# yzh119/custom_op_benchmark

Measured on AMD Instinct MI355X. Metric: edges/sec fwd+bwd (SDDMM+softmax+SpMM) on Reddit d=64; HBM GB/s vs roofline, higher is better.
Workload: dtype f32; 1 GPU; reddit-shape Chung-Lu(alpha=0.50) graph, N=232965 E=114615892 per GPU, h=1 d=64, U[0,1) values, chunk_size=32, int64 CSR both orientations; graph=reddit, nodes=232965, edges=114615892, heads=1, d=64, chunk_size=32, row_chunks=3694777, col_chunks=3694424, parallelism=single GPU

## Files before the change

custom_op_benchmark_amd/_lib.py:

```python
import atexit
import collections
import ctypes
import os
import weakref

import torch

_HERE = os.path.dirname(os.path.abspath(__file__))
LIB_PATH = os.environ.get("GRAPHOP_LIB") or os.path.join(_HERE, "libgraphop_hip.so")
ABI_VERSION = 8

F32, F64 = 0, 1
_c64 = ctypes.c_int64
_vp = ctypes.c_void_p
_lib = None


class PlanInfo(ctypes.Structure):
    _fields_ = [("n_chunks", _c64), ("n_edges", _c64), ("n_segments", _c64), ("max_row", _c64),
                ("max_index", _c64), ("max_segment_len", _c64), ("rows_sorted", ctypes.c_int32),
                ("indptr_monotone", ctypes.c_int32), ("eid_identity", ctypes.c_int32),
                ("full_coverage", ctypes.c_int32), ("row_owned", ctypes.c_int32),
                ("has_idx32", ctypes.c_int32), ("dense_fill_pct", ctypes.c_int32),
                ("sorted_in_rows", ctypes.c_int32), ("n_dense_blocks", _c64), ("max_row_gap", _c64),
                ("n_geometry_fallbacks", _c64)]


class SweepInfo(ctypes.Structure):
    _fields_ = [("win_cols", _c64), ("W", ctypes.c_int32), ("T", ctypes.c_int32), ("V", ctypes.c_int32),
                ("n_dealt", ctypes.c_int32)]


ALLOC_FN = ctypes.CFUNCTYPE(ctypes.c_void_p, ctypes.c_size_t, ctypes.c_int, ctypes.c_void_p)
FREE_FN = ctypes.CFUNCTYPE(None, ctypes.c_void_p)


class ProfileRec(ctypes.Structure):
    _fields_ = [("name", ctypes.c_char * 48), ("kernel", ctypes.c_char * 48), ("calls", _c64), ("total_ms", ctypes.c_double),
                ("min_ms", ctypes.c_double), ("max_ms", ctypes.c_double)]


_P = _vp
_SIGNATURES = {
    "graphop_tune": [ctypes.c_char_p, ctypes.c_int],
    "graphop_tune_reset": [],
    "graphop_check_device_errors": [],
    "graphop_tune_get": [ctypes.c_char_p, ctypes.POINTER(ctypes.c_int)],
    "graphop_profile_enable": [ctypes.c_int],
    "graphop_profile_read": [ctypes.POINTER(ProfileRec), ctypes.c_int],
    "graphop_partition_csr_count": [_P, _c64, _c64, _P, _P],
    "graphop_partition_csr_fill": [_P, _P, _c64, _c64, _c64, _P, _P, _P],
    "graphop_plan_create": [_P, _P, _P, _P, _c64, _c64, _c64, _P, ctypes.POINTER(_vp)],
    "graphop_plan_info": [_P, ctypes.POINTER(PlanInfo)],
    "graphop_set_allocator": [ALLOC_FN, FREE_FN],
    "graphop_plan_prepare": [_P, ctypes.c_int, _c64, _c64, _c64, ctypes.c_int, _P],
    "graphop_plan_n_sweeps": [_P],
    "graphop_plan_sweep_info": [_P, ctypes.c_int, ctypes.POINTER(SweepInfo)],
    "graphop_plan_array": [_P, ctypes.c_char_p, ctypes.c_int, ctypes.POINTER(_vp), ctypes.POINTER(_c64)],
    "graphop_plan_import": [_P] * 4 + [ctypes.POINTER(PlanInfo)] + [_P] * 4 + [_c64] + [_P] * 4 + [ctypes.POINTER(_vp)],
    "graphop_plan_import_sweep": [_P, ctypes.POINTER(SweepInfo), _P, _P, _P, _P],
    "graphop_plan_sweep_dealt": [_P, ctypes.c_int, ctypes.c_int, ctypes.POINTER(ctypes.c_int32), ctypes.POINTER(ctypes.c_int32)],
    "graphop_plan_sweep_build_dealt": [_P, ctypes.POINTER(SweepInfo), ctypes.c_int32, ctypes.c_int32, _P],
    "graphop_maskedmm_csr_forward": [ctypes.c_int] + [_P] * 7 + [_c64] * 6 + [_P, _P],
    "graphop_maskedmm_csr_forward_partial": [ctypes.c_int] + [_P] * 7 + [_c64] * 7 + [_P],
    "graphop_maskedmm_csr_backward": [ctypes.c_int] + [_P] * 13 + [_c64] * 7 + [_P, _P, _P],
    "graphop_sparse_softmax_forward": [ctypes.c_int] + [_P] * 5 + [_c64] * 3 + [_P, _c64, _P, _P],
    "graphop_sparse_softmax_backward": [ctypes.c_int] + [_P] * 6 + [_c64] * 3 + [_P, _c64, _P, _P],
    "graphop_vector_spmm_forward": [ctypes.c_int] + [_P] * 7 + [_c64] * 6 + [_P, _P],
    "graphop_vector_spmm_backward": [ctypes.c_int] + [_P] * 13 + [_c64] * 7 + [_P, _P, _P],
    "graphop_spmm_pair_supported": [ctypes.c_int] + [_c64] * 5 + [_P],
    "graphop_spmm_pair": [ctypes.c_int] + [_P] * 9 + [_c64] * 6 + [_P, _P],
    "graphop_interleave_pairs": [ctypes.c_int, _P, _P, _P, _c64, _P],
    "graphop_node_mul_edge_forward": [ctypes.c_int] + [_P] * 6 + [_c64] * 5 + [_P, _P],
    "graphop_node_mul_edge_backward": [ctypes.c_int] + [_P] * 8 + [_c64] * 5 + [_P, _P],
    "graphop_gat_scores_forward": [ctypes.c_int] + [_P] * 7 + [_c64] * 5 + [ctypes.c_double, _P, _P],
    "graphop_gat_scores_backward": [ctypes.c_int] + [_P] * 13 + [_c64] * 6 + [ctypes.c_double, _P, _P, _P],
    "graphop_gatv2_scores_forward": [ctypes.c_int] + [_P] * 8 + [_c64] * 6 + [ctypes.c_double, _P, _P],
    "graphop_gatv2_scores_backward": [ctypes.c_int] + [_P] * 16 + [_c64] * 8 + [ctypes.c_double, _P, _P, _P],
    "graphop_gatv2_attention_forward": [ctypes.c_int] + [_P] * 9 + [_c64] * 6 + [ctypes.c_double, _P, _P],
    "graphop_gatv2_attention_backward": [ctypes.c_int] + [_P] * 18 + [_c64] * 8 + [ctypes.c_double, _P, _P, _P],
    "graphop_gatv2_attention_dropout_forward": [ctypes.c_int] + [_P] * 9 + [_c64] * 6
    + [ctypes.c_double, ctypes.c_double, ctypes.c_uint64, ctypes.c_uint32, _P, _P],
    "graphop_gatv2_attention_dropout_backward": [ctypes.c_int] + [_P] * 18 + [_c64] * 8
    + [ctypes.c_double, ctypes.c_double, ctypes.c_uint64, ctypes.c_uint32, _P, _P, _P],
    "graphop_gat_attention_forward": [ctypes.c_int] + [_P] * 9 + [_c64] * 6 + [ctypes.c_double, _P, _P],
    "graphop_gat_attention_backward": [ctypes.c_int] + [_P] * 18 + [_c64] * 8 + [ctypes.c_double, _P, _P, _P],
    "graphop_gat_attention_dropout_forward": [ctypes.c_int] + [_P] * 9 + [_c64] * 6
    + [ctypes.c_double, ctypes.c_double, ctypes.c_uint64, ctypes.c_uint32, _P, _P],
    "graphop_gat_attention_dropout_backward": [ctypes.c_int] + [_P] * 18 + [_c64] * 8
    + [ctypes.c_double, ctypes.c_double, ctypes.c_uint64, ctypes.c_uint32, _P, _P, _P],
    "graphop_edge_dropout_mask": [ctypes.c_int] + [_P] * 5 + [_c64] * 5
    + [ctypes.c_double, ctypes.c_uint64, ctypes.c_uint32, _P, _P],
    "graphop_gat_edge_attention_forward": [ctypes.c_int] + [_P] * 10 + [_c64] * 6
    + [ctypes.c_double, ctypes.c_double, ctypes.c_uint64, ctypes.c_uint32, _P, _P],
    "graphop_gat_edge_attention_backward": [ctypes.c_int] + [_P] * 20 + [_c64] * 8
    + [ctypes.c_double, ctypes.c_double, ctypes.c_uint64, ctypes.c_uint32, _P, _P, _P],
    "graphop_gatv2_edge_attention_forward": [ctypes.c_int] + [_P] * 10 + [_c64] * 6
    + [ctypes.c_double, ctypes.c_double, ctypes.c_uint64, ctypes.c_uint32, _P, _P],
    "graphop_gatv2_edge_attention_backward": [ctypes.c_int] + [_P] * 20 + [_c64] * 8
    + [ctypes.c_double, ctypes.c_double, ctypes.c_uint64, ctypes.c_uint32, _P, _P, _P],
    "graphop_gather_rows": [ctypes.c_int, _P, _P, _P, _c64, _c64, _c64, _P],
    "graphop_scatter_add_rows": [ctypes.c_int, _P, _P, _P, _c64, _c64, _c64, _P],
    "graphop_add_rows_unique": [ctypes.c_int, _P, _P, _P, _c64, _c64, _c64, _P],
    "graphop_add_rows_grouped": [ctypes.c_int, _P, _P, _P, _P, _P, _c64, _c64, _c64, _P],
    "graphop_attention_workspace_bytes": [ctypes.c_int, ctypes.c_int] + [_c64] * 5 + [_P, _P, _P,
                                                                                       ctypes.POINTER(_c64)],
    "graphop_attention_backward_is_fused": [ctypes.c_int] + [_c64] * 5 + [_P, _P, _P, ctypes.POINTER(ctypes.c_int)],
    "graphop_attention_forward": [ctypes.c_int] + [_P] * 9 + [_c64] * 6 + [_P, _c64, _P, _P],
    "graphop_attention_backward": [ctypes.c_int] + [_P] * 17 + [_c64] * 7 + [_P, _c64, _P, _P, _P],
    "graphop_attention_dropout_workspace_bytes": [ctypes.c_int, ctypes.c_int] + [_c64] * 5 + [_P, _P, _P,
                                                                                               ctypes.POINTER(_c64)],
    "graphop_attention_dropout_forward": [ctypes.c_int] + [_P] * 9 + [_c64] * 6 + [_P, _c64, _P, _P]
    + [ctypes.c_double, ctypes.c_uint64, ctypes.c_uint32, _c64],
    "graphop_attention_dropout_backward": [ctypes.c_int] + [_P] * 17 + [_c64] * 7 + [_P, _c64, _P, _P, _P]
    + [ctypes.c_double, ctypes.c_uint64, ctypes.c_uint32, _c64],
    "graphop_attention_bias_workspace_bytes": [ctypes.c_int, ctypes.c_int] + [_c64] * 5 + [_P, _P, _P, ctypes.c_int,
                                                                                            ctypes.POINTER(_c64)],
    "graphop_attention_bias_forward": [ctypes.c_int] + [_P] * 10 + [_c64] * 6 + [_P, _c64, _P, _P]
    + [ctypes.c_double, ctypes.c_uint64, ctypes.c_uint32, _c64],
    "graphop_attention_bias_backward": [ctypes.c_int] + [_P] * 19 + [_c64] * 7 + [_P, _c64, _P, _P, _P]
    + [ctypes.c_double, ctypes.c_uint64, ctypes.c_uint32, _c64],
    "graphop_attention_edge_workspace_bytes": [ctypes.c_int, ctypes.c_int] + [_c64] * 5 + [_P, _P, _P,
                                                                                            ctypes.POINTER(_c64)],
    "graphop_attention_edge_forward": [ctypes.c_int] + [_P] * 10 + [_c64] * 6 + [_P, _c64, _P, _P]
    + [ctypes.c_double, ctypes.c_uint64, ctypes.c_uint32, _c64],
    "graphop_attention_edge_backward": [ctypes.c_int] + [_P] * 19 + [_c64] * 7 + [_P, _c64, _P, _P, _P]
    + [ctypes.c_double, ctypes.c_uint64, ctypes.c_uint32, _c64],
    "graphop_attention_etype_workspace_bytes": [ctypes.c_int, ctypes.c_int] + [_c64] * 6 + [_P, _P, _P,
                                                                                             ctypes.POINTER(_c64)],
    "graphop_attention_etype_forward": [ctypes.c_int] + [_P] * 11 + [_c64] * 7 + [_P, _c64, _P, _P]
    + [ctypes.c_double, ctypes.c_uint64, ctypes.c_uint32, _c64],
    "graphop_attention_etype_backward": [ctypes.c_int] + [_P] * 20 + [_c64] * 8 + [_P, _c64, _P, _P, _P]
    + [ctypes.c_double, ctypes.c_uint64, ctypes.c_uint32, _c64],
    "graphop_attention_tbias_workspace_bytes": [ctypes.c_int, ctypes.c_int] + [_c64] * 6 + [_P, _P, _P,
                                                                                             ctypes.POINTER(_c64)],
    "graphop_attention_tbias_forward": [ctypes.c_int] + [_P] * 11 + [_c64] * 7 + [_P, _c64, _P, _P]
    + [ctypes.c_double, ctypes.c_uint64, ctypes.c_uint32, _c64],
    "graphop_attention_tbias_backward": [ctypes.c_int] + [_P] * 20 + [_c64] * 8 + [_P, _c64, _P, _P, _P]
    + [ctypes.c_double, ctypes.c_uint64, ctypes.c_uint32, _c64],
    "graphop_attention_weights": [ctypes.c_int] + [_P] * 10 + [_c64] * 6 + [_P, _P],
}
EXPORTED_SYMBOLS = sorted(list(_SIGNATURES) + ["graphop_abi_version", "graphop_last_error",
                                               "graphop_plan_destroy", "graphop_memory_bytes", "graphop_tune_key"])


def lib():
    global _lib
    if _lib is None:
        if not os.path.exists(LIB_PATH):
            raise RuntimeError(
                "graphop: %s is missing -- the HIP extension has not been built. Run "
                "`python -c 'import __graft_entry__ as g; g.build()'` (or `make -C "
                "custom_op_benchmark_amd/csrc`). There is no CPU fallback." % LIB_PATH)
        l = ctypes.CDLL(LIB_PATH)
        l.graphop_abi_version.restype = ctypes.c_int
        l.graphop_last_error.restype = ctypes.c_char_p
        l.graphop_plan_destroy.restype = None
        l.graphop_plan_destroy.argtypes = [_vp]
        l.graphop_memory_bytes.restype = ctypes.c_int64
        l.graphop_memory_bytes.argtypes = []
        l.graphop_tune_key.restype = ctypes.c_char_p
        l.graphop_tune_key.argtypes = [ctypes.c_int]
        for name, argtypes in _SIGNATURES.items():
            fn = getattr(l, name)
            fn.restype = ctypes.c_int
            fn.argtypes = argtypes
        if l.graphop_abi_version() != ABI_VERSION:
            raise RuntimeError("graphop: ABI version mismatch (library %d, binding %d)"
                               % (l.graphop_abi_version(), ABI_VERSION))
        if os.environ.get("GRAPHOP_TORCH_ALLOC", "1") != "0":
            l.graphop_set_allocator(_ALLOC_CB, _FREE_CB)
            atexit.register(_drop_allocator, l)
        _lib = l
    return _lib


_live_blocks = {}

# ... 379 lines not shown
```

custom_op_benchmark_amd/csrc/common.h:

```cpp
#pragma once

#include <hip/hip_runtime.h>
#include <stdint.h>
#include <stdio.h>
#include <stdlib.h>
#include <string.h>

#include <utility>

#include "graphop_hip.h"

namespace graphop {

using i64 = long long;

void set_error(const char* fmt, ...) __attribute__((format(printf, 1, 2)));
const char* get_error();

#define GO_CHECK_ARG(cond, ...)                \
  do {                                         \
    if (!(cond)) {                             \
      ::graphop::set_error(__VA_ARGS__);       \
      return GRAPHOP_ERR_INVALID_ARGUMENT;     \
    }                                          \
  } while (0)

#define GO_HIP(expr)                                                                      \
  do {                                                                                    \
    hipError_t _e = (expr);                                                               \
    if (_e != hipSuccess) {                                                               \
      ::graphop::set_error("%s failed: %s (%s:%d)", #expr, hipGetErrorString(_e), __FILE__, \
                           __LINE__);                                                     \
      return GRAPHOP_ERR_HIP;                                                             \
    }                                                                                     \
  } while (0)

#define GO_LAUNCH_CHECK() GO_HIP(hipGetLastError())

inline int env_int(const char* name, int dflt) {
  const char* v = getenv(name);
  return (v && *v) ? atoi(v) : dflt;
}

inline i64 ceil_div(i64 a, i64 b) { return (a + b - 1) / b; }

hipError_t go_malloc(void** p, size_t bytes, hipStream_t st);
void go_free(void* p);
bool go_alloc_stream_ordered();

int check_not_capturing(hipStream_t st, const char* what);

int* device_error_word(bool create);
int check_async_error(bool clear = false);
int tuning_plan_trim();
int walk_launch_id(const char* tag);

struct PlanStats {
  i64 unsorted;
  i64 bad_indptr;
  i64 eid_not_identity;
  i64 bad_eid;
  i64 bad_index;
  i64 max_row;
  i64 max_gap;
  i64 max_index;
  i64 max_seg_len;
  i64 n_segments;
  i64 unsorted_ids;
};

}

namespace graphop {
struct Sweep {
  int W = 0;
  i64 win_cols = 0;
  int T = 0;
  int V = 0;
  int* vr_row = nullptr;
  int* wp_lo = nullptr;
  int* wp_hi = nullptr;
  int runtime_wp = 0;
  int* queues = nullptr;
  unsigned queue_next = 0;
  struct Dealt {
    int L = 0, K = 0;
    int tiles = 0;
    int* rec = nullptr;
    int* ids = nullptr;
    int* eids = nullptr;
    long long n_ids = 0;
  };
  static constexpr int kMaxDealt = 4;
  Dealt dealt[kMaxDealt];
  int n_dealt = 0;
};
struct Walk {
  int W = 0;
  i64 win_cols = 0;
  int groups = 0;
  int GW = 0;
  int K = 0;
  int rounds = 0;
  int xcd_slots = 0;
  long long n_slots = 0;
  int* ids = nullptr;
  int* widx = nullptr;
  int* bin_pos = nullptr;
  int* bin_rows = nullptr;
  int* bin_cum = nullptr;
  int* sync = nullptr;
  long long sync_ints = 0;
  unsigned sync_next = 0;
  int max_steps = 0;
  long long longest_run = 0;
};
constexpr int kWalkSyncRing = 4;
constexpr int kWalkK = 15;
constexpr int kWalkFirstPiece = 1 << 30;
constexpr int kWalkRowMask = (1 << 30) - 1;
constexpr int kWalkKShift = 26;
constexpr long long kLongSegment = 1024;
constexpr long long kLongSegmentBwd = 2048;
constexpr int kQueueRing = 64;
constexpr int kQueueInts = 8 * 64;
}

struct graphop_plan {
  graphop_plan_info_t info;
  int sorted_in_rows;
  void* sweeps;
  void* sweep_mu;
  void* walks;
  const int64_t* row;
  const int64_t* indptr;
  const int64_t* eid;
  const int64_t* indices;
  int64_t* seg_chunk;
  int64_t* seg_eptr;
  int32_t* idx32;
  int32_t* eid32;
  int32_t* long_segs;
  int64_t n_long;
  int32_t* blk_seg;
  int32_t* seg_e0;
  int32_t* seg_row;
  int device;
  int mirrors_pinned;
};

#ifdef __HIPCC__
namespace graphop {

constexpr int kWave = 64;

template <int CTRL>
__device__ __forceinline__ float dpp_f32(float v) {
  return __builtin_bit_cast(
      float, __builtin_amdgcn_update_dpp(0, __builtin_bit_cast(int, v), CTRL, 0xF, 0xF, true));
}

template <int CTRL>
__device__ __forceinline__ double dpp_f64(double v) {
  const long long b = __builtin_bit_cast(long long, v);
  const int lo = __builtin_amdgcn_update_dpp(0, (int)b, CTRL, 0xF, 0xF, true);
  const int hi = __builtin_amdgcn_update_dpp(0, (int)(b >> 32), CTRL, 0xF, 0xF, true);
  return __builtin_bit_cast(double, ((long long)hi << 32) | (unsigned)lo);
}
template <int CTRL> __device__ __forceinline__ float dpp_t(float v) { return dpp_f32<CTRL>(v); }
template <int CTRL> __device__ __forceinline__ double dpp_t(double v) { return dpp_f64<CTRL>(v); }

template <int G>
__device__ __forceinline__ double group_sum(double v) {
  if constexpr (G >= 2) v += dpp_f64<0xB1>(v);
  if constexpr (G >= 4) v += dpp_f64<0x4E>(v);
  if constexpr (G >= 8) v += dpp_f64<0x141>(v);
  if constexpr (G >= 16) v += dpp_f64<0x140>(v);
  if constexpr (G >= 32) v += __shfl_xor(v, 16);
  if constexpr (G >= 64) v += __shfl_xor(v, 32);
  return v;
}

template <int G>
__device__ __forceinline__ float group_sum(float v) {
  if constexpr (G >= 2) v += dpp_f32<0xB1>(v);
  if constexpr (G >= 4) v += dpp_f32<0x4E>(v);
  if constexpr (G >= 8) v += dpp_f32<0x141>(v);
  if constexpr (G >= 16) v += dpp_f32<0x140>(v);
  if constexpr (G >= 32) v += __shfl_xor(v, 16);
  if constexpr (G >= 64) v += __shfl_xor(v, 32);
  return v;
}

__device__ __forceinline__ float group_sum_rt(float v, int g) {
  switch (g) {
    case 2: return group_sum<2>(v);
    case 4: return group_sum<4>(v);
    case 8: return group_sum<8>(v);
    case 16: return group_sum<16>(v);
    case 32: return group_sum<32>(v);
    case 64: return group_sum<64>(v);
    default: return v;
  }
}

template <typename F, int... I>
__device__ __forceinline__ void static_for_impl(F&& f, std::integer_sequence<int, I...>) {
  (f(std::integral_constant<int, I>{}), ...);
}
template <int N, typename F>
__device__ __forceinline__ void static_for(F&& f) {
  static_for_impl(f, std::make_integer_sequence<int, N>{});
}

template <int L, int U>
__device__ __forceinline__ int group_bcast(int v) {
  static_assert(U >= 0 && U < L, "lane out of range");
  if constexpr (L == 16) {
    return __builtin_amdgcn_update_dpp(0, v, 0x150 + U, 0xF, 0xF, true);
  } else if constexpr (L == 4) {
    return __builtin_amdgcn_update_dpp(0, v, U * 0x55, 0xF, 0xF, true);
  } else if constexpr (L == 8) {
    const int lo = __builtin_amdgcn_update_dpp(0, v, 0x150 + U, 0xF, 0xF, true);
    const int hi = __builtin_amdgcn_update_dpp(0, v, 0x150 + U + 8, 0xF, 0xF, true);
    return (threadIdx.x & 8) ? hi : lo;
  } else if constexpr (L == 64) {
    return __builtin_amdgcn_readlane(v, U);
  } else if constexpr (L == 32) {
    const int lo = __builtin_amdgcn_readlane(v, U);
    const int hi = __builtin_amdgcn_readlane(v, U + 32);
    return (threadIdx.x & 32) ? hi : lo;
  } else {
    return __shfl(v, U, L);
  }
}
template <int L, int U>
__device__ __forceinline__ unsigned group_bcast(unsigned v) { return (unsigned)group_bcast<L, U>((int)v); }
template <int L, int U>
__device__ __forceinline__ float group_bcast(float v) {
  return __builtin_bit_cast(float, group_bcast<L, U>(__builtin_bit_cast(int, v)));
}
template <int L, int U>
__device__ __forceinline__ double group_bcast(double v) {
  const long long b = __builtin_bit_cast(long long, v);
  const int lo = group_bcast<L, U>((int)b), hi = group_bcast<L, U>((int)(b >> 32));
  return __builtin_bit_cast(double, ((long long)hi << 32) | (unsigned)lo);
}

// ... 97 lines not shown
```

custom_op_benchmark_amd/csrc/graphop_hip.hip:

```cpp
#include <stdarg.h>

#include <map>
#include <mutex>
#include <set>
#include <string>
#include <vector>

#include "common.h"
#include "host.h"
#include "host_attn_rows.h"
#include "kernels_fast.h"
#include "kernels_walk.h"
#include "kernels_attn_walk.h"
#include "kernels_attn_bias_fwd.h"
#include "kernels_block.h"
#include "kernels_attn.h"
#include "kernels_generic.h"

namespace graphop {

namespace {

inline int cpg_for(i64 n_chunks, int cpg_max, int F) {
  return (int)chunks_per_group(n_chunks, F >= 256 ? 64 : (F / 4 > 0 ? F / 4 : 1), cpg_max);
}

inline unsigned blocks_for(i64 work, i64 per_block) {
  i64 b = ceil_div(work > 0 ? work : 1, per_block);
  return (unsigned)b;
}

inline bool fast_ok(int dtype, i64 h, i64 d, i64 n_edges, i64 n_src_rows) {
  if (tuning().force_generic || dtype != GRAPHOP_F32) return false;
  const i64 F = h * d;
  if (d % 4 != 0 || !pow2(F) || F < 16 || F > 1024 || !pow2(h)) return false;
  if (n_edges >= 0x7fffffffLL || n_src_rows >= 0x7fffffffLL) return false;
  return true;
}

inline bool fast64_ok(int dtype, i64 h, i64 d, i64 n_edges, i64 n_src_rows) {
  if (tuning().force_generic || dtype != GRAPHOP_F64 || h != 1) return false;
  if (d != 32 && d != 64 && d != 128) return false;
  return n_edges < 0x7fffffffLL && n_src_rows < 0x7fffffffLL;
}
}

int choose_sweep(const graphop_plan* plan, i64 n_table_rows, int L, int NV, hipStream_t st,
                 SweepLaunch* out, bool accumulating, const SweepOpts* opts) {
  const Tuning& t = tuning();
  if (!t.sweep || !plan) return 0;
  const graphop_plan_info_t& pi = plan->info;
  if (!pi.row_owned || !plan->sorted_in_rows || !pi.has_idx32 || !plan->indices) return 0;
  if (pi.n_segments == 0 || pi.n_edges == 0) return 0;
  const i64 row_bytes = (opts && opts->row_bytes > 0) ? opts->row_bytes : 16LL * L * NV;
  const i64 table_bytes = n_table_rows * row_bytes;
  if (table_bytes < (i64)t.sweep_min_kb * 1024) return 0;
  const i64 mean_row = pi.n_edges / pi.n_segments;
  auto windows_ok = [&](i64 w) {
    return w >= 2 && w <= t.max_windows && mean_row >= (i64)t.sweep_min_granule * w;
  };
  int coarse = (accumulating && pi.eid_identity && t.spmm_window_scale > 1) ? t.spmm_window_scale : 1;
  const i64 win_kb = (opts && opts->window_scale > 0) ? (i64)t.window_kb * opts->window_scale : (i64)t.window_kb;
  if (opts && opts->window_scale > 0) coarse = 1;
  i64 W = pow2ceil(ceil_div(table_bytes, win_kb * 1024));
  if (t.sweep_w > 0) W = t.sweep_w;
  if (!windows_ok(W)) {
    coarse = 1;
    W = table_bytes > (128LL << 20) ? pow2ceil(ceil_div(table_bytes, (i64)t.mall_window_kb * 1024)) : 0;
    if (!windows_ok(W)) return 0;
  } else if (t.sweep_w <= 0 && coarse > 1) {
    const i64 Wc = pow2ceil(ceil_div(table_bytes, (i64)t.window_kb * 1024 * coarse));
    if (Wc >= 2) W = Wc; else coarse = 1;
  } else if (t.sweep_w <= 0 && !accumulating && !(opts && opts->window_scale > 0) && row_bytes >= 1024) {
    while (W > 2 && mean_row < 12 * W) W >>= 1;
  }
  if (W < 2 || W > t.max_windows) return 0;
  const i64 win_cols = ceil_div(n_table_rows, W);
  int K = t.sweep_k > 0 ? t.sweep_k : (8 / NV > 0 ? 8 / NV : 1);
  if (opts && opts->K > 0) K = opts->K;
  if (t.sweep_k <= 0 && !(opts && opts->K > 0) && !pi.eid_identity && K > 1) K /= 2;
  if (K > L) K = L;
  const int gpb = kFastBlock / L;
  const int bpc_req = (opts && opts->bpc > 0) ? (opts->bpc < t.sweep_bpc || opts->window_scale > 0 ? opts->bpc : t.sweep_bpc)
                                              : t.sweep_bpc;
  const int bpc = bpc_req < 1 ? 1 : (bpc_req > kSweepBlocksPerCu ? kSweepBlocksPerCu : bpc_req);
  int T = t.vrow_t;
  if (T <= 0) {
    const i64 resident_vrows = (i64)t.n_cu * bpc * gpb * K;
    i64 target = pi.n_edges / (resident_vrows > 0 ? resident_vrows : 1);
    i64 p2 = 64;
    while (p2 * 2 <= target && p2 < 4096) p2 <<= 1;
    T = (int)(p2 * coarse * ((opts && opts->window_scale > 0) ? opts->window_scale : 1));
  }
  const Sweep* sw = nullptr;
  const int rc = plan_get_sweep(const_cast<graphop_plan*>(plan), (int)W, win_cols, T, st, &sw);
  if (rc != GRAPHOP_OK) return -rc;
  if (!sw) return 0;
  const int tile = (kWave / L) * K;
  const i64 tiles = ceil_div(sw->V, tile);
  if (tiles * ceil_div((i64)sw->W, 8) >= 0x7fffffffLL) return 0;
  out->view = SweepView{};
  const bool dry = opts && opts->dry_run;
  out->view.sync = dry ? nullptr : plan_take_queue(const_cast<graphop_plan*>(plan), sw);
  out->view.V = sw->V;
  out->view.W = sw->W;
  out->view.K = K;
  out->view.win_bytes = win_cols * row_bytes;
  out->view.table_bytes = table_bytes;
  out->view.touch = opts ? opts->touch : 0;
  if (!dry && zero_async(out->view.sync, sizeof(int) * kQueueInts, st) != hipSuccess) return -GRAPHOP_ERR_HIP;
  i64 nb = (i64)t.n_cu * bpc;
  const i64 need = ceil_div(tiles * sw->W, (i64)(kFastBlock / kWave));
  if (nb > need) nb = need;
  out->blocks = (unsigned)(nb < 1 ? 1 : nb);
  out->lds_bytes = (size_t)gpb * K * row_bytes;
  bool staged_ok = false;
  if (opts && opts->staged) {
    const Sweep::Dealt* dl = nullptr;
    const int rcd = plan_get_dealt(const_cast<graphop_plan*>(plan), sw, L, K, st, &dl, !opts->no_eids);
    if (rcd != GRAPHOP_OK) return -rcd;
    if (dl) {
      out->view.rec = (const int4*)dl->rec;
      out->view.ids_w = dl->ids;
      out->view.eids_w = dl->eids;
      out->lds_bytes += (size_t)gpb * opts->stage_lds_per_group;
      staged_ok = pi.eid_identity || dl->eids != nullptr || opts->no_eids;
    }
  }
  if (!staged_ok) {
    const int rcp = plan_pin_sweep_tables(const_cast<graphop_plan*>(plan), sw, st);
    if (rcp != GRAPHOP_OK) return -rcp;
  }
  out->view.wp_lo = sw->wp_lo;
  out->view.wp_hi = sw->wp_hi;
  out->view.vr_row = sw->vr_row;
  out->view.idx32 = plan->idx32;
  out->view.eid32 = plan->eid32;
  plan_trim(const_cast<graphop_plan*>(plan));
  out->view.wp_lo = sw->wp_lo;
  out->view.wp_hi = sw->wp_hi;
  out->view.idx32 = plan->idx32;
  out->view.eid32 = plan->eid32;
  return 1;
}

namespace {

inline bool table_off32(i64 n_table_rows, int L, int NV) { return n_table_rows * 16LL * L * NV < (1LL << 32); }
inline bool sddmm_staged_heads(int L, int NV, i64 h, i64 n_edges) {
  if (h < 2 || NV != 1 || L < 16 || L % h != 0 || n_edges * h >= 0x7fffffffLL) return false;
  const i64 d4 = L / h;
  return d4 == 4 || d4 == 8 || d4 == 16 || d4 == 32;
}
inline bool sddmm_staged(const graphop_plan* plan, int L, int NV, i64 h, i64 n_table_rows) {
  return (tuning().staged_ids & 1) && plan->info.eid_identity &&
         (h == 1 || (sddmm_staged_heads(L, NV, h, plan->info.n_edges) && table_off32(n_table_rows, L, NV)));
}
inline bool spmm_staged(int L, int NV, i64 h, i64 n_table_rows) {
  return (tuning().staged_ids & 2) && h == 1 && table_off32(n_table_rows, L, NV);
}

inline void allow_full_lds(const void* fn) {
  static std::mutex mu;
  static std::set<std::pair<int, const void*>> done;
  int dev = 0;
  (void)hipGetDevice(&dev);
  std::lock_guard<std::mutex> lk(mu);
  if (done.insert({dev, fn}).second)
    (void)hipFuncSetAttribute(fn, hipFuncAttributeMaxDynamicSharedMemorySize, 160 * 1024 - 1024);
}
struct WalkLaunch {
  WalkView view;
  unsigned blocks;
  size_t lds_bytes;
};

struct WalkDebug {
  long long* buf = nullptr;
  unsigned blocks = 0;
  const char* tag = "";
  hipStream_t st = nullptr;
  int rounds = 0, W = 0, waves_per_wg = 4;
  void arm(WalkLaunch* wl, const char* t, hipStream_t s, int wpw = 4) {
    waves_per_wg = wpw;
    if (!tuning().walk_debug) return;
    blocks = wl->blocks; tag = t; st = s; rounds = wl->view.rounds; W = wl->view.steps;
    if (hipMalloc((void**)&buf, sizeof(long long) * 34 * blocks) != hipSuccess) { buf = nullptr; return; }
    (void)hipMemsetAsync(buf, 0, sizeof(long long) * 34 * blocks, s);
    wl->view.dbg = buf;
  }
  ~WalkDebug() {
    if (!buf) return;
    std::vector<long long> h((size_t)34 * blocks);
    if (hipStreamSynchronize(st) == hipSuccess &&
        hipMemcpy(h.data(), buf, sizeof(long long) * h.size(), hipMemcpyDeviceToHost) == hipSuccess) {
      double tot = 0, wait = 0, nw = 0, feed = 0, ftot = 0, fspace = 0; long long tmax = 0, tmin = 1LL << 62; int gave = 0;
      for (size_t b = 0; b < blocks; ++b) { ftot += h[(size_t)32 * blocks + 2 * b]; fspace += h[(size_t)32 * blocks + 2 * b + 1]; }
      double xt[8] = {0}, xw[8] = {0}; int xn[8] = {0};
      const size_t n = (size_t)waves_per_wg * blocks;
      for (size_t i = 0; i < n; ++i) {
        const long long* d = &h[i * 4];
        tot += d[0]; wait += d[1]; nw += d[2] & 0xffff; feed += (double)(d[2] >> 16);
        tmax = d[0] > tmax ? d[0] : tmax; tmin = d[0] < tmin ? d[0] : tmin;
        gave += (d[3] & 16) ? 1 : 0;
        const int x = (int)(d[3] & 7); xt[x] += d[0]; xw[x] += d[1]; xn[x]++;
      }
      fprintf(stderr, "[walk] %s rounds=%d steps=%d waves=%zu cycles mean %.0f min %lld max %lld | pacer wait %.1f %% of wave time, %.1f waits/wave, %d gave up | per XCD wait%%:",
              tag, rounds, W, n, tot / n, tmin, tmax, 100.0 * wait / (tot > 0 ? tot : 1), nw / n, gave);
      for (int x = 0; x < 8; ++x) fprintf(stderr, " %.0f(%d)", xn[x] ? 100.0 * xw[x] / (xt[x] > 0 ? xt[x] : 1) : 0.0, xn[x]);
      fprintf(stderr, " | workers wait for the feeder %.1f %%; feeder: %.0f cycles, %.1f %% waiting for ring space", 100.0 * feed / (tot > 0 ? tot : 1),
              ftot / (blocks ? blocks : 1), 100.0 * fspace / (ftot > 0 ? ftot : 1));
      fprintf(stderr, "\n");
    }
    (void)hipFree(buf);
  }
};

template <int L, int NV>
int choose_walk(const graphop_plan* plan, i64 n_table_rows, int K, hipStream_t st, WalkLaunch* out, bool dry_run = false,
                int tables = 1) {
  if constexpr (NV != 1 || L < 16) {
    return 0;
  } else {
    const Tuning& t = tuning();
    if (!plan) return 0;
    const graphop_plan_info_t& pi = plan->info;
    if (!pi.row_owned || !plan->sorted_in_rows || !pi.has_idx32 || !plan->indices) return 0;
    if (pi.n_segments == 0 || pi.n_edges == 0) return 0;
    if (pi.max_index >= (1LL << kWalkKShift) || n_table_rows > (1LL << kWalkKShift)) return 0;
    const i64 table_bytes = n_table_rows * 16LL * L * NV;
    if (table_bytes < (i64)t.sweep_min_kb * 1024) return 0;
    const i64 win_kb = pi.eid_identity ? t.walk_window_kb : (16LL * L * NV >= 1024 ? 2 * (i64)t.walk_window_kb_col : t.walk_window_kb_col);
    i64 W = t.sweep_w > 0 ? t.sweep_w : pow2ceil(ceil_div(table_bytes * tables, (win_kb > 0 ? win_kb : 1) * 1024));
    if (W < 2) W = 2;
    if (W > t.max_windows || W > 512) return 0;
    const i64 mean_row = pi.n_edges / pi.n_segments;
    if (mean_row < (i64)t.sweep_min_granule * W / 2) return 0;
    const int GPB = kWalkWorkers / L;
    i64 blocks = t.walk_blocks > 0 ? ceil_div((i64)t.walk_blocks * kFastBlock, kWalkWorkers) : (i64)t.n_cu;
    int slots = 8;
    if (blocks >= 8) blocks -= blocks % 8; else slots = 1;
    const i64 groups = blocks * GPB;
    if (pi.n_edges < groups * (i64)t.walk_min_bin) return 0;
    if (K < 1 || K > kWalkK) return 0;
    const Walk* wk = nullptr;
    const int rc = plan_get_walk(const_cast<graphop_plan*>(plan), (int)W, ceil_div(n_table_rows, W), (int)groups, 1, K,
                                 slots, st, &wk, tables == 1);
    if (rc != GRAPHOP_OK) return -rc;
    plan_trim(const_cast<graphop_plan*>(plan));
    if (!wk) return 0;
    out->view.ids = wk->ids; out->view.widx = wk->widx; out->view.bin_pos = wk->bin_pos;
    out->view.bin_rows = wk->bin_rows; out->view.bin_cum = wk->bin_cum;
    out->view.W = wk->W; out->view.groups = wk->groups; out->view.rounds = wk->rounds;
    out->view.K = wk->K;
    out->view.xcd_slots = slots;
    {
      i64 steps = (i64)wk->W * (t.walk_steps > 0 ? t.walk_steps : 1);
      if (steps > wk->max_steps) steps = wk->max_steps;
      if (steps > wk->longest_run / 16) steps = wk->longest_run / 16;
      out->view.steps = (int)(steps < 1 ? 1 : steps);
    }
    out->view.drift = t.walk_drift;
    out->view.sync = (t.walk_drift > 0 && !dry_run) ? plan_take_walk_sync(const_cast<graphop_plan*>(plan), wk) : nullptr;
    out->view.dbg = nullptr;
    out->view.err = device_error_word(false);
    out->view.launch_id = 0;
    out->view.fault = t.walk_fault;
    out->view.stream_weights = pi.eid_identity ? 1 : 0;
    out->blocks = (unsigned)blocks;
    out->lds_bytes = 0;
    if (!dry_run && out->view.sync &&
        zero_async(out->view.sync, sizeof(int) * 64 * (size_t)(8 + 16 * (i64)wk->rounds * out->view.steps), st) != hipSuccess)
      return -GRAPHOP_ERR_HIP;
    return 1;
  }
}

template <int L, int NV>
inline int spmm_walk_k(i64 h, int dtype = GRAPHOP_F32) {
  if (h != 1 && h != 2 && h != 4 && h != 8) return 0;
  if (dtype == GRAPHOP_F64 && h != 1) return 0;
  if (h > 1 && (NV != 1 || (4 * L) % h != 0 || (4 * L / h) % 4 != 0)) return 0;
// ... 24 lines not shown
      allow_full_lds((const void*)kfn);
      if (tuning().walk_debug) {
        int nb = -1;
        (void)hipOccupancyMaxActiveBlocksPerMultiprocessor(&nb, (const void*)kfn, kWalkThreads, lds_bytes);
        hipFuncAttributes fa;
        (void)hipFuncGetAttributes(&fa, (const void*)kfn);
        fprintf(stderr, "[walk] occupancy API: %d workgroups of %d threads per CU (dynamic LDS %zu, static %zu, regs %d, K %d)\n", nb,
                kWalkThreads, lds_bytes, (size_t)fa.sharedSizeBytes, fa.numRegs, K);
      }
      hipLaunchKernelGGL(kfn, dim3(wl.blocks), dim3(kWalkThreads), lds_bytes, st, wl.view, args...);
    };
    if (dtype == GRAPHOP_F64) {
      if constexpr (spmm_walk_rows<L, NV>(1, 2) >= 8) {
        const size_t lds_bytes = spmm_walk_lds_bytes<L, NV>(K, 1, 2);
        if (off32) launch(k_spmm_walk_f64<L, NV, true>, lds_bytes, (const double*)w, (const double*)X, (double*)out);
        else launch(k_spmm_walk_f64<L, NV, false>, lds_bytes, (const double*)w, (const double*)X, (double*)out);
      }
      return 1;
    }
    auto go = [&](auto hc) {
      constexpr int HV = decltype(hc)::value;
      if constexpr (spmm_walk_rows<L, NV>(HV) < 8) return;
      else {
        const size_t lds_bytes = spmm_walk_lds_bytes<L, NV>(K, HV);
        if constexpr (HV == 1) {
          if (!off32) { launch(k_spmm_walk_f32<L, NV, 1, false>, lds_bytes, (const float*)w, (const float*)X, (float*)out, d4); return; }
        }
        launch(k_spmm_walk_f32<L, NV, HV, true>, lds_bytes, (const float*)w, (const float*)X, (float*)out, d4);
      }
    };
    switch ((int)h) {
      case 1: go(std::integral_constant<int, 1>{}); break;
      case 2: go(std::integral_constant<int, 2>{}); break;
      case 4: go(std::integral_constant<int, 4>{}); break;
      default: go(std::integral_constant<int, 8>{}); break;
    }
    return 1;
  }
}

}

int attn_fwd_walk(const graphop_plan* plan, i64 n_q, i64 n_k, i64 h, i64 d, int dtype, const void* Q, const void* K,
                  const void* V, void* o, void* stats, void* ws, i64 ws_bytes, hipStream_t st, bool dry_run,
                  size_t* ws_needed, const AttnDrop* drop) {
  constexpr int L = 16;
  const Tuning& t = tuning();
  if (ws_needed) *ws_needed = 0;
  if (!t.attn_fwd_walk || !t.attn_fused || t.force_generic || dtype != GRAPHOP_F32 || h != 1 || d != 4 * L || !plan) return 0;
  if (!plan->info.eid_identity || !(t.walk & 2) || !table_off32(n_k, L, 1)) return 0;
  if (plan->info.max_row >= n_q || plan->info.max_index >= n_k) return 0;
  constexpr int KR = attn_walk_rows<L>();
  static_assert(KR >= 4, "rows per lane group of the fused forward");
  WalkLaunch wl;
  const int use = choose_walk<L, 1>(plan, n_k, KR, st, &wl, dry_run, 2);
  if (use != 1) return use;
  if (t.walk_steps > 1 && wl.view.steps >= 2 * t.walk_steps) wl.view.steps /= t.walk_steps;
  const i64 bins = (i64)wl.view.groups * wl.view.rounds, F = 4 * L;
  const AttnRowsFwdWs w(ws, 2 * bins, n_q, 1, F);
  if (ws_needed) *ws_needed = w.total;
  if (dry_run) return 1;
  if (!ws || (size_t)ws_bytes < w.total) return 0;
  AttnWalkArgs a;
  a.Q = (const float*)Q; a.K = (const float*)K; a.V = (const float*)V; a.o = (float*)o; a.stats = (float*)stats;
  a.p_row = w.p_row; a.p_ml = w.p_ml; a.p_o = w.p_o;
  if (zero_async(o, sizeof(float) * (size_t)(n_q * F), st) != hipSuccess) return -GRAPHOP_ERR_HIP;
  attn_pieces_fill("attn_fwd_setup", w, kAttnNegBig, st);
  {
    WalkDebug dbg;
    dbg.arm(&wl, "attn_fwd", st, kWalkWorkers / kWave);
    wl.view.launch_id = walk_launch_id("attn_fwd");
    ProfScope prof("attn_fwd", st, drop ? "k_attn_fwd_walk_f32<DROP>" : "k_attn_fwd_walk_f32");
    const size_t lds_bytes = (size_t)(kWalkWorkers / L) * attn_walk_group_bytes<L>(KR);
    if (drop) {
      allow_full_lds((const void*)k_attn_fwd_walk_f32<L, true>);
      hipLaunchKernelGGL((k_attn_fwd_walk_f32<L, true>), dim3(wl.blocks), dim3(kWalkThreads), lds_bytes, st, wl.view, a, *drop);
    } else {
      allow_full_lds((const void*)k_attn_fwd_walk_f32<L, false>);
      hipLaunchKernelGGL((k_attn_fwd_walk_f32<L, false>), dim3(wl.blocks), dim3(kWalkThreads), lds_bytes, st, wl.view, a, NoDrop{});
    }
  }
  attn_pieces_merge(
      "attn_fwd_merge", "k_attn_piece_add", w, L, st,
      [&](dim3 grid, dim3 block) { hipLaunchKernelGGL(k_attn_piece_max, grid, block, 0, st, w.p_row, w.p_ml, w.Mtmp, w.np); },
      [&](dim3 grid, dim3 block) {
        hipLaunchKernelGGL((k_attn_piece_add<L>), grid, block, 0, st, w.p_row, w.p_ml, w.p_o, w.Mtmp, w.Ltmp, a.o, w.np);
      },
      [&](dim3 grid, dim3 block) {
        hipLaunchKernelGGL((k_attn_piece_fin<L>), grid, block, 0, st, w.p_row, w.Mtmp, w.Ltmp, a.o, a.stats, w.np);
      });
  if (hipGetLastError() != hipSuccess) return -GRAPHOP_ERR_HIP;
  return 1;
}

int attn_bias_fwd_rows(const Csr& g, i64 n_q, i64 n_k, i64 h, i64 d, int dtype, const void* Q, const void* K,
                       const void* V, const void* b, void* o, void* stats, void* ws, i64 ws_bytes, hipStream_t st,
                       bool dry_run, size_t* ws_needed, const AttnDrop* drop) {
  const Tuning& t = tuning();
  const graphop_plan* plan = g.plan;
  const i64 n_chunks = g.n_chunks, n_edges = g.n_edges;
  if (ws_needed) *ws_needed = 0;
  if (!t.attn_fused || !t.attn_rows || t.force_generic || dtype != GRAPHOP_F32 || h != 1 || !plan) return 0;
  if (d % 4 != 0 || !pow2(d) || d < 16 || d > 1024 || n_edges == 0 || n_chunks == 0) return 0;
  if (!g.owned() || !plan->indices) return 0;
  if (plan->info.max_row >= n_q || plan->info.max_index >= n_k || n_q >= kWalkRowMask) return 0;
  const i64 F = d;
  const ChunkGeometry geo = attn_one_head_geometry(n_chunks, F);
  if (2 * geo.groups >= 0x7fffffffLL) return 0;
  const AttnRowsFwdWs w(ws, 2 * geo.groups, n_q, 1, F);
  if (ws_needed) *ws_needed = w.total;
  if (dry_run) return 1;
  if (!ws || (size_t)ws_bytes < w.total) return 0;
  AttnBiasFwdArgs a;
  a.Q = (const float*)Q; a.K = (const float*)K; a.V = (const float*)V; a.b = (const float*)b;
  a.o = (float*)o; a.stats = (float*)stats;
  a.p_row = w.p_row; a.p_ml = w.p_ml; a.p_o = w.p_o;
  if (zero_async(o, sizeof(float) * (size_t)(n_q * F), st) != hipSuccess) return -GRAPHOP_ERR_HIP;
  attn_pieces_fill("attn_bias_fwd_setup", w, kAttnNegBig, st);
  const i64* eids = g.eid_or_null();
  {
    ProfScope prof("attn_bias_fwd_rows", st, drop ? "k_attn_bias_fwd_rows_f32<DROP>" : "k_attn_bias_fwd_rows_f32");
    GO_DISPATCH_LNV((int)F, {
      if (drop)
        hipLaunchKernelGGL((k_attn_bias_fwd_rows_f32<L, NV, true>), dim3(geo.blocks), dim3(kFastBlock), 0, st,
                           g.row, g.indptr, eids, g.indices, a, n_chunks,
                           (int)geo.cpg, *drop);
      else
        hipLaunchKernelGGL((k_attn_bias_fwd_rows_f32<L, NV, false>), dim3(geo.blocks), dim3(kFastBlock), 0, st,
                           g.row, g.indptr, eids, g.indices, a, n_chunks,
                           (int)geo.cpg, NoDrop{});
    });
  }
  attn_pieces_merge(
      "attn_bias_fwd_merge", "k_attn_bias_piece_add", w, geo.lanes, st,
      [&](dim3 grid, dim3 block) { hipLaunchKernelGGL(k_attn_piece_max, grid, block, 0, st, w.p_row, w.p_ml, w.Mtmp, w.np); },
      [&](dim3 grid, dim3 block) {
        GO_DISPATCH_LNV((int)F, {
          hipLaunchKernelGGL((k_attn_bias_piece_add<L, NV>), grid, block, 0, st, w.p_row, w.p_ml, w.p_o, w.Mtmp, w.Ltmp,
                             a.o, w.np);
        });
      },
      [&](dim3 grid, dim3 block) {
        GO_DISPATCH_LNV((int)F, {
          hipLaunchKernelGGL((k_attn_bias_piece_fin<L, NV>), grid, block, 0, st, w.p_row, w.Mtmp, w.Ltmp, a.o, a.stats,
                             w.np);
        });
      });
  if (hipGetLastError() != hipSuccess) return -GRAPHOP_ERR_HIP;
  return 1;
}

namespace {

template <int L, int NV>
int try_sddmm_sweep(const char* tag, int dtype, const graphop_plan* plan, i64 n_table_rows, const void* A,
                    const void* B, void* y, i64 h, int d4, hipStream_t st) {
  if (!plan) return 0;
  SweepLaunch sl;
  SweepOpts so;
  const bool f64 = dtype == GRAPHOP_F64;
  if (f64 && (h != 1 || NV != 1 || L < 16 || !sddmm_staged(plan, L, NV, h, n_table_rows))) return 0;
  const bool off32 = table_off32(n_table_rows, L, NV);
  so.bpc = (f64 || !off32) ? 3 : sweep_bpc(NV, h == 1);
  so.touch = tuning().touch_sddmm;
  const bool id = plan->info.eid_identity != 0;
  so.staged = sddmm_staged(plan, L, NV, h, n_table_rows);
  so.stage_lds_per_group = StageCfg<L, 1>::kLdsIntsPerGroup * (int)sizeof(int) + (h > 1 ? 64 * (int)h : 0);
  if (h > 1 && !aligned16(y)) so.staged = false;
  const int use = choose_sweep(plan, n_table_rows, L, NV, st, &sl, false, &so);
  if (use != 1) return use;
  const bool staged = sl.view.rec != nullptr;
  if (f64 && !staged) return 0;
  ProfScope prof(tag, st, f64 ? "k_sddmm_wown_staged_f64" : staged ? "k_sddmm_wown_staged_f32" : "k_sddmm_wown_f32");
  const dim3 grid(sl.blocks), block(kFastBlock);
  if (f64) {
    if constexpr (NV == 1 && L >= 16) {
      if (off32) hipLaunchKernelGGL((k_sddmm_wown_staged_f64<L, NV, true>), grid, block, sl.lds_bytes, st, sl.view,
                                    (const double*)A, (const double*)B, (double*)y);
      else hipLaunchKernelGGL((k_sddmm_wown_staged_f64<L, NV, false>), grid, block, sl.lds_bytes, st, sl.view,
                              (const double*)A, (const double*)B, (double*)y);
    }
    return 1;
  }
  const float* a = (const float*)A;
  const float* b = (const float*)B;
  float* yy = (float*)y;
  if (staged) {
    if (h == 1) {
      if (off32) hipLaunchKernelGGL((k_sddmm_wown_staged_f32<L, NV, 0, true>), grid, block, sl.lds_bytes, st, sl.view, a, b, yy);
      else hipLaunchKernelGGL((k_sddmm_wown_staged_f32<L, NV, 0, false>), grid, block, sl.lds_bytes, st, sl.view, a, b, yy);
    } else if constexpr (NV == 1 && L >= 16) {
      auto go = [&](auto dc) {
        constexpr int D4 = decltype(dc)::value;
        if constexpr (D4 < L)
          hipLaunchKernelGGL((k_sddmm_wown_staged_f32<L, NV, D4>), grid, block, sl.lds_bytes, st, sl.view, a, b, yy);
      };
      switch (d4) {
        case 4: go(std::integral_constant<int, 4>{}); break;
        case 8: go(std::integral_constant<int, 8>{}); break;
        case 16: go(std::integral_constant<int, 16>{}); break;
        default: go(std::integral_constant<int, 32>{}); break;
      }
    }
    return 1;
  }
#define GO_K(H1, ID, O32)                                                                      \
  hipLaunchKernelGGL((k_sddmm_wown_f32<L, NV, H1, ID, O32>), grid, block, sl.lds_bytes, st,    \
                     sl.view, a, b, yy, (int)h, d4)
  if (h == 1) {
    if (id) { if (off32) GO_K(true, true, true); else GO_K(true, true, false); }
    else { if (off32) GO_K(true, false, true); else GO_K(true, false, false); }
  } else {
    if (id) GO_K(false, true, false); else GO_K(false, false, false);
  }
#undef GO_K
  return 1;
}

template <int L, int NV>
int try_spmm_sweep(const char* tag, const graphop_plan* plan, i64 n_table_rows, const void* w,
                   const void* X, void* out, i64 h, int d4, hipStream_t st) {
  SweepLaunch sl;
  SweepOpts so;
  so.bpc = sweep_bpc(NV, h == 1);
  const bool off32 = table_off32(n_table_rows, L, NV);
  so.staged = spmm_staged(L, NV, h, n_table_rows);
  const int use = choose_sweep(plan, n_table_rows, L, NV, st, &sl, true, &so);
  if (use != 1) return use;
  const bool id = plan->info.eid_identity != 0;
  const float* ww = (const float*)w;
  const bool staged = sl.view.rec != nullptr && (id || sl.view.eids_w != nullptr);
  ProfScope prof(tag, st, staged ? "k_spmm_wown_staged_f32" : "k_spmm_wown_f32");
  const dim3 grid(sl.blocks), block(kFastBlock);
  const float* x = (const float*)X;
  float* o = (float*)out;
  if (staged) {
    const size_t lds = (size_t)(kFastBlock / L) * (id ? StageCfg<L, 1>::kLdsIntsPerGroup : StageCfg<L, 2>::kLdsIntsPerGroup) * sizeof(int);
    if (id) hipLaunchKernelGGL((k_spmm_wown_staged_f32<L, NV, true>), grid, block, lds, st, sl.view, ww, x, o);
    else hipLaunchKernelGGL((k_spmm_wown_staged_f32<L, NV, false>), grid, block, lds, st, sl.view, ww, x, o);
    return 1;
  }
#define GO_K(H1, ID, O32)                                                                      \
  hipLaunchKernelGGL((k_spmm_wown_f32<L, NV, H1, ID, O32>), grid, block, 0, st, sl.view, ww,   \
                     x, o, (int)h, d4)
  if (h == 1) {
    if (id) { if (off32) GO_K(true, true, true); else GO_K(true, true, false); }
    else { if (off32) GO_K(true, false, true); else GO_K(true, false, false); }
  } else {
    if (id) GO_K(false, true, false); else GO_K(false, false, false);
  }
#undef GO_K
  return 1;
}

inline bool block_ok(const graphop_plan* plan, int dtype, i64 h, i64 d, i64 n_table_rows) {
  const Tuning& t = tuning();
  return t.dense_blocks && !t.force_generic && dtype == GRAPHOP_F32 && plan && plan->blk_seg &&
         plan->info.n_dense_blocks > 0 && plan->info.dense_fill_pct >= t.dense_min_fill &&
         plan->idx32 && (plan->info.eid_identity || plan->eid32) && n_table_rows < 0x7fffffffLL &&
         plan->info.n_dense_blocks * h < 0x7fffffffLL && h * d < 0x7fffffffLL;
}
inline BlockView block_view(const graphop_plan* plan) {
  BlockView bv;
  bv.blk_seg = plan->blk_seg; bv.seg_e0 = plan->seg_e0; bv.seg_row = plan->seg_row;
  bv.idx32 = plan->idx32; bv.eid32 = plan->eid32; bv.nb = (int)plan->info.n_dense_blocks;
  return bv;
}

inline int try_sddmm_block(const char* tag, int dtype, const graphop_plan* plan, i64 n_table_rows,
                           const void* A, const void* B, void* y, i64 h, i64 d, hipStream_t st) {
  if (!block_ok(plan, dtype, h, d, n_table_rows) || d % 8 != 0 || !aligned16(A) || !aligned16(B)) return 0;
  const int nw = d % 32 == 0 ? 4 : (d % 16 == 0 ? 2 : 1);
  ProfScope prof(tag, st, "k_sddmm_block_f32");
  const dim3 grid((unsigned)(plan->info.n_dense_blocks * h)), block(kWave * nw);
  const BlockView bv = block_view(plan);
  if (plan->info.eid_identity)
    hipLaunchKernelGGL((k_sddmm_block_f32<true>), grid, block, 0, st, bv, (const float*)A,
                       (const float*)B, (float*)y, (int)h, (int)d);
  else
    hipLaunchKernelGGL((k_sddmm_block_f32<false>), grid, block, 0, st, bv, (const float*)A,
                       (const float*)B, (float*)y, (int)h, (int)d);
  return 1;
}

inline bool spmm_block_applies(int dtype, const graphop_plan* plan, i64 n_table_rows, const void* X,
                               const void* out, i64 h, i64 d) {
  return block_ok(plan, dtype, h, d, n_table_rows) && d % 32 == 0 && aligned16(X) && aligned16(out);
}
inline bool spmm_block_writes_all(int dtype, const Csr& g, i64 n_table_rows, const void* X, const void* out, i64 h,
                                  i64 d, i64 n_out_rows) {
  return g.owned() && spmm_block_applies(dtype, g.plan, n_table_rows, X, out, h, d) &&
         g.plan->info.n_segments == n_out_rows && g.plan->info.max_row == n_out_rows - 1;
}

inline int try_spmm_block(const char* tag, int dtype, const graphop_plan* plan, i64 n_table_rows,
                          const void* w, const void* X, void* out, i64 h, i64 d, hipStream_t st) {
  if (!spmm_block_applies(dtype, plan, n_table_rows, X, out, h, d)) return 0;
  const int vw = d % 128 == 0 ? 4 : (d % 64 == 0 ? 2 : 1);
  const i64 groups = d / (32 * vw);
  const int nw = (int)(groups < 4 ? groups : 4);
  ProfScope prof(tag, st, "k_spmm_block_f32");
  const dim3 grid((unsigned)(plan->info.n_dense_blocks * h)), block(kWave * nw);
  const BlockView bv = block_view(plan);
  const bool id = plan->info.eid_identity != 0;
#define GO_K(VW, ID) hipLaunchKernelGGL((k_spmm_block_f32<VW, ID>), grid, block, 0, st, bv, \
                                        (const float*)w, (const float*)X, (float*)out, (int)h, (int)d)
  if (vw == 4) { if (id) GO_K(4, true); else GO_K(4, false); }
  else if (vw == 2) { if (id) GO_K(2, true); else GO_K(2, false); }
  else { if (id) GO_K(1, true); else GO_K(1, false); }
#undef GO_K
// ... 238 lines not shown
      const bool small_rows = mean_n4 <= 2 * G;
      const int n_long = (int)p->n_long;
      const unsigned nb = blocks_for(S, kFastBlock / G) + (unsigned)n_long;
      const i64 long_len = n_long > 0 ? kLongSegment : (i64)1 << 30;
      prof.kernel = BWD ? "k_softmax_bwd_vec4" : "k_softmax_fwd_vec4";
#define GO_V4R(GW, RM)                                                                              \
  if constexpr (!BWD)                                                                               \
    hipLaunchKernelGGL((k_softmax_fwd_vec4<GW, (RM ? 8 : kVec4CacheFwd)>), dim3(nb), dim3(kFastBlock), 0, st, \
                       (const i64*)p->seg_chunk, indptr, (const i64*)p->seg_eptr, in0, out, S, (int)h, long_len,             \
                       (const int*)p->long_segs, n_long, (const i64*)p->row, stats);                \
  else                                                                                              \
    hipLaunchKernelGGL((k_softmax_bwd_vec4<GW, (RM ? 8 : kVec4CacheBwd)>), dim3(nb), dim3(kFastBlock), 0, st, \
                       (const i64*)p->seg_chunk, indptr, (const i64*)p->seg_eptr, in0, in1, out, S, (int)h, long_len,        \
                       (const int*)p->long_segs, n_long);
#define GO_V4(GW) if (small_rows) { GO_V4R(GW, 1) } else { GO_V4R(GW, 0) }
      switch (G) {
        case 8: GO_V4(8) break;
        case 16: GO_V4(16) break;
        case 32: GO_V4(32) break;
        default: GO_V4(64) break;
      }
#undef GO_V4
#undef GO_V4R
      GO_LAUNCH_CHECK();
      return GRAPHOP_OK;
    }
  }
  if (pow2(h) && h <= 64) {
    const int G = seg_group_width(p->info.n_edges * h / S, h);
    const int n_long = (int)p->n_long;
    const unsigned nb = blocks_for(S, kFastBlock / G) + (unsigned)n_long;
    const i64 long_len = n_long > 0 ? (BWD ? kLongSegmentBwd : kLongSegment) : (i64)1 << 62;
#define GO_SEG(GW, ID)                                                                           \
  if constexpr (!BWD)                                                                            \
    hipLaunchKernelGGL((k_softmax_fwd_seg<T, GW, ID>), dim3(nb), dim3(kFastBlock), 0, st,        \
                       (const i64*)p->seg_chunk, indptr, (const i64*)p->seg_eptr, eid, in0, out, S, (int)h, long_len,     \
                       (const int*)p->long_segs, n_long, (const i64*)p->row, stats);             \
  else                                                                                           \
    hipLaunchKernelGGL((k_softmax_bwd_seg<T, GW, ID>), dim3(nb), dim3(kFastBlock), 0, st,        \
                       (const i64*)p->seg_chunk, indptr, (const i64*)p->seg_eptr, eid, in0, in1, out, S, (int)h, long_len, \
                       (const int*)p->long_segs, n_long);
#define GO_SEG_ID(GW) if (id) { GO_SEG(GW, true) } else { GO_SEG(GW, false) }
    switch (G) {
      case 8: GO_SEG_ID(8) break;
      case 16: GO_SEG_ID(16) break;
      case 32: GO_SEG_ID(32) break;
      default: GO_SEG_ID(64) break;
    }
#undef GO_SEG_ID
#undef GO_SEG
  } else {
    const unsigned nb = blocks_for(S, kFastBlock / kWave);
    hipLaunchKernelGGL((k_softmax_seg_anyh<T, BWD>), dim3(nb), dim3(kFastBlock), 0, st,
                       (const i64*)p->seg_chunk, indptr, (const i64*)p->seg_eptr, eid, in0, in1, out, S, h, (const i64*)p->row,
                       BWD ? (T*)nullptr : stats);
  }
  GO_LAUNCH_CHECK();
  return GRAPHOP_OK;
}

template <typename T>
int softmax_forward_t(const Csr& g, const T* x, T* y, i64 h, T* ws, i64 ws_rows, hipStream_t st, T* stats = nullptr) {
  const i64 *row = g.row, *indptr = g.indptr, *eid = g.eid;
  const i64 C = g.n_chunks, E = g.n_edges;
  const graphop_plan* plan = g.plan_slots;
  const bool owned = plan && plan->info.row_owned;
  const bool covered = owned && plan->info.full_coverage && plan->info.eid_identity;
  if (!covered && E * h > 0) GO_HIP(zero_async(y, sizeof(T) * (size_t)(E * h), st));
  if (C == 0) return GRAPHOP_OK;
  if (owned) return launch_softmax_seg<T, false>(g, x, (const T*)nullptr, y, h, st, stats);
  GO_CHECK_ARG(ws != nullptr && ws_rows > 0,
               "sparse_softmax_forward: the general (plan-less) path needs a workspace of "
               "2*workspace_rows*h values with workspace_rows > max(row)");
  T* max_val = ws;
  T* sum = ws + ws_rows * h;
  const unsigned fb = (unsigned)ceil_div(ws_rows * h, 256) > 4096u ? 4096u
                                                                   : (unsigned)ceil_div(ws_rows * h, 256);
  hipLaunchKernelGGL((k_fill<T>), dim3(fb), dim3(256), 0, st, max_val, ws_rows * h, (T)-1e9);
  GO_HIP(zero_async(sum, sizeof(T) * (size_t)(ws_rows * h), st));
  const unsigned nb = blocks_for(C, kGenericWavesPerBlock);
  hipLaunchKernelGGL((k_softmax_max<T>), dim3(nb), dim3(kGenericBlock), 0, st, row, indptr, eid, x,
                     max_val, C, h);
  hipLaunchKernelGGL((k_softmax_exp_sum<T>), dim3(nb), dim3(kGenericBlock), 0, st, row, indptr,
                     eid, x, (const T*)max_val, sum, y, C, h);
  hipLaunchKernelGGL((k_softmax_norm<T>), dim3(nb), dim3(kGenericBlock), 0, st, row, indptr, eid,
                     (const T*)sum, y, C, h);
  if (stats)
    hipLaunchKernelGGL((k_attn_stats_from_ws<T>), dim3(fb), dim3(256), 0, st, (const T*)max_val,
                       (const T*)sum, stats, ws_rows * h);
  GO_LAUNCH_CHECK();
  return GRAPHOP_OK;
}

template <typename T>
int softmax_backward_t(const Csr& g, const T* y, const T* dy, T* dx, i64 h, T* ws, i64 ws_rows, hipStream_t st) {
  const i64 *row = g.row, *indptr = g.indptr, *eid = g.eid;
  const i64 C = g.n_chunks, E = g.n_edges;
  const graphop_plan* plan = g.plan_slots;
  const bool owned = plan && plan->info.row_owned;
  const bool covered = owned && plan->info.full_coverage && plan->info.eid_identity;
  if (!covered && E * h > 0) GO_HIP(zero_async(dx, sizeof(T) * (size_t)(E * h), st));
  if (C == 0) return GRAPHOP_OK;
  if (owned) return launch_softmax_seg<T, true>(g, y, dy, dx, h, st);
  GO_CHECK_ARG(ws != nullptr && ws_rows > 0,
               "sparse_softmax_backward: the general (plan-less) path needs a workspace of "
               "workspace_rows*h values with workspace_rows > max(row)");
  GO_HIP(zero_async(ws, sizeof(T) * (size_t)(ws_rows * h), st));
  const unsigned nb = blocks_for(C, kGenericWavesPerBlock);
  hipLaunchKernelGGL((k_softmax_bwd_aggre<T>), dim3(nb), dim3(kGenericBlock), 0, st, row, indptr,
                     eid, dy, y, ws, C, h);
  hipLaunchKernelGGL((k_softmax_bwd_dx<T>), dim3(nb), dim3(kGenericBlock), 0, st, row, indptr, eid,
                     dy, y, (const T*)ws, dx, C, h);
  GO_LAUNCH_CHECK();
  return GRAPHOP_OK;
}

inline int check_common(const char* fn, int dtype, i64 C, i64 E, i64 h, i64 d) {
  GO_TRY(check_async_error(false));
  GO_CHECK_ARG(dtype == GRAPHOP_F32 || dtype == GRAPHOP_F64, "%s: dtype must be GRAPHOP_F32 or "
               "GRAPHOP_F64", fn);
  GO_CHECK_ARG(C >= 0 && E >= 0 && h >= 1 && d >= 0, "%s: negative size (n_chunks=%lld n_edges=%lld "
               "h=%lld d=%lld)", fn, (long long)C, (long long)E, (long long)h, (long long)d);
  return GRAPHOP_OK;
}

}

int softmax_forward_stats(int dtype, const Csr& g, const void* x, void* y, i64 h, void* ws, i64 ws_rows, hipStream_t st,
                          void* stats) {
  if (dtype == GRAPHOP_F32)
    return softmax_forward_t<float>(g, (const float*)x, (float*)y, h, (float*)ws, ws_rows, st, (float*)stats);
  return softmax_forward_t<double>(g, (const double*)x, (double*)y, h, (double*)ws, ws_rows, st, (double*)stats);
}
}

using namespace graphop;

extern "C" {

int graphop_plan_prepare(graphop_plan_t* plan, int dtype, int64_t n_table_rows, int64_t h, int64_t d,
                         int fused, void* stream) {
  GO_CHECK_ARG(plan != nullptr && n_table_rows >= 0 && h >= 1 && d >= 0, "plan_prepare: bad arguments");
  hipStream_t st = (hipStream_t)stream;
  const bool f64 = fast64_ok(dtype, h, d, plan->info.n_edges, n_table_rows);
  if (!f64 && !fast_ok(dtype, h, d, plan->info.n_edges, n_table_rows)) return GRAPHOP_OK;
  int rc = 0;
  GO_DISPATCH_LNV((int)(f64 ? 2 * d : h * d), {
    SweepLaunch sl;
    SweepOpts o;
    o.dry_run = 1;
    o.bpc = f64 ? 3 : sweep_bpc(NV, h == 1);
    o.staged = sddmm_staged(plan, L, NV, h, n_table_rows);
    o.stage_lds_per_group = StageCfg<L, 1>::kLdsIntsPerGroup * (int)sizeof(int) + (h > 1 ? 64 * (int)h : 0);
    if (!f64 || (o.staged && NV == 1 && L >= 16))
      rc = choose_sweep(plan, n_table_rows, L, NV, st, &sl, false, &o);
    o.staged = spmm_staged(L, NV, h, n_table_rows);
    if (rc >= 0 && !f64) rc = choose_sweep(plan, n_table_rows, L, NV, st, &sl, true, &o);
    if constexpr (NV == 1 && L >= 16) {
      WalkLaunch wl;
      const int bit = plan->info.eid_identity ? 2 : 4;
      const int K = spmm_walk_k<L, NV>(h, dtype);
      if (rc >= 0 && K > 0 && (tuning().walk & bit) && (h == 1 || table_off32(n_table_rows, L, NV))) {
        const int r2 = choose_walk<L, NV>(plan, n_table_rows, K, st, &wl, true);
        if (r2 < 0) rc = r2;
      }
    }
  });
  if (rc < 0) return -rc;
  if (fused && h == 1) {
    rc = 0;
    if (fused != 3) {
      const int fw = attn_fwd_walk(plan, plan->info.max_row + 1, n_table_rows, h, d, dtype, nullptr, nullptr, nullptr, nullptr,
                                   nullptr, nullptr, 0, st, true, nullptr);
      if (fw < 0) return -fw;
    }
    if (fused != 3) rc = attn_prepare_plan(plan, n_table_rows, d, false, st);
    if (rc >= 0 && fused != 2) rc = attn_prepare_plan(plan, n_table_rows, d, true, st);
    if (rc < 0) return -rc;
  }
  return GRAPHOP_OK;
}

int graphop_maskedmm_csr_forward(int dtype, const int64_t* row, const int64_t* indptr,
                                 const int64_t* eid, const int64_t* indices, const void* A,
                                 const void* B, void* y, int64_t n_chunks, int64_t n_edges,
                                 int64_t n_a, int64_t n_b, int64_t h, int64_t d,
                                 const graphop_plan_t* plan, void* stream) {
  const char* fn = "maskedmm_csr_forward";
  GO_TRY(check_common(fn, dtype, n_chunks, n_edges, h, d));
  hipStream_t st = (hipStream_t)stream;
  if (n_edges * h == 0) return GRAPHOP_OK;
  GO_PTR(fn, y);
  const Csr g(row, indptr, eid, indices, n_chunks, n_edges, plan);
  if (!g.covered(true)) GO_HIP(zero_async(y, esize(dtype) * (size_t)(n_edges * h), st));
  if (n_chunks == 0) return GRAPHOP_OK;
  GO_TRY(g.require(fn)); GO_PTR(fn, A); GO_PTR(fn, B);
  GO_TRY(Csr::check_bounds(fn, g.plan_slots, "A", n_a, nullptr, 0));
  GO_TRY(Csr::check_bounds(fn, g.plan, "A", n_a, "B", n_b));
  return launch_sddmm<false>("sddmm_fwd", dtype, g, A, B, y, n_b, h, d, st);
}

int graphop_maskedmm_csr_forward_partial(int dtype, const int64_t* row, const int64_t* indptr,
                                         const int64_t* eid, const int64_t* indices, const void* A,
                                         const void* B, void* y, int64_t n_chunks, int64_t n_slots,
                                         int64_t n_y, int64_t n_a, int64_t n_b, int64_t h, int64_t d,
                                         void* stream) {
  const char* fn = "maskedmm_csr_forward_partial";
  GO_TRY(check_common(fn, dtype, n_chunks, n_slots, h, d));
  GO_CHECK_ARG(n_y >= n_slots && n_a >= 0 && n_b >= 0, "%s: n_y (%lld) must be at least n_slots (%lld): eid[] names distinct "
               "entries of y", fn, (long long)n_y, (long long)n_slots);
  hipStream_t st = (hipStream_t)stream;
  if (n_slots * h == 0 || n_chunks == 0) return GRAPHOP_OK;
  const Csr g(row, indptr, eid, indices, n_chunks, n_y, nullptr);
  GO_PTR(fn, y); GO_TRY(g.require(fn)); GO_PTR(fn, A); GO_PTR(fn, B);
  return launch_sddmm<false>("sddmm_fwd_part", dtype, g, A, B, y, n_b, h, d, st);
}

int graphop_maskedmm_csr_backward(int dtype, const int64_t* row, const int64_t* indptr_r,
                                  const int64_t* eid_r, const int64_t* indices_r,
                                  const int64_t* col, const int64_t* indptr_c,
                                  const int64_t* eid_c, const int64_t* indices_c, const void* A,
                                  const void* B, const void* dy, void* dA, void* dB,
                                  int64_t n_row_chunks, int64_t n_col_chunks, int64_t n_edges,
                                  int64_t n_a, int64_t n_b, int64_t h, int64_t d,
                                  const graphop_plan_t* plan_r, const graphop_plan_t* plan_c,
                                  void* stream) {
  const char* fn = "maskedmm_csr_backward";
  GO_TRY(check_common(fn, dtype, n_row_chunks, n_edges, h, d));
  GO_CHECK_ARG(n_col_chunks >= 0 && n_a >= 0 && n_b >= 0, "%s: negative size", fn);
  hipStream_t st = (hipStream_t)stream;
  const size_t es = esize(dtype);
  const Csr r(row, indptr_r, eid_r, indices_r, n_row_chunks, n_edges, plan_r, "row", "indptr_r", "eid_r", "indices_r");
  const Csr c(col, indptr_c, eid_c, indices_c, n_col_chunks, n_edges, plan_c, "col", "indptr_c", "eid_c", "indices_c");
  GO_TRY(Csr::check_bounds(fn, r.plan, "A / dA", n_a, "B", n_b));
  GO_TRY(Csr::check_bounds(fn, c.plan, "B / dB", n_b, "A", n_a));
  bool sz_a = false, sz_b = false;
  if (n_a * h * d > 0 && !(dA == nullptr && n_row_chunks == 0)) {
    GO_PTR(fn, dA);
    sz_a = dy != nullptr && B != nullptr && spmm_selfzero(dtype, r, n_b, dy, B, dA, h, d, n_a, st);
    if (!sz_a && !spmm_block_writes_all(dtype, r, n_b, B, dA, h, d, n_a))
      GO_HIP(zero_async(dA, es * (size_t)(n_a * h * d), st));
  }
  if (n_b * h * d > 0 && !(dB == nullptr && n_col_chunks == 0)) {
    GO_PTR(fn, dB);
    sz_b = dy != nullptr && A != nullptr && spmm_selfzero(dtype, c, n_a, dy, A, dB, h, d, n_b, st);
    if (!sz_b && !spmm_block_writes_all(dtype, c, n_a, A, dB, h, d, n_b))
      GO_HIP(zero_async(dB, es * (size_t)(n_b * h * d), st));
  }
  if (h * d == 0) return GRAPHOP_OK;
  if (n_row_chunks > 0) {
    GO_TRY(r.require(fn)); GO_PTR(fn, B); GO_PTR(fn, dy);
    GO_TRY(launch_spmm<false>("sddmm_bwd_dA", dtype, r, dy, B, dA, n_b, h, d, st, sz_a ? n_a : -1));
  }
  if (n_col_chunks > 0) {
    GO_TRY(c.require(fn)); GO_PTR(fn, A); GO_PTR(fn, dy);
    GO_TRY(launch_spmm<false>("sddmm_bwd_dB", dtype, c, dy, A, dB, n_a, h, d, st, sz_b ? n_b : -1));
  }
  return GRAPHOP_OK;
}

int graphop_sparse_softmax_forward(int dtype, const int64_t* row, const int64_t* indptr,
                                   const int64_t* eid, const void* x, void* y, int64_t n_chunks,
                                   int64_t n_edges, int64_t h, void* workspace,
                                   int64_t workspace_rows, const graphop_plan_t* plan,
                                   void* stream) {
  const char* fn = "sparse_softmax_forward";
  GO_TRY(check_common(fn, dtype, n_chunks, n_edges, h, 0));
  if (n_edges * h == 0) return GRAPHOP_OK;
  GO_PTR(fn, y);
  const Csr g(row, indptr, eid, nullptr, n_chunks, n_edges, plan);
  if (n_chunks > 0) { GO_TRY(g.require(fn, false)); GO_PTR(fn, x); }
  return softmax_forward_stats(dtype, g, x, y, h, workspace, workspace_rows, (hipStream_t)stream, nullptr);
}

int graphop_sparse_softmax_backward(int dtype, const int64_t* row, const int64_t* indptr,
                                    const int64_t* eid, const void* y, const void* dy, void* dx,
                                    int64_t n_chunks, int64_t n_edges, int64_t h,
                                    void* workspace, int64_t workspace_rows,
                                    const graphop_plan_t* plan, void* stream) {
  const char* fn = "sparse_softmax_backward";
  GO_TRY(check_common(fn, dtype, n_chunks, n_edges, h, 0));
  if (n_edges * h == 0) return GRAPHOP_OK;
  GO_PTR(fn, dx);
  const Csr g(row, indptr, eid, nullptr, n_chunks, n_edges, plan);
  if (n_chunks > 0) { GO_TRY(g.require(fn, false)); GO_PTR(fn, y); GO_PTR(fn, dy); }
  if (dtype == GRAPHOP_F32)
    return softmax_backward_t<float>(g, (const float*)y, (const float*)dy, (float*)dx, h, (float*)workspace,
                                     workspace_rows, (hipStream_t)stream);
  return softmax_backward_t<double>(g, (const double*)y, (const double*)dy, (double*)dx, h, (double*)workspace,
                                    workspace_rows, (hipStream_t)stream);
}

int graphop_vector_spmm_forward(int dtype, const int64_t* row, const int64_t* indptr,
                                const int64_t* eid, const int64_t* indices, const void* edata,
                                const void* x, void* y, int64_t n_chunks, int64_t n_edges,
                                int64_t n_x, int64_t n_y, int64_t h, int64_t d,
                                const graphop_plan_t* plan, void* stream) {
  const char* fn = "vector_spmm_forward";
  GO_TRY(check_common(fn, dtype, n_chunks, n_edges, h, d));
  GO_CHECK_ARG(n_x >= 0 && n_y >= 0, "%s: negative size", fn);
  hipStream_t st = (hipStream_t)stream;
  const Csr g(row, indptr, eid, indices, n_chunks, n_edges, plan);
  GO_TRY(Csr::check_bounds(fn, g.plan, "y", n_y, "x", n_x));
  if (n_y * h * d == 0) return GRAPHOP_OK;
  GO_PTR(fn, y);
  const bool sz = edata != nullptr && x != nullptr && spmm_selfzero(dtype, g, n_x, edata, x, y, h, d, n_y, st);
  if (!sz && !spmm_block_writes_all(dtype, g, n_x, x, y, h, d, n_y))
// ... 186 lines not shown
```

custom_op_benchmark_amd/csrc/host.h:

```cpp
#pragma once
#include "common.h"

namespace graphop {

struct ProfScope {
  hipEvent_t t0 = nullptr, t1 = nullptr;
  hipStream_t st;
  const char* name;
  const char* kernel;
  ProfScope(const char* n, hipStream_t s, const char* k = "");
  ~ProfScope();
};

struct Tuning {
  int sddmm_cpg;
  int spmm_cpg;
  int force_generic;
  int sweep;
  int window_kb;
  int mall_window_kb;
  int max_windows;
  int sweep_min_kb;
  int sweep_bpc;
  int sweep_k;
  int vrow_t;
  int sweep_min_granule;
  int dense_blocks;
  int dense_min_fill;
  int dense_detect_min_fill;
  int sweep_w;
  int spmm_window_scale;
  int attn_fused;
  int attn_window_scale;
  int attn_k;
  int attn_bpc;
  int staged_ids;
  int attn_fwd_walk;
  int spmm_selfzero;
  int spmm_selfzero_min_mb;
  int spmm_flat;
  int spmm_flat_max_mean;
  int spmm_flat_cpg;
  int spmm_flat_min_chunks;
  int attn_max_d;
  int attn_rows;
  int attn_heads;
  int touch_sddmm;
  int walk;
  int walk_window_kb;
  int walk_window_kb_col;
  int walk_drift;
  int walk_steps;
  int walk_min_bin;
  int walk_debug;
  int walk_fault;
  int walk_blocks;
  int plan_trim;
  int n_cu;
  Tuning() {
    sweep = env_int("GRAPHOP_SWEEP", 1);
    window_kb = env_int("GRAPHOP_WINDOW_KB", 4096);
    mall_window_kb = env_int("GRAPHOP_MALL_WINDOW_KB", 32768);
    max_windows = env_int("GRAPHOP_MAX_WINDOWS", 128);
    sweep_min_kb = env_int("GRAPHOP_SWEEP_MIN_KB", 4608);
    sweep_bpc = env_int("GRAPHOP_SWEEP_BPC", 3);
    sweep_k = env_int("GRAPHOP_SWEEP_K", 0);
    vrow_t = env_int("GRAPHOP_VROW_T", 0);
    sweep_min_granule = env_int("GRAPHOP_SWEEP_MIN_GRANULE", 4);
    sweep_w = env_int("GRAPHOP_SWEEP_W", 0);
    spmm_window_scale = env_int("GRAPHOP_SPMM_WINDOW_SCALE", 2);
    dense_blocks = env_int("GRAPHOP_DENSE_BLOCKS", 1);
    dense_min_fill = env_int("GRAPHOP_DENSE_MIN_FILL", 40);
    dense_detect_min_fill = env_int("GRAPHOP_DENSE_DETECT_MIN_FILL", 10);
    attn_fused = env_int("GRAPHOP_ATTN_FUSED", 1);
    attn_fwd_walk = env_int("GRAPHOP_ATTN_FWD_WALK", 1);
    spmm_selfzero = env_int("GRAPHOP_SPMM_SELFZERO", 1);
    spmm_selfzero_min_mb = env_int("GRAPHOP_SPMM_SELFZERO_MIN_MB", 256);
    spmm_flat = env_int("GRAPHOP_SPMM_FLAT", 1);
    spmm_flat_max_mean = env_int("GRAPHOP_SPMM_FLAT_MAX_MEAN", 10);
    spmm_flat_cpg = env_int("GRAPHOP_SPMM_FLAT_CPG", 32);
    if (spmm_flat_cpg < 1) spmm_flat_cpg = 1;
    spmm_flat_min_chunks = env_int("GRAPHOP_SPMM_FLAT_MIN_CHUNKS", 1 << 20);
    attn_window_scale = env_int("GRAPHOP_ATTN_WINDOW_SCALE", 2);
    attn_k = env_int("GRAPHOP_ATTN_K", 0);
    attn_bpc = env_int("GRAPHOP_ATTN_BPC", 0);
    attn_rows = env_int("GRAPHOP_ATTN_ROWS", -1);
    attn_heads = env_int("GRAPHOP_ATTN_HEADS", -1);
    attn_max_d = env_int("GRAPHOP_ATTN_MAX_D", 64);
    staged_ids = env_int("GRAPHOP_STAGED_IDS", 7);
    touch_sddmm = env_int("GRAPHOP_TOUCH_SDDMM", 1);
    walk = env_int("GRAPHOP_WALK", 6);
    walk_window_kb = env_int("GRAPHOP_WALK_WINDOW_KB", 4096);
    walk_window_kb_col = env_int("GRAPHOP_WALK_WINDOW_KB_COL", 2048);
    walk_drift = env_int("GRAPHOP_WALK_DRIFT", 3);
    walk_steps = env_int("GRAPHOP_WALK_STEPS", 2);
    walk_min_bin = env_int("GRAPHOP_WALK_MIN_BIN", 1024);
    walk_blocks = env_int("GRAPHOP_WALK_BLOCKS", 0);
    walk_debug = env_int("GRAPHOP_WALK_DEBUG", 0);
    walk_fault = 0;
    plan_trim = env_int("GRAPHOP_PLAN_TRIM", 1);
    n_cu = 256;
    int dev = 0;
    hipDeviceProp_t prop;
    if (hipGetDevice(&dev) == hipSuccess && hipGetDeviceProperties(&prop, dev) == hipSuccess &&
        prop.multiProcessorCount > 0)
      n_cu = prop.multiProcessorCount;
    sddmm_cpg = env_int("GRAPHOP_SDDMM_CPG", 8);
    spmm_cpg = env_int("GRAPHOP_SPMM_CPG", 16);
    force_generic = env_int("GRAPHOP_FORCE_GENERIC", 0);
    if (sddmm_cpg < 1) sddmm_cpg = 1;
    if (spmm_cpg < 1) spmm_cpg = 1;
  }
};
Tuning& tuning_mut();
const Tuning& tuning();

hipError_t zero_async(void* ptr, size_t bytes, hipStream_t st);

struct SweepView;
}

#include "kernels_fast.h"

namespace graphop {

inline i64 chunks_per_group(i64 n_chunks, int lanes, i64 cap, int rounds = 8) {
  const i64 groups_wanted = (i64)tuning().n_cu * (kFastBlock / lanes) * rounds;
  const i64 c = n_chunks / (groups_wanted > 0 ? groups_wanted : 1);
  return c < 1 ? 1 : (c < cap ? c : cap);
}

struct ChunkGeometry {
  i64 cpg, groups;
  unsigned blocks;
  int lanes;
};
inline ChunkGeometry chunk_geometry(i64 n_chunks, int lanes, i64 cap, int rounds = 8) {
  const i64 cpg = chunks_per_group(n_chunks, lanes, cap, rounds), groups = ceil_div(n_chunks, cpg);
  return {cpg, groups, (unsigned)ceil_div(groups, (i64)(kFastBlock / lanes)), lanes};
}

struct SweepLaunch {
  SweepView view;
  unsigned blocks;
  size_t lds_bytes;
};

struct SweepOpts {
  i64 row_bytes = 0;
  int K = 0;
  int window_scale = 0;
  int bpc = 0;
  int dry_run = 0;
  int touch = 0;
  int staged = 0;
  int stage_lds_per_group = 0;
  int no_eids = 0;
};

int choose_sweep(const graphop_plan* plan, i64 n_table_rows, int L, int NV, hipStream_t st,
                 SweepLaunch* out, bool accumulating = false, const SweepOpts* opts = nullptr);

int partition_count(const i64*, i64, i64, i64*, hipStream_t);
int partition_fill(const i64*, const i64*, i64, i64, i64, i64*, i64*, hipStream_t);
int plan_build(graphop_plan*, i64, hipStream_t, int);
int plan_get_sweep(graphop_plan*, int, i64, int, hipStream_t, const Sweep**);
int* plan_take_queue(graphop_plan*, const Sweep*);
int plan_get_dealt(graphop_plan*, const Sweep*, int, int, hipStream_t, const Sweep::Dealt**, bool want_eids = true);
void plan_free_sweeps(graphop_plan*);
int plan_get_walk(graphop_plan*, int, i64, int, int, int, int, hipStream_t, const Walk**, bool want_widx = true);
int plan_build_seg_eptr(graphop_plan*, hipStream_t);
int* plan_take_walk_sync(graphop_plan*, const Walk*);
int plan_n_sweeps(const graphop_plan* p);
const Sweep* plan_sweep_at(const graphop_plan* p, int i);
int plan_import_arrays(graphop_plan* p, const i64* seg_chunk, const int32_t* idx32, const int32_t* eid32,
                       const int32_t* long_segs, i64 n_long, const int32_t* blk_seg,
                       const int32_t* seg_e0, const int32_t* seg_row, hipStream_t st);
int plan_import_sweep(graphop_plan* p, int W, i64 win_cols, int T, int V, const int32_t* vr_row,
                      const int32_t* wp_lo, const int32_t* wp_hi, hipStream_t st);
void plan_init_sweeps(graphop_plan*);
int plan_ensure_mirrors(graphop_plan* p, hipStream_t st);
int plan_pin_mirrors(graphop_plan* p, hipStream_t st);
int plan_ensure_mirrors_locked(graphop_plan* p, hipStream_t st);
int plan_rebuild_sweep_tables(graphop_plan* p, const Sweep* sw, hipStream_t st);
int plan_pin_sweep_tables(graphop_plan* p, const Sweep* sw, hipStream_t st);
void plan_trim(graphop_plan* p);
int attn_prepare_plan(const graphop_plan* plan, i64 n_table_rows, i64 d, bool col, hipStream_t st);

struct AttnDrop;
int attn_fwd_walk(const graphop_plan* plan, i64 n_q, i64 n_k, i64 h, i64 d, int dtype, const void* Q, const void* K,
                  const void* V, void* o, void* stats, void* ws, i64 ws_bytes, hipStream_t st, bool dry_run,
                  size_t* ws_needed, const AttnDrop* drop = nullptr);

struct Csr;
int attn_bias_fwd_rows(const Csr& g, i64 n_q, i64 n_k, i64 h, i64 d, int dtype, const void* Q, const void* K,
                       const void* V, const void* b, void* o, void* stats, void* ws, i64 ws_bytes, hipStream_t st,
                       bool dry_run, size_t* ws_needed, const AttnDrop* drop = nullptr);

struct HostDrop;
int attn_heads_fwd_rows(const Csr& g, i64 n_q, i64 n_k, i64 h, i64 d, int dtype, const void* Q, const void* K,
                        const void* V, const void* b, void* o, void* stats, void* ws, i64 ws_bytes, hipStream_t st,
                        bool dry_run, size_t* ws_needed, const HostDrop* drop = nullptr, i64 head0 = 0);
bool attn_heads_bwd_ok(int dtype, i64 h, i64 d, i64 n_edges, i64 n_q, i64 n_k, const graphop_plan* plan_r,
                       const graphop_plan* plan_c, hipStream_t st);
size_t attn_heads_bwd_workspace(i64 n_q, i64 n_k, i64 h, i64 d);
int attn_heads_backward(const Csr& r, const Csr& c, i64 n_q, i64 n_k, i64 h, i64 d, const void* Q, const void* K,
                        const void* V, const void* b, const void* o, const void* stats, const void* dO, void* dQ, void* dK,
                        void* dV, void* db, void* ws, hipStream_t st, const HostDrop* drop, i64 head0);

inline size_t esize(int dtype) { return dtype == GRAPHOP_F64 ? 8 : 4; }
inline bool pow2(i64 v) { return v > 0 && (v & (v - 1)) == 0; }
inline i64 pow2ceil(i64 v) { i64 p = 1; while (p < v) p <<= 1; return p; }

inline bool aligned16(const void* p) { return ((uintptr_t)p & 15) == 0; }

struct Csr {
  const i64 *row, *indptr, *eid, *indices;
  i64 n_chunks, n_edges;
  const graphop_plan *plan, *plan_slots;
  const char* names[4];

  Csr(const int64_t* row_, const int64_t* indptr_, const int64_t* eid_, const int64_t* indices_, i64 C, i64 E,
      const graphop_plan* p, const char* row_name = "row", const char* indptr_name = "indptr",
      const char* eid_name = "eid", const char* indices_name = "indices")
      : row((const i64*)row_), indptr((const i64*)indptr_), eid((const i64*)eid_), indices((const i64*)indices_),
        n_chunks(C), n_edges(E), names{row_name, indptr_name, eid_name, indices_name} {
    plan_slots = (p && p->row == row_ && p->indptr == indptr_ && p->eid == eid_ && p->info.n_chunks == C &&
                  p->info.n_edges == E) ? p : nullptr;
    plan = (plan_slots && p->indices == indices_) ? p : nullptr;
  }

  bool covered(bool slots = false) const {
    const graphop_plan* p = slots ? plan_slots : plan;
    return p && p->info.full_coverage && p->info.eid_identity && p->info.indptr_monotone;
  }
  bool owned() const { return plan && plan->info.rows_sorted; }
  const i64* eid_or_null() const { return plan->info.eid_identity ? nullptr : eid; }

  int require(const char* fn, bool has_indices = true) const {
    const void* ps[4] = {row, indptr, eid, indices};
    for (int i = 0; i < (has_indices ? 4 : 3); ++i)
      GO_CHECK_ARG(ps[i] != nullptr, "%s: %s is NULL", fn, names[i]);
    return GRAPHOP_OK;
  }
  static int check_bounds(const char* fn, const graphop_plan* p, const char* seg_name, i64 n_seg, const char* idx_name,
                          i64 n_idx) {
    if (!p) return GRAPHOP_OK;
    GO_CHECK_ARG(p->info.max_row < n_seg, "%s: row id %lld but %s has only %lld rows", fn, (long long)p->info.max_row,
                 seg_name, (long long)n_seg);
    GO_CHECK_ARG(!idx_name || p->info.max_index < n_idx, "%s: neighbour id %lld but %s has only %lld rows", fn,
                 (long long)p->info.max_index, idx_name, (long long)n_idx);
    return GRAPHOP_OK;
  }
};

#define GO_DISPATCH_LNV(F, ...)                                      \
  switch (F) {                                                       \
    case 16: { constexpr int L = 4, NV = 1; __VA_ARGS__; } break;    \
    case 32: { constexpr int L = 8, NV = 1; __VA_ARGS__; } break;    \
    case 64: { constexpr int L = 16, NV = 1; __VA_ARGS__; } break;   \
    case 128: { constexpr int L = 32, NV = 1; __VA_ARGS__; } break;  \
    case 256: { constexpr int L = 64, NV = 1; __VA_ARGS__; } break;  \
    case 512: { constexpr int L = 64, NV = 2; __VA_ARGS__; } break;  \
    case 1024: { constexpr int L = 64, NV = 4; __VA_ARGS__; } break; \
    default: break;                                                  \
  }

int softmax_forward_stats(int dtype, const Csr& g, const void* x, void* y, i64 h, void* ws, i64 ws_rows, hipStream_t st,
                          void* stats);

#define GO_PTR(fn, p) GO_CHECK_ARG((p) != nullptr, "%s: " #p " is NULL", fn)
#define GO_TRY(expr)                     \
  do {                                   \
    int _rc = (expr);                    \
    if (_rc != GRAPHOP_OK) return _rc;   \
  } while (0)

}
```

custom_op_benchmark_amd/csrc/plan.hip:

```cpp
#include <hipcub/hipcub.hpp>

#include <mutex>
#include <vector>

#include "common.h"

namespace graphop {

namespace {

constexpr int kBlock = 256;

inline unsigned grid_for(i64 n, int block = kBlock, i64 cap = 1 << 20) {
  i64 g = ceil_div(n > 0 ? n : 1, block);
  return (unsigned)(g > cap ? cap : g);
}

__global__ void k_part_count(const i64* __restrict__ indptr, i64 n_rows, i64 chunk,
                             i64* __restrict__ cnt) {
  i64 i = (i64)blockIdx.x * blockDim.x + threadIdx.x;
  const i64 stride = (i64)gridDim.x * blockDim.x;
  for (; i <= n_rows; i += stride) {
    i64 c = 0;
    if (i < n_rows) {
      const i64 deg = indptr[i + 1] - indptr[i];
      c = deg > 0 ? (deg + chunk - 1) / chunk : 0;
    }
    cnt[i] = c;
  }
}

__global__ void k_part_fill(const i64* __restrict__ indptr, const i64* __restrict__ first,
                            i64 n_rows, i64 chunk, i64 n_chunks, i64* __restrict__ row,
                            i64* __restrict__ out) {
  i64 c = (i64)blockIdx.x * blockDim.x + threadIdx.x;
  const i64 stride = (i64)gridDim.x * blockDim.x;
  if (c == 0) out[n_chunks] = indptr[n_rows];
  for (; c < n_chunks; c += stride) {
    i64 lo = 0, hi = n_rows;
    while (hi - lo > 1) {
      const i64 mid = (lo + hi) >> 1;
      if (first[mid] <= c) lo = mid; else hi = mid;
    }
    row[c] = lo;
    out[c] = indptr[lo] + (c - first[lo]) * chunk;
  }
}

__global__ void k_plan_chunks(const i64* __restrict__ row, const i64* __restrict__ indptr,
                              i64 n_chunks, i64 n_edges, int* __restrict__ head,
                              PlanStats* __restrict__ st) {
  i64 c = (i64)blockIdx.x * blockDim.x + threadIdx.x;
  const i64 stride = (i64)gridDim.x * blockDim.x;
  i64 unsorted = 0, bad = 0, mx = -1, gap = 0;
  for (; c < n_chunks; c += stride) {
    const i64 r = row[c];
    const i64 rp = c > 0 ? row[c - 1] : -1;
    head[c] = (c == 0 || r != rp) ? 1 : 0;
    if (c > 0 && r < rp) ++unsorted;
    if (r - rp - 1 > gap) gap = r - rp - 1;
    if (r < 0) ++bad;
    const i64 a = indptr[c], b = indptr[c + 1];
    if (a > b || a < 0 || b > n_edges) ++bad;
    mx = r > mx ? r : mx;
  }
  if (unsorted) atomicAdd((unsigned long long*)&st->unsorted, (unsigned long long)unsorted);
  if (bad) atomicAdd((unsigned long long*)&st->bad_indptr, (unsigned long long)bad);
  if (mx >= 0) atomicMax(&st->max_row, mx);
  if (gap > 0) atomicMax(&st->max_gap, gap);
}

__global__ void k_plan_edges(const i64* __restrict__ eid, const i64* __restrict__ indices,
                             i64 n_edges, i64 bound, PlanStats* __restrict__ st) {
  i64 k = (i64)blockIdx.x * blockDim.x + threadIdx.x;
  const i64 stride = (i64)gridDim.x * blockDim.x;
  i64 notid = 0, bad_e = 0, bad_i = 0, mx = -1;
  for (; k < n_edges; k += stride) {
    const i64 e = eid[k];
    if (e != k) ++notid;
    if (e < 0 || e >= n_edges) ++bad_e;
    if (indices) {
      const i64 v = indices[k];
      if (v < 0 || (bound > 0 && v >= bound)) ++bad_i;
      mx = v > mx ? v : mx;
    }
  }
  if (notid) atomicAdd((unsigned long long*)&st->eid_not_identity, (unsigned long long)notid);
  if (bad_e) atomicAdd((unsigned long long*)&st->bad_eid, (unsigned long long)bad_e);
  if (bad_i) atomicAdd((unsigned long long*)&st->bad_index, (unsigned long long)bad_i);
  if (mx >= 0) atomicMax(&st->max_index, mx);
}

__global__ void k_plan_fill_heads(const int* __restrict__ head, const i64* __restrict__ pos,
                                  i64 n_chunks, i64* __restrict__ seg_chunk,
                                  PlanStats* __restrict__ st) {
  i64 c = (i64)blockIdx.x * blockDim.x + threadIdx.x;
  const i64 stride = (i64)gridDim.x * blockDim.x;
  for (; c < n_chunks; c += stride) {
    if (head[c]) seg_chunk[pos[c]] = c;
    if (c == n_chunks - 1) {
      const i64 ns = pos[c] + head[c];
      seg_chunk[ns] = n_chunks;
      st->n_segments = ns;
    }
  }
}

__global__ void k_plan_seg_len(const i64* __restrict__ seg_chunk, const i64* __restrict__ indptr,
                               const PlanStats* __restrict__ st_in, PlanStats* __restrict__ st) {
  const i64 ns = st_in->n_segments;
  i64 s = (i64)blockIdx.x * blockDim.x + threadIdx.x;
  const i64 stride = (i64)gridDim.x * blockDim.x;
  i64 mx = 0;
  for (; s < ns; s += stride) {
    const i64 len = indptr[seg_chunk[s + 1]] - indptr[seg_chunk[s]];
    mx = len > mx ? len : mx;
  }
  if (mx > 0) atomicMax(&st->max_seg_len, mx);
}

__global__ void k_plan_long_segs(const i64* __restrict__ seg_chunk, const i64* __restrict__ indptr,
                                 i64 n_seg, i64 thresh, int* __restrict__ out, int cap,
                                 int* __restrict__ count) {
  i64 s = (i64)blockIdx.x * blockDim.x + threadIdx.x;
  const i64 stride = (i64)gridDim.x * blockDim.x;
  for (; s < n_seg; s += stride) {
    const i64 len = indptr[seg_chunk[s + 1]] - indptr[seg_chunk[s]];
    if (len > thresh) {
      const int pos = atomicAdd(count, 1);
      if (pos < cap) out[pos] = (int)s;
    }
  }
}

__global__ void k_narrow(const i64* __restrict__ src, int32_t* __restrict__ dst, i64 n) {
  i64 i = (i64)blockIdx.x * blockDim.x + threadIdx.x;
  const i64 stride = (i64)gridDim.x * blockDim.x;
  for (; i < n; i += stride) dst[i] = (int32_t)src[i];
}

__global__ void k_plan_sorted_ids(const i64* __restrict__ row, const i64* __restrict__ indptr,
                                  const i64* __restrict__ indices, i64 n_chunks,
                                  PlanStats* __restrict__ st) {
  i64 c = (i64)blockIdx.x * blockDim.x + threadIdx.x;
  const i64 stride = (i64)gridDim.x * blockDim.x;
  i64 bad = 0;
  for (; c < n_chunks; c += stride) {
    const i64 a = indptr[c], b = indptr[c + 1];
    for (i64 k = a; k + 1 < b; ++k) bad += indices[k] > indices[k + 1];
    if (b > a) {
      i64 c2 = c + 1;
      while (c2 < n_chunks && row[c2] == row[c] && indptr[c2 + 1] <= b) ++c2;
      if (c2 < n_chunks && row[c2] == row[c]) bad += indices[b - 1] > indices[b];
    }
  }
  if (bad) atomicAdd((unsigned long long*)&st->unsorted_ids, (unsigned long long)bad);
}

// ... 476 lines not shown
    std::vector<unsigned char> h_same((size_t)S);
    keep = hipMemcpy(h_same.data(), same.p, (size_t)S, hipMemcpyDeviceToHost) == hipSuccess;
    if (keep) {
      int run = 0;
      for (i64 s = 0; s < S; ++s) {
        if (s == 0 || !h_same[(size_t)s] || run == 32) { blk.push_back((int32_t)s); run = 0; }
        ++run;
      }
      blk.push_back((int32_t)S);
      const double fill = (double)E / (1024.0 * (double)(blk.size() - 1)) * 100.0;
      if (fill < min_fill) keep = false;
      else info.dense_fill_pct = (int32_t)(fill + 0.5) > 0 ? (int32_t)(fill + 0.5) : 1;
    }
  }
  if (keep) {
    keep = go_malloc((void**)&p->blk_seg, sizeof(int32_t) * blk.size(), st) == hipSuccess &&
           hipMemcpy(p->blk_seg, blk.data(), sizeof(int32_t) * blk.size(), hipMemcpyHostToDevice) == hipSuccess;
  }
  if (!keep) {
    go_free(seg_e0); go_free(seg_row);
    if (p->blk_seg) { go_free(p->blk_seg); p->blk_seg = nullptr; }
    info.dense_fill_pct = 0;
    return GRAPHOP_OK;
  }
  p->seg_e0 = seg_e0;
  p->seg_row = seg_row;
  info.n_dense_blocks = (i64)blk.size() - 1;
  return GRAPHOP_OK;
}

int plan_build_seg_eptr(graphop_plan* p, hipStream_t st) {
  const i64 S = p->info.n_segments;
  if (p->seg_eptr || !p->info.row_owned || !p->seg_chunk || !p->indptr || S <= 0) return GRAPHOP_OK;
  if (go_malloc((void**)&p->seg_eptr, sizeof(i64) * (size_t)(S + 1), st) != hipSuccess) {
    p->seg_eptr = nullptr;
    (void)hipGetLastError();
    return GRAPHOP_OK;
  }
  hipLaunchKernelGGL(k_seg_eptr, dim3(grid_for(S + 1, kBlock, 4096)), dim3(kBlock), 0, st,
                     (const i64*)p->seg_chunk, (const i64*)p->indptr, S, (i64*)p->seg_eptr);
  if (hipGetLastError() != hipSuccess || hipStreamSynchronize(st) != hipSuccess) {
    go_free(p->seg_eptr); p->seg_eptr = nullptr;
    return GRAPHOP_ERR_HIP;
  }
  return GRAPHOP_OK;
}

int plan_ensure_mirrors(graphop_plan* p, hipStream_t st) {
  if (!p->info.has_idx32) return GRAPHOP_OK;
  const i64 E = p->info.n_edges;
  const bool need_idx = p->indices && !p->idx32, need_eid = !p->info.eid_identity && p->eid && !p->eid32;
  if (!need_idx && !need_eid) return GRAPHOP_OK;
  const int rc_cap = check_not_capturing(st, "rebuilding the 32-bit index mirrors of a plan");
  if (rc_cap != GRAPHOP_OK) return rc_cap;
  if (need_idx) {
    GO_HIP(go_malloc((void**)&p->idx32, sizeof(int32_t) * (size_t)E, st));
    hipLaunchKernelGGL(k_narrow, dim3(grid_for(E, kBlock, 8192)), dim3(kBlock), 0, st, (const i64*)p->indices, p->idx32, E);
    GO_LAUNCH_CHECK();
  }
  if (need_eid) {
    GO_HIP(go_malloc((void**)&p->eid32, sizeof(int32_t) * (size_t)E, st));
    hipLaunchKernelGGL(k_narrow, dim3(grid_for(E, kBlock, 8192)), dim3(kBlock), 0, st, (const i64*)p->eid, p->eid32, E);
    GO_LAUNCH_CHECK();
  }
  GO_HIP(hipStreamSynchronize(st));
  return GRAPHOP_OK;
}

static int sweep_fill_arrays(graphop_plan* p, Sweep& s, hipStream_t st) {
  const i64 S = p->info.n_segments, E = p->info.n_edges;
  const int W = s.W, T = s.T;
  int rc = plan_ensure_mirrors(p, st);
  if (rc != GRAPHOP_OK) return rc;
  GO_CHECK_ARG(p->info.row_owned && p->sorted_in_rows && p->idx32 && E < 0x7fffffffLL && S > 0,
               "plan_get_sweep: plan is not sweepable");
  const i64* indptr = (const i64*)p->indptr;
  DevBuf seg_eptr, first, vr_seg, vr_ptr;
  GO_HIP(go_malloc(&seg_eptr.p, sizeof(i64) * (size_t)(S + 1), st));
  GO_HIP(go_malloc(&first.p, sizeof(i64) * (size_t)(S + 1), st));
  hipLaunchKernelGGL(k_seg_eptr, dim3(grid_for(S + 1, kBlock, 4096)), dim3(kBlock), 0, st,
                     (const i64*)p->seg_chunk, indptr, S, (i64*)seg_eptr.p);
  GO_LAUNCH_CHECK();
  rc = partition_count((const i64*)seg_eptr.p, S, T, (i64*)first.p, st);
  if (rc != GRAPHOP_OK) return rc;
  i64 V = 0;
  GO_HIP(hipMemcpyAsync(&V, (i64*)first.p + S, sizeof(i64), hipMemcpyDeviceToHost, st));
  GO_HIP(hipStreamSynchronize(st));
  GO_CHECK_ARG(V > 0 && V < 0x7fffffffLL && V * (W + 1) < (i64)1 << 40, "plan_get_sweep: size");
  GO_CHECK_ARG(s.V == 0 || s.V == (int)V, "plan_get_sweep: the graph changed under its plan");
  GO_HIP(go_malloc(&vr_seg.p, sizeof(i64) * (size_t)V, st));
  GO_HIP(go_malloc(&vr_ptr.p, sizeof(i64) * (size_t)(V + 1), st));
  rc = partition_fill((const i64*)seg_eptr.p, (const i64*)first.p, S, T, V, (i64*)vr_seg.p,
                      (i64*)vr_ptr.p, st);
  if (rc != GRAPHOP_OK) return rc;
  DevBuf rw;
  GO_HIP(go_malloc(&rw.p, sizeof(int) * (size_t)(S * (W + 1)), st));
  hipLaunchKernelGGL(k_sweep_row_windows, dim3(grid_for(S * (W + 1), kBlock, 16384)), dim3(kBlock),
                     0, st, (const i64*)seg_eptr.p, (const int32_t*)p->idx32, S, W, s.win_cols,
                     (int*)rw.p);
  GO_LAUNCH_CHECK();
  s.V = (int)V;
  const size_t wp_bytes = sizeof(int) * (size_t)(V * W);
  if ((!s.vr_row && go_malloc((void**)&s.vr_row, sizeof(int) * (size_t)V, st) != hipSuccess) ||
      (!s.wp_lo && go_malloc((void**)&s.wp_lo, wp_bytes, st) != hipSuccess) ||
      (!s.wp_hi && go_malloc((void**)&s.wp_hi, wp_bytes, st) != hipSuccess)) {
    go_free(s.vr_row); go_free(s.wp_lo); go_free(s.wp_hi);
    s.vr_row = s.wp_lo = s.wp_hi = nullptr;
    set_error("plan_get_sweep: out of device memory for %lld window pointers", (long long)(2 * V * W));
    return GRAPHOP_ERR_HIP;
  }
  hipLaunchKernelGGL(k_sweep_fill, dim3(grid_for(V * W, kBlock, 16384)), dim3(kBlock), 0, st,
                     (const i64*)vr_seg.p, (const i64*)first.p, (const i64*)p->seg_chunk,
                     (const i64*)p->row, (const int*)rw.p, S, V, W, s.vr_row, s.wp_lo, s.wp_hi);
  GO_LAUNCH_CHECK();
  GO_HIP(hipStreamSynchronize(st));
  return GRAPHOP_OK;
}

int plan_pin_sweep_tables(graphop_plan* p, const Sweep* sw, hipStream_t st) {
  std::lock_guard<std::mutex> lk(*(std::mutex*)p->sweep_mu);
  Sweep* s = const_cast<Sweep*>(sw);
  p->mirrors_pinned = 1;
  s->runtime_wp = 1;
  int rc = plan_ensure_mirrors(p, st);
  if (rc != GRAPHOP_OK) return rc;
  if (!s->wp_lo || !s->wp_hi || !s->vr_row) {
    const int rc_cap = check_not_capturing(st, "rebuilding the window tables of a plan");
    if (rc_cap != GRAPHOP_OK) return rc_cap;
    rc = sweep_fill_arrays(p, *s, st);
  }
  return rc;
}
int plan_rebuild_sweep_tables(graphop_plan* p, const Sweep* sw, hipStream_t st) {
  std::lock_guard<std::mutex> lk(*(std::mutex*)p->sweep_mu);
  return sweep_fill_arrays(p, *const_cast<Sweep*>(sw), st);
}
int plan_ensure_mirrors_locked(graphop_plan* p, hipStream_t st) {
  std::lock_guard<std::mutex> lk(*(std::mutex*)p->sweep_mu);
  return plan_ensure_mirrors(p, st);
}
int plan_pin_mirrors(graphop_plan* p, hipStream_t st) {
  std::lock_guard<std::mutex> lk(*(std::mutex*)p->sweep_mu);
  p->mirrors_pinned = 1;
  return plan_ensure_mirrors(p, st);
}

void plan_trim(graphop_plan* p) {
  if (!tuning_plan_trim()) return;
  std::lock_guard<std::mutex> lk(*(std::mutex*)p->sweep_mu);
  if (!p->mirrors_pinned && p->info.has_idx32 && !p->blk_seg) {
    if (p->idx32 && p->indices) { go_free(p->idx32); p->idx32 = nullptr; }
    if (p->eid32 && p->eid) { go_free(p->eid32); p->eid32 = nullptr; }
  }
  for (auto& s : *(std::vector<Sweep>*)p->sweeps)
    if (!s.runtime_wp && s.n_dealt > 0) {
      go_free(s.wp_lo); go_free(s.wp_hi);
      s.wp_lo = s.wp_hi = nullptr;
    }
}

int plan_get_sweep(graphop_plan* p, int W, i64 win_cols, int T, hipStream_t st, const Sweep** out) {
  auto* mu = (std::mutex*)p->sweep_mu;
  auto* vec = (std::vector<Sweep>*)p->sweeps;
  std::lock_guard<std::mutex> lk(*mu);
  for (auto& s : *vec)
    if (s.W == W && s.win_cols == win_cols && s.T == T) { *out = &s; return GRAPHOP_OK; }
  *out = nullptr;
  if (vec->size() >= 16) {
    if (p->info.n_geometry_fallbacks++ == 0)
      fprintf(stderr, "graphop: warning: a plan already holds 16 window geometries; the pass that asked for W=%d windows of "
              "%lld ids (pieces of <= %d slots) runs on the chunk drivers (2-3x slower on window-friendly shapes).  Use one "
              "plan per row width / fewer tuning changes, or drop the plan (graphs.release) between sweeps; "
              "graphop_plan_info().n_geometry_fallbacks counts these passes.\n", W, (long long)win_cols, T);
    return GRAPHOP_OK;
  }
  {
    const int rc_cap = check_not_capturing(st, "building the column-window structure of a plan");
    if (rc_cap != GRAPHOP_OK) return rc_cap;
  }
  Sweep s;
  s.W = W; s.win_cols = win_cols; s.T = T; s.V = 0;
  if (go_malloc((void**)&s.queues, sizeof(int) * kQueueRing * kQueueInts, st) != hipSuccess) {
    set_error("plan_get_sweep: out of device memory");
    return GRAPHOP_ERR_HIP;
  }
  const int rc = sweep_fill_arrays(p, s, st);
  if (rc != GRAPHOP_OK) {
    go_free(s.vr_row); go_free(s.wp_lo); go_free(s.wp_hi); go_free(s.queues);
    return rc;
  }
  vec->push_back(s);
  *out = &vec->back();
  return GRAPHOP_OK;
}

int* plan_take_walk_sync(graphop_plan* p, const Walk* wk) {
  std::lock_guard<std::mutex> lk(*(std::mutex*)p->sweep_mu);
  Walk* w = const_cast<Walk*>(wk);
  return w->sync + (size_t)(w->sync_next++ % kWalkSyncRing) * (size_t)w->sync_ints;
}

int* plan_take_queue(graphop_plan* p, const Sweep* sw) {
  std::lock_guard<std::mutex> lk(*(std::mutex*)p->sweep_mu);
  Sweep* s = const_cast<Sweep*>(sw);
  return s->queues + (size_t)(s->queue_next++ % kQueueRing) * kQueueInts;
}

int plan_get_dealt(graphop_plan* p, const Sweep* sw, int L, int K, hipStream_t st, const Sweep::Dealt** out, bool want_eids) {
  std::lock_guard<std::mutex> lk(*(std::mutex*)p->sweep_mu);
  Sweep* s = const_cast<Sweep*>(sw);
  const bool need_eids = want_eids && !p->info.eid_identity;
  for (int i = 0; i < s->n_dealt; ++i)
    if (s->dealt[i].L == L && s->dealt[i].K == K && (!need_eids || s->dealt[i].eids != nullptr)) { *out = &s->dealt[i]; return GRAPHOP_OK; }
  *out = nullptr;
  if (s->n_dealt >= Sweep::kMaxDealt) return GRAPHOP_OK;
  {
    const int rc_cap = check_not_capturing(st, "building the window-major id layout of a plan");
    if (rc_cap != GRAPHOP_OK) return rc_cap;
  }
  GO_CHECK_ARG(L >= 1 && L <= 64 && (64 % L) == 0 && K >= 1 && K <= L, "plan_get_dealt: bad geometry");
  {
    int rc_in = plan_ensure_mirrors(p, st);
    if (rc_in == GRAPHOP_OK && (!s->wp_lo || !s->wp_hi || !s->vr_row)) rc_in = sweep_fill_arrays(p, *s, st);
    if (rc_in != GRAPHOP_OK) return rc_in;
  }
  const int GW = 64 / L, tile = GW * K;
  const i64 tiles = ceil_div((i64)s->V, tile);
  const i64 tasks = tiles * s->W, strips = tasks * GW;
  const i64 E = p->info.n_edges;
  if (tasks * tile >= 0x7fffffffLL || E + 4 * strips + 1024 >= 0x7fffffffLL) return GRAPHOP_OK;
  Sweep::Dealt d;
  d.L = L; d.K = K; d.tiles = (int)tiles;
  d.n_ids = E + 3 * strips + 1024;
  DevBuf len, tmp;
  GO_HIP(go_malloc(&len.p, sizeof(int) * (size_t)(strips + 1), st));
  const bool with_eid = need_eids && p->eid32;
  if (go_malloc((void**)&d.rec, sizeof(int4) * (size_t)(tasks * tile), st) != hipSuccess ||
      go_malloc((void**)&d.ids, sizeof(int) * (size_t)d.n_ids, st) != hipSuccess ||
      (with_eid && go_malloc((void**)&d.eids, sizeof(int) * (size_t)d.n_ids, st) != hipSuccess)) {
    go_free(d.rec); go_free(d.ids); go_free(d.eids);
    set_error("plan_get_dealt: out of device memory for %lld ids", (long long)d.n_ids);
    return GRAPHOP_ERR_HIP;
  }
  auto fail = [&](int rc) { go_free(d.rec); go_free(d.ids); go_free(d.eids); return rc; };
  const unsigned grid = (unsigned)ceil_div(tasks, 4);
  hipLaunchKernelGGL(k_deal_records, dim3(grid), dim3(256), 0, st, s->wp_lo, s->wp_hi, s->vr_row, s->V, s->W,
                     L, K, (int)tiles, (int4*)d.rec, (int*)len.p);
  if (hipGetLastError() != hipSuccess) return fail(GRAPHOP_ERR_HIP);
  size_t tmp_bytes = 0;
  if (hipcub::DeviceScan::ExclusiveSum(nullptr, tmp_bytes, (int*)len.p, (int*)len.p, (int)(strips + 1), st) != hipSuccess ||
      go_malloc(&tmp.p, tmp_bytes, st) != hipSuccess ||
      hipcub::DeviceScan::ExclusiveSum(tmp.p, tmp_bytes, (int*)len.p, (int*)len.p, (int)(strips + 1), st) != hipSuccess)
    return fail(GRAPHOP_ERR_HIP);
  if (hipMemsetAsync(d.ids, 0, sizeof(int) * (size_t)d.n_ids, st) != hipSuccess) return fail(GRAPHOP_ERR_HIP);
  if (d.eids && hipMemsetAsync(d.eids, 0, sizeof(int) * (size_t)d.n_ids, st) != hipSuccess) return fail(GRAPHOP_ERR_HIP);
  hipLaunchKernelGGL(k_deal_fill, dim3(grid), dim3(256), 0, st, (const int*)len.p, s->W, L, K, (int)tiles,
                     (const int32_t*)p->idx32, (const int32_t*)(with_eid ? p->eid32 : nullptr), (int4*)d.rec,
                     d.ids, d.eids);
  if (hipGetLastError() != hipSuccess || hipStreamSynchronize(st) != hipSuccess) return fail(GRAPHOP_ERR_HIP);
  s->dealt[s->n_dealt] = d;
  *out = &s->dealt[s->n_dealt++];
  return GRAPHOP_OK;
}

int plan_get_walk(graphop_plan* p, int W, i64 win_cols, int groups, int GW, int K, int xcd_slots, hipStream_t st,
                  const Walk** out, bool want_widx) {
  auto* vec = (std::vector<Walk>*)p->walks;
  std::lock_guard<std::mutex> lk(*(std::mutex*)p->sweep_mu);
  *out = nullptr;
  for (auto& w : *vec)
    if (w.W == W && w.win_cols == win_cols && w.groups == groups && w.GW == GW && w.K == K && w.xcd_slots == xcd_slots &&
        (w.widx != nullptr || !want_widx || w.rounds == 0)) {
      if (w.rounds > 0) *out = &w;
      return GRAPHOP_OK;
    }
  if (vec->size() >= 8) return GRAPHOP_OK;
  {
    const int rc_cap = check_not_capturing(st, "building the walk layout of a plan");
    if (rc_cap != GRAPHOP_OK) return rc_cap;
  }
  (void)device_error_word(true);
  {
    const int rc_m = plan_ensure_mirrors(p, st);
    if (rc_m != GRAPHOP_OK) return rc_m;
  }
  const i64 S = p->info.n_segments, E = p->info.n_edges;
  GO_CHECK_ARG(p->info.row_owned && p->sorted_in_rows && p->idx32 && E > 0 && E < 0x7fffffffLL && S > 0 &&
               W >= 1 && groups >= 1 && GW >= 1 && GW <= 4 && groups % GW == 0 && K >= 1 && K <= kWalkK,
               "plan_get_walk: plan is not walkable");
  Walk wk;
  wk.W = W; wk.win_cols = win_cols; wk.groups = groups; wk.GW = GW; wk.K = K; wk.xcd_slots = xcd_slots; wk.rounds = 0;
  const int kmax = K * GW;
  const i64 waves = groups / GW;
  auto remember_unfit = [&]() { vec->push_back(wk); return GRAPHOP_OK; };
  if (p->info.max_index >= (1LL << kWalkKShift) || S * (W + 1) >= (i64)1 << 40 || p->info.max_row >= kWalkRowMask) return remember_unfit();
  const i64* indptr = (const i64*)p->indptr;
  DevBuf seg_eptr, rw, len, ovf, tmp;
  GO_HIP(go_malloc(&seg_eptr.p, sizeof(i64) * (size_t)(S + 1), st));
  hipLaunchKernelGGL(k_seg_eptr, dim3(grid_for(S + 1, kBlock, 4096)), dim3(kBlock), 0, st,
                     (const i64*)p->seg_chunk, indptr, S, (i64*)seg_eptr.p);
  GO_LAUNCH_CHECK();
  GO_HIP(go_malloc(&rw.p, sizeof(int) * (size_t)(S * (W + 1)), st));
  hipLaunchKernelGGL(k_sweep_row_windows, dim3(grid_for(S * (W + 1), kBlock, 16384)), dim3(kBlock), 0, st,
                     (const i64*)seg_eptr.p, (const int32_t*)p->idx32, S, W, win_cols, (int*)rw.p);
  GO_LAUNCH_CHECK();
  GO_HIP(go_malloc(&ovf.p, sizeof(int), st));
  std::vector<i64> h_eptr((size_t)(S + 1));
  GO_HIP(hipMemcpyAsync(h_eptr.data(), seg_eptr.p, sizeof(i64) * (size_t)(S + 1), hipMemcpyDeviceToHost, st));
  GO_HIP(hipStreamSynchronize(st));
  const i64 e0 = h_eptr[0], e_end = h_eptr[(size_t)S];
  std::vector<i64> h_t;
  i64 rounds = ceil_div(S, waves * kmax);
  if (rounds < 1) rounds = 1;
  i64 bins = 0, longest = 0;
  bool fit = false;
  for (int attempt = 0; attempt < 12 && !fit; ++attempt, ++rounds) {
    bins = waves * rounds;
    if (bins * GW >= (1 << 24)) break;
    h_t.assign((size_t)(bins + 1), e_end);
    i64 pos = e0, seg = 0;
    longest = 0;
    for (i64 b = 0; b < bins; ++b) {
      h_t[(size_t)b] = pos;
      if (pos >= e_end) continue;
      const i64 target = ceil_div(e_end - pos, bins - b);
      while (seg < S && h_eptr[(size_t)(seg + 1)] <= pos) ++seg;
      i64 end = pos + target;
      const i64 last_row = seg + kmax - 1 < S - 1 ? seg + kmax - 1 : S - 1;
      if (h_eptr[(size_t)(last_row + 1)] < end) end = h_eptr[(size_t)(last_row + 1)];
      if (end > e_end) end = e_end;
      longest = end - pos > longest ? end - pos : longest;
      pos = end;
    }
    h_t[(size_t)bins] = pos;
    fit = pos >= e_end;
    if (fit) break;
  }
  if (!fit) return remember_unfit();
  DevBuf bin_t;
  GO_HIP(go_malloc(&bin_t.p, sizeof(i64) * (size_t)(bins + 1), st));
  GO_HIP(hipMemcpyAsync(bin_t.p, h_t.data(), sizeof(i64) * (size_t)(bins + 1), hipMemcpyHostToDevice, st));
  GO_HIP(go_malloc(&len.p, sizeof(int) * (size_t)(bins * GW + 1), st));
  GO_HIP(hipMemsetAsync(ovf.p, 0, sizeof(int), st));
  GO_HIP(hipMemsetAsync(len.p, 0, sizeof(int) * (size_t)(bins * GW + 1), st));
  hipLaunchKernelGGL(k_walk_count, dim3((unsigned)ceil_div(bins, 4)), dim3(256), 0, st, (const i64*)seg_eptr.p,
                     (const int*)rw.p, S, W, bins, (const i64*)bin_t.p, GW, kmax, (int*)len.p, (int*)ovf.p);
  GO_LAUNCH_CHECK();
  {
    int h_ovf = 0;
    GO_HIP(hipMemcpyAsync(&h_ovf, ovf.p, sizeof(int), hipMemcpyDeviceToHost, st));
    GO_HIP(hipStreamSynchronize(st));
    if (h_ovf != 0) return remember_unfit();
  }
  wk.longest_run = ceil_div(longest, GW) + W + 1;
  size_t tmp_bytes = 0;
  const i64 gbins = bins * GW;
  GO_HIP(hipcub::DeviceScan::ExclusiveSum(nullptr, tmp_bytes, (int*)len.p, (int*)len.p, (int)(gbins + 1), st));
  GO_HIP(go_malloc(&tmp.p, tmp_bytes ? tmp_bytes : 16, st));
  GO_HIP(hipcub::DeviceScan::ExclusiveSum(tmp.p, tmp_bytes, (int*)len.p, (int*)len.p, (int)(gbins + 1), st));
  int total = 0;
  GO_HIP(hipMemcpyAsync(&total, (int*)len.p + gbins, sizeof(int), hipMemcpyDeviceToHost, st));
  GO_HIP(hipStreamSynchronize(st));
  if (total < 0 || (i64)total > E + 4 * gbins) return remember_unfit();
  wk.rounds = (int)rounds;
  wk.n_slots = (i64)total + 1024;
  wk.max_steps = 8 * W < 1024 ? 8 * W : 1024;
  const i64 steps = rounds * wk.max_steps;
  wk.sync_ints = 64LL * (8 + 16 * steps);
  if (go_malloc((void**)&wk.ids, sizeof(int) * (size_t)wk.n_slots, st) != hipSuccess ||
      (want_widx && go_malloc((void**)&wk.widx, sizeof(int) * (size_t)wk.n_slots, st) != hipSuccess) ||
      go_malloc((void**)&wk.bin_pos, sizeof(int) * (size_t)(gbins + 1), st) != hipSuccess ||
      go_malloc((void**)&wk.bin_rows, sizeof(int) * (size_t)(bins * kmax), st) != hipSuccess ||
      go_malloc((void**)&wk.bin_cum, sizeof(int) * (size_t)gbins, st) != hipSuccess ||
      go_malloc((void**)&wk.sync, sizeof(int) * (size_t)wk.sync_ints * kWalkSyncRing, st) != hipSuccess) {
    go_free(wk.ids); go_free(wk.widx); go_free(wk.bin_pos); go_free(wk.bin_rows); go_free(wk.bin_cum); go_free(wk.sync);
    set_error("plan_get_walk: out of device memory for %lld slots", (long long)wk.n_slots);
    return GRAPHOP_ERR_HIP;
  }
  auto fail = [&](int rc) {
    go_free(wk.ids); go_free(wk.widx); go_free(wk.bin_pos); go_free(wk.bin_rows); go_free(wk.bin_cum); go_free(wk.sync);
    return rc;
  };
  if (hipMemcpyAsync(wk.bin_pos, len.p, sizeof(int) * (size_t)(gbins + 1), hipMemcpyDeviceToDevice, st) != hipSuccess ||
      hipMemsetAsync(wk.ids, 0, sizeof(int) * (size_t)wk.n_slots, st) != hipSuccess ||
      (wk.widx && hipMemsetAsync(wk.widx, 0, sizeof(int) * (size_t)wk.n_slots, st) != hipSuccess))
    return fail(GRAPHOP_ERR_HIP);
  hipLaunchKernelGGL(k_walk_fill, dim3((unsigned)ceil_div(bins, 4)), dim3(256), 0, st, (const i64*)seg_eptr.p,
                     (const int*)rw.p, (const i64*)p->seg_chunk, (const i64*)p->row, (const int32_t*)p->idx32,
                     (const int32_t*)(p->info.eid_identity ? nullptr : p->eid32), S, W, bins, (const i64*)bin_t.p, GW, kmax,
                     (const int*)wk.bin_pos, wk.ids, wk.widx, wk.bin_rows, wk.bin_cum);
  if (hipGetLastError() != hipSuccess || hipStreamSynchronize(st) != hipSuccess) return fail(GRAPHOP_ERR_HIP);
  vec->push_back(wk);
  *out = &vec->back();
  return GRAPHOP_OK;
}

void plan_free_sweeps(graphop_plan* p) {
  if (auto* wv = (std::vector<Walk>*)p->walks) {
    for (auto& w : *wv) {
      go_free(w.ids); go_free(w.widx); go_free(w.bin_pos); go_free(w.bin_rows); go_free(w.bin_cum); go_free(w.sync);
    }
    delete wv;
    p->walks = nullptr;
  }
  auto* vec = (std::vector<Sweep>*)p->sweeps;
  if (vec) {
    for (auto& s : *vec) {
      go_free(s.vr_row); go_free(s.wp_lo); go_free(s.wp_hi);
      go_free(s.queues);
      for (int i = 0; i < s.n_dealt; ++i) { go_free(s.dealt[i].rec); go_free(s.dealt[i].ids); go_free(s.dealt[i].eids); }
    }
    delete vec;
  }
  delete (std::mutex*)p->sweep_mu;
  p->sweeps = nullptr; p->sweep_mu = nullptr;
}

void plan_init_sweeps(graphop_plan* p) {
  p->sweeps = new std::vector<Sweep>();
  ((std::vector<Sweep>*)p->sweeps)->reserve(16);
  p->walks = new std::vector<Walk>();
  ((std::vector<Walk>*)p->walks)->reserve(8);
  p->sweep_mu = new std::mutex();
}

int plan_n_sweeps(const graphop_plan* p) {
  std::lock_guard<std::mutex> lk(*(std::mutex*)p->sweep_mu);
  return (int)((std::vector<Sweep>*)p->sweeps)->size();
}
const Sweep* plan_sweep_at(const graphop_plan* p, int i) {
  std::lock_guard<std::mutex> lk(*(std::mutex*)p->sweep_mu);
  auto* vec = (std::vector<Sweep>*)p->sweeps;
  return (i >= 0 && i < (int)vec->size()) ? &(*vec)[i] : nullptr;
}

static int copy_in(void** dst, const void* src, size_t bytes, hipStream_t st) {
  *dst = nullptr;
  if (!src || bytes == 0) return GRAPHOP_OK;
  GO_HIP(go_malloc(dst, bytes, st));
  GO_HIP(hipMemcpyAsync(*dst, src, bytes, hipMemcpyDeviceToDevice, st));
  return GRAPHOP_OK;
}

int plan_import_arrays(graphop_plan* p, const i64* seg_chunk, const int32_t* idx32, const int32_t* eid32,
                       const int32_t* long_segs, i64 n_long, const int32_t* blk_seg,
                       const int32_t* seg_e0, const int32_t* seg_row, hipStream_t st) {
  const graphop_plan_info_t& in = p->info;
  int rc;
  if ((rc = copy_in((void**)&p->seg_chunk, seg_chunk, sizeof(i64) * (size_t)(in.n_segments + 1), st))) return rc;
  GO_CHECK_ARG(p->seg_chunk != nullptr, "plan_import: seg_chunk is required");
  if ((rc = copy_in((void**)&p->idx32, idx32, sizeof(int32_t) * (size_t)in.n_edges, st))) return rc;
  if ((rc = copy_in((void**)&p->eid32, eid32, sizeof(int32_t) * (size_t)in.n_edges, st))) return rc;
  if ((rc = copy_in((void**)&p->long_segs, long_segs, sizeof(int32_t) * (size_t)n_long, st))) return rc;
  p->n_long = p->long_segs ? n_long : 0;
  if (in.n_dense_blocks > 0 && blk_seg && seg_e0 && seg_row) {
    if ((rc = copy_in((void**)&p->blk_seg, blk_seg, sizeof(int32_t) * (size_t)(in.n_dense_blocks + 1), st))) return rc;
    if ((rc = copy_in((void**)&p->seg_e0, seg_e0, sizeof(int32_t) * (size_t)(in.n_segments + 1), st))) return rc;
    if ((rc = copy_in((void**)&p->seg_row, seg_row, sizeof(int32_t) * (size_t)in.n_segments, st))) return rc;
  } else {
    p->info.n_dense_blocks = 0;
    p->info.dense_fill_pct = 0;
  }
  p->sorted_in_rows = in.sorted_in_rows;
  p->info.has_idx32 = p->idx32 != nullptr;
  return GRAPHOP_OK;
}

int plan_import_sweep(graphop_plan* p, int W, i64 win_cols, int T, int V, const int32_t* vr_row,
                      const int32_t* wp_lo, const int32_t* wp_hi, hipStream_t st) {
  auto* vec = (std::vector<Sweep>*)p->sweeps;
  std::lock_guard<std::mutex> lk(*(std::mutex*)p->sweep_mu);
  for (auto& s : *vec)
    if (s.W == W && s.win_cols == win_cols && s.T == T) return GRAPHOP_OK;
  GO_CHECK_ARG(vec->size() < 16, "plan_import_sweep: too many window geometries for one plan");
  GO_CHECK_ARG(W >= 1 && V >= 1 && vr_row && wp_lo && wp_hi, "plan_import_sweep: bad arguments");
  Sweep s;
  s.W = W; s.win_cols = win_cols; s.T = T; s.V = V;
  int rc;
  if ((rc = copy_in((void**)&s.vr_row, vr_row, sizeof(int) * (size_t)V, st)) ||
      (rc = copy_in((void**)&s.wp_lo, wp_lo, sizeof(int) * (size_t)V * W, st)) ||
      (rc = copy_in((void**)&s.wp_hi, wp_hi, sizeof(int) * (size_t)V * W, st))) {
    go_free(s.vr_row); go_free(s.wp_lo); go_free(s.wp_hi);
    return rc;
  }
  if (go_malloc((void**)&s.queues, sizeof(int) * kQueueRing * kQueueInts, st) != hipSuccess) {
    go_free(s.vr_row); go_free(s.wp_lo); go_free(s.wp_hi); go_free(s.queues);
    set_error("plan_import_sweep: out of device memory");
    return GRAPHOP_ERR_HIP;
  }
  vec->push_back(s);
  return GRAPHOP_OK;
}

}
```

custom_op_benchmark_amd/csrc/plan_api.hip:

```cpp
#include <string.h>

#include "common.h"
#include "host.h"

using namespace graphop;

extern "C" {

int graphop_plan_create(const int64_t* row, const int64_t* indptr, const int64_t* eid,
                        const int64_t* indices, int64_t n_chunks, int64_t n_edges,
                        int64_t n_index_bound, void* stream, graphop_plan_t** plan_out) {
  GO_CHECK_ARG(plan_out != nullptr, "plan_create: plan_out is NULL");
  *plan_out = nullptr;
  GO_CHECK_ARG(indptr != nullptr && (row != nullptr || n_chunks == 0) &&
               (eid != nullptr || n_edges == 0), "plan_create: NULL pointer");
  GO_CHECK_ARG(n_chunks >= 0 && n_chunks < 0x7fffffffLL && n_edges >= 0,
               "plan_create: size out of range");
  GO_TRY(check_not_capturing((hipStream_t)stream, "plan_create"));
  graphop_plan* p = (graphop_plan*)calloc(1, sizeof(graphop_plan));
  GO_CHECK_ARG(p != nullptr, "plan_create: out of host memory");
  p->row = row; p->indptr = indptr; p->eid = eid; p->indices = indices;
  p->info.n_chunks = n_chunks;
  p->info.n_edges = n_edges;
  (void)hipGetDevice(&p->device);
  plan_init_sweeps(p);
  int rc = plan_build(p, n_index_bound, (hipStream_t)stream, tuning().dense_detect_min_fill);
  if (rc == GRAPHOP_OK) rc = plan_build_seg_eptr(p, (hipStream_t)stream);
  if (rc != GRAPHOP_OK) {
    graphop_plan_destroy(p);
    return rc;
  }
  *plan_out = p;
  return GRAPHOP_OK;
}

int graphop_plan_info(const graphop_plan_t* plan, graphop_plan_info_t* info_out) {
  GO_CHECK_ARG(plan && info_out, "plan_info: NULL pointer");
  *info_out = plan->info;
  return GRAPHOP_OK;
}

int graphop_plan_n_sweeps(const graphop_plan_t* plan) { return plan ? plan_n_sweeps(plan) : 0; }

int graphop_plan_sweep_info(const graphop_plan_t* plan, int sweep, graphop_sweep_info_t* out) {
  GO_CHECK_ARG(plan && out, "plan_sweep_info: NULL pointer");
  const Sweep* s = plan_sweep_at(plan, sweep);
  GO_CHECK_ARG(s != nullptr, "plan_sweep_info: no window structure %d", sweep);
  out->win_cols = s->win_cols; out->W = s->W; out->T = s->T; out->V = s->V; out->n_dealt = s->n_dealt;
  return GRAPHOP_OK;
}

int graphop_plan_array(const graphop_plan_t* plan, const char* name, int sweep, const void** ptr,
                       int64_t* bytes) {
  GO_CHECK_ARG(plan && name && ptr && bytes, "plan_array: NULL pointer");
  *ptr = nullptr; *bytes = 0;
  const graphop_plan_info_t& in = plan->info;
  auto give = [&](const void* p, size_t n) { if (p) { *ptr = p; *bytes = (int64_t)n; } return GRAPHOP_OK; };
  if (sweep >= 0) {
    const Sweep* s = plan_sweep_at(plan, sweep);
    GO_CHECK_ARG(s != nullptr, "plan_array: no window structure %d", sweep);
    if (!s->wp_lo || !s->wp_hi || !s->vr_row) {
      const int rcw = plan_rebuild_sweep_tables(const_cast<graphop_plan*>(plan), s, nullptr);
      if (rcw != GRAPHOP_OK) return rcw;
    }
    if (!strcmp(name, "vr_row")) return give(s->vr_row, sizeof(int) * (size_t)s->V);
    if (!strcmp(name, "wp_lo")) return give(s->wp_lo, sizeof(int) * (size_t)s->V * s->W);
    if (!strcmp(name, "wp_hi")) return give(s->wp_hi, sizeof(int) * (size_t)s->V * s->W);
  } else {
    if (!strcmp(name, "idx32") || !strcmp(name, "eid32")) {
      const int rcm = plan_ensure_mirrors_locked(const_cast<graphop_plan*>(plan), nullptr);
      if (rcm != GRAPHOP_OK) return rcm;
    }
    if (!strcmp(name, "seg_chunk")) return give(plan->seg_chunk, sizeof(int64_t) * (size_t)(in.n_segments + 1));
    if (!strcmp(name, "idx32")) return give(plan->idx32, sizeof(int32_t) * (size_t)in.n_edges);
    if (!strcmp(name, "eid32")) return give(plan->eid32, sizeof(int32_t) * (size_t)in.n_edges);
    if (!strcmp(name, "long_segs")) return give(plan->long_segs, sizeof(int32_t) * (size_t)plan->n_long);
    if (!strcmp(name, "blk_seg")) return give(plan->blk_seg, sizeof(int32_t) * (size_t)(in.n_dense_blocks + 1));
    if (!strcmp(name, "seg_e0")) return give(plan->seg_e0, sizeof(int32_t) * (size_t)(in.n_segments + 1));
    if (!strcmp(name, "seg_row")) return give(plan->seg_row, sizeof(int32_t) * (size_t)in.n_segments);
  }
  set_error("plan_array: unknown array '%s'", name);
  return GRAPHOP_ERR_INVALID_ARGUMENT;
}

int graphop_plan_import(const int64_t* row, const int64_t* indptr, const int64_t* eid,
                        const int64_t* indices, const graphop_plan_info_t* info,
                        const int64_t* seg_chunk, const int32_t* idx32, const int32_t* eid32,
                        const int32_t* long_segs, int64_t n_long, const int32_t* blk_seg,
                        const int32_t* seg_e0, const int32_t* seg_row, void* stream,
                        graphop_plan_t** plan_out) {
  GO_CHECK_ARG(plan_out && info && indptr, "plan_import: NULL pointer");
  *plan_out = nullptr;
  GO_CHECK_ARG(info->n_chunks >= 0 && info->n_edges >= 0 && info->n_segments >= 0 && n_long >= 0,
               "plan_import: bad sizes");
  GO_TRY(check_not_capturing((hipStream_t)stream, "plan_import"));
  graphop_plan* p = (graphop_plan*)calloc(1, sizeof(graphop_plan));
  GO_CHECK_ARG(p != nullptr, "plan_import: out of host memory");
  p->row = row; p->indptr = indptr; p->eid = eid; p->indices = indices;
  p->info = *info;
  p->info.n_geometry_fallbacks = 0;
  (void)hipGetDevice(&p->device);
  plan_init_sweeps(p);
  int rc = plan_import_arrays(p, (const i64*)seg_chunk, idx32, eid32, long_segs, n_long, blk_seg, seg_e0,
                              seg_row, (hipStream_t)stream);
  if (rc == GRAPHOP_OK) rc = plan_build_seg_eptr(p, (hipStream_t)stream);
  if (rc != GRAPHOP_OK) { graphop_plan_destroy(p); return rc; }
  *plan_out = p;
  return GRAPHOP_OK;
}

int graphop_plan_import_sweep(graphop_plan_t* plan, const graphop_sweep_info_t* info,
                              const int32_t* vr_row, const int32_t* wp_lo, const int32_t* wp_hi,
                              void* stream) {
  GO_CHECK_ARG(plan && info, "plan_import_sweep: NULL pointer");
  GO_TRY(check_not_capturing((hipStream_t)stream, "plan_import_sweep"));
  return plan_import_sweep(plan, info->W, info->win_cols, info->T, info->V, vr_row, wp_lo, wp_hi,
                           (hipStream_t)stream);
}

int graphop_plan_sweep_dealt(const graphop_plan_t* plan, int sweep, int i, int32_t* L, int32_t* K) {
  GO_CHECK_ARG(plan && L && K, "plan_sweep_dealt: NULL pointer");
  const Sweep* s = plan_sweep_at(plan, sweep);
  GO_CHECK_ARG(s != nullptr && i >= 0 && i < s->n_dealt, "plan_sweep_dealt: no layout %d of window structure %d", i, sweep);
  *L = s->dealt[i].L; *K = s->dealt[i].K;
  return GRAPHOP_OK;
}

int graphop_plan_sweep_build_dealt(graphop_plan_t* plan, const graphop_sweep_info_t* info, int32_t L,
                                   int32_t K, void* stream) {
  GO_CHECK_ARG(plan && info, "plan_sweep_build_dealt: NULL pointer");
  GO_CHECK_ARG(plan->info.has_idx32, "plan_sweep_build_dealt: the plan has no 32-bit mirrors");
  for (int i = 0; i < plan_n_sweeps(plan); ++i) {
    const Sweep* s = plan_sweep_at(plan, i);
    if (s->W == info->W && s->win_cols == info->win_cols && s->T == info->T) {
      const Sweep::Dealt* d = nullptr;
      return plan_get_dealt(plan, s, L, K, (hipStream_t)stream, &d);
    }
  }
  set_error("plan_sweep_build_dealt: no window structure W=%d T=%d", (int)info->W, (int)info->T);
  return GRAPHOP_ERR_INVALID_ARGUMENT;
}

void graphop_plan_destroy(graphop_plan_t* plan) {
  if (!plan) return;
  plan_free_sweeps(plan);
  if (plan->seg_chunk) go_free(plan->seg_chunk);
  if (plan->seg_eptr) go_free(plan->seg_eptr);
  if (plan->idx32) go_free(plan->idx32);
  if (plan->eid32) go_free(plan->eid32);
  if (plan->long_segs) go_free(plan->long_segs);
  if (plan->blk_seg) go_free(plan->blk_seg);
  if (plan->seg_e0) go_free(plan->seg_e0);
  if (plan->seg_row) go_free(plan->seg_row);
  free(plan);
}

}
```

custom_op_benchmark_amd/csrc/runtime.hip:

```cpp
#include <stdarg.h>

#include <map>
#include <mutex>
#include <string>
#include <vector>

#include "common.h"
#include "host.h"
#include "kernels_walk.h"

namespace graphop {

__global__ void k_zero16(uint4* __restrict__ p, i64 n16, unsigned char* __restrict__ tail, int n_tail) {
  i64 i = (i64)blockIdx.x * blockDim.x + threadIdx.x;
  const i64 stride = (i64)gridDim.x * blockDim.x;
  if (i < n_tail) tail[i] = 0;
  for (; i < n16; i += stride) p[i] = make_uint4(0u, 0u, 0u, 0u);
}
__global__ void k_zero1(unsigned char* __restrict__ p, i64 n) {
  i64 i = (i64)blockIdx.x * blockDim.x + threadIdx.x;
  const i64 stride = (i64)gridDim.x * blockDim.x;
  for (; i < n; i += stride) p[i] = 0;
}

// ... 50 lines not shown
      g_bytes -= it->second;
      g_hooked.erase(it);
    } else {
      auto jt = g_plain.find(p);
      if (jt != g_plain.end()) { g_bytes -= jt->second; g_plain.erase(jt); }
    }
    f = g_free;
  }
  if (hooked) { if (f) f(p); return; }
  (void)hipFree(p);
}
bool go_alloc_stream_ordered() {
  std::lock_guard<std::mutex> lk(g_alloc_mu);
  return g_alloc != nullptr;
}

int check_not_capturing(hipStream_t st, const char* what) {
  hipStreamCaptureStatus cs = hipStreamCaptureStatusNone;
  if (hipStreamIsCapturing(st, &cs) == hipSuccess && cs != hipStreamCaptureStatusNone) {
    set_error("%s would allocate and synchronise while the stream is being captured into a HIP graph: "
              "build it first (graphop_plan_create / graphop_plan_prepare, Python: graphop.prepare(graph, h, d)) "
              "and capture afterwards", what);
    return GRAPHOP_ERR_INVALID_ARGUMENT;
  }
  (void)hipGetLastError();
  return GRAPHOP_OK;
}

struct ProfRec { const char* name; const char* kernel; hipEvent_t t0, t1; };
static bool g_prof_on = false;
static std::vector<ProfRec> g_prof;
static std::mutex g_prof_mu;

ProfScope::ProfScope(const char* n, hipStream_t s, const char* k) : st(s), name(n), kernel(k) {
  if (!g_prof_on) return;
  if (hipEventCreate(&t0) != hipSuccess || hipEventCreate(&t1) != hipSuccess) { t0 = nullptr; return; }
  (void)hipEventRecord(t0, st);
}
ProfScope::~ProfScope() {
  if (!t0) return;
  (void)hipEventRecord(t1, st);
  std::lock_guard<std::mutex> lk(g_prof_mu);
  g_prof.push_back({name, kernel, t0, t1});
}



Tuning& tuning_mut() {
  static Tuning t;
  return t;
}
const Tuning& tuning() { return tuning_mut(); }
int tuning_plan_trim() { return tuning().plan_trim; }

hipError_t zero_async(void* ptr, size_t bytes, hipStream_t st) {
  if (bytes == 0) return hipSuccess;
  ProfScope prof("zero_fill", st, "k_zero16");
  unsigned char* p = (unsigned char*)ptr;
  const size_t head = (16 - ((uintptr_t)p & 15)) & 15;
  if (head >= bytes || bytes < 64) {
    hipLaunchKernelGGL(k_zero1, dim3((unsigned)ceil_div((i64)bytes, 256)), dim3(256), 0, st, p, (i64)bytes);
    return hipGetLastError();
  }
  if (head) hipLaunchKernelGGL(k_zero1, dim3(1), dim3(64), 0, st, p, (i64)head);
  p += head;
  const size_t body = bytes - head;
  const i64 n16 = (i64)(body / 16);
  const int n_tail = (int)(body % 16);
  i64 blocks = ceil_div(n16, 256 * 4);
  if (blocks > 8192) blocks = 8192;
  if (blocks < 1) blocks = 1;
  hipLaunchKernelGGL(k_zero16, dim3((unsigned)blocks), dim3(256), 0, st, (uint4*)p, n16, p + n16 * 16, n_tail);
  return hipGetLastError();
}

static int* g_err_host = nullptr;
static int* g_err_dev = nullptr;
static std::mutex g_err_mu;
struct WalkLaunchRec { const char* tag; int device; unsigned seq; };
static WalkLaunchRec g_walk_ring[256];
static unsigned g_walk_seq = 0;
int* device_error_word(bool create) {
  std::lock_guard<std::mutex> lk(g_err_mu);
  if (!g_err_host && create) {
    void* h = nullptr;
    if (hipHostMalloc(&h, 64, hipHostMallocMapped | hipHostMallocPortable) == hipSuccess) {
      memset(h, 0, 64);
      void* d = nullptr;
      if (hipHostGetDevicePointer(&d, h, 0) == hipSuccess) { g_err_host = (int*)h; g_err_dev = (int*)d; }
      else (void)hipHostFree(h);
    }
    (void)hipGetLastError();
  }
  return g_err_dev;
}
int walk_launch_id(const char* tag) {
  int dev = 0;
  (void)hipGetDevice(&dev);
  std::lock_guard<std::mutex> lk(g_err_mu);
  const unsigned seq = ++g_walk_seq;
  g_walk_ring[seq & 255] = WalkLaunchRec{tag, dev, seq};
  return (int)seq;
}
int check_async_error(bool clear) {
  int code = 0, seq = 0;
  WalkLaunchRec rec{nullptr, -1, 0};
  {
    std::lock_guard<std::mutex> lk(g_err_mu);
    if (!g_err_host) return GRAPHOP_OK;
    code = __atomic_load_n(g_err_host, __ATOMIC_ACQUIRE);
    if (code == 0) return GRAPHOP_OK;
    seq = __atomic_load_n(g_err_host + 1, __ATOMIC_ACQUIRE);
    if (g_walk_ring[(unsigned)seq & 255].seq == (unsigned)seq) rec = g_walk_ring[(unsigned)seq & 255];
    if (clear) {
      __atomic_store_n(g_err_host + 1, 0, __ATOMIC_RELEASE);
      __atomic_store_n(g_err_host, 0, __ATOMIC_RELEASE);
    }
  }
  const char* what = code == kWalkErrQuad ? "a (step, quad) unit waited for its quad's previous step"
                   : code == kWalkErrRing ? "a worker wave waited for a ring chunk of its feeder wave"
                   : "unknown code";
  char where[96];
  if (rec.tag) snprintf(where, sizeof(where), "pass '%s' on device %d, walk launch #%d", rec.tag, rec.device, seq);
  else snprintf(where, sizeof(where), "walk launch #%d", seq);
  set_error("a walk kernel (k_spmm_walk_* / k_attn_fwd_walk_f32) of an earlier launch aborted (%s): %s until its spin bound "
            "expired (device error code %d); the outputs of that launch and of every launch that consumed them are invalid%s",
            where, what, code,
            clear ? "" : " -- sticky: graphop_check_device_errors() acknowledges and clears it");
  return GRAPHOP_ERR_HIP;
}

}

using namespace graphop;

namespace {
struct TuneEntry { const char* k; int* p; };
std::vector<TuneEntry> tune_table() {
  Tuning& t = tuning_mut();
  return {
      {"sddmm_cpg", &t.sddmm_cpg}, {"spmm_cpg", &t.spmm_cpg}, {"force_generic", &t.force_generic},
      {"sweep", &t.sweep}, {"window_kb", &t.window_kb}, {"mall_window_kb", &t.mall_window_kb}, {"max_windows", &t.max_windows},
      {"sweep_min_kb", &t.sweep_min_kb}, {"sweep_bpc", &t.sweep_bpc}, {"sweep_k", &t.sweep_k},
      {"vrow_t", &t.vrow_t}, {"sweep_min_granule", &t.sweep_min_granule}, {"sweep_w", &t.sweep_w}, {"spmm_window_scale", &t.spmm_window_scale}, {"dense_blocks", &t.dense_blocks}, {"dense_min_fill", &t.dense_min_fill},
      {"dense_detect_min_fill", &t.dense_detect_min_fill},
      {"attn_fused", &t.attn_fused},
      {"attn_window_scale", &t.attn_window_scale}, {"attn_k", &t.attn_k}, {"attn_bpc", &t.attn_bpc},
      {"attn_rows", &t.attn_rows}, {"attn_heads", &t.attn_heads}, {"attn_fwd_walk", &t.attn_fwd_walk}, {"spmm_selfzero", &t.spmm_selfzero},
      {"spmm_selfzero_min_mb", &t.spmm_selfzero_min_mb}, {"spmm_flat", &t.spmm_flat},
      {"spmm_flat_cpg", &t.spmm_flat_cpg}, {"spmm_flat_max_mean", &t.spmm_flat_max_mean},
      {"spmm_flat_min_chunks", &t.spmm_flat_min_chunks}, {"staged_ids", &t.staged_ids}, {"attn_max_d", &t.attn_max_d},
      {"touch_sddmm", &t.touch_sddmm}, {"walk", &t.walk}, {"walk_window_kb", &t.walk_window_kb}, {"walk_window_kb_col", &t.walk_window_kb_col},
      {"walk_drift", &t.walk_drift}, {"walk_min_bin", &t.walk_min_bin}, {"walk_blocks", &t.walk_blocks}, {"walk_debug", &t.walk_debug}, {"walk_fault", &t.walk_fault}, {"walk_steps", &t.walk_steps},
      {"plan_trim", &t.plan_trim}};
}
}


extern "C" {


int graphop_abi_version(void) { return GRAPHOP_ABI_VERSION; }
const char* graphop_last_error(void) { return get_error(); }

int graphop_tune(const char* key, int value) {
  GO_CHECK_ARG(key != nullptr, "tune: key is NULL");
  for (auto& e : tune_table())
    if (strcmp(e.k, key) == 0) {
      *e.p = value;
      return GRAPHOP_OK;
    }
  set_error("tune: unknown key '%s'", key);
  return GRAPHOP_ERR_INVALID_ARGUMENT;
}

int graphop_tune_get(const char* key, int* value) {
  GO_CHECK_ARG(key != nullptr && value != nullptr, "tune_get: NULL pointer");
  for (auto& e : tune_table())
    if (strcmp(e.k, key) == 0) {
      *value = *e.p;
      return GRAPHOP_OK;
    }
  set_error("tune_get: unknown key '%s'", key);
  return GRAPHOP_ERR_INVALID_ARGUMENT;
}

const char* graphop_tune_key(int i) {
  static const std::vector<TuneEntry> tab = tune_table();
  return (i >= 0 && i < (int)tab.size()) ? tab[(size_t)i].k : nullptr;
}

int64_t graphop_memory_bytes(void) {
  std::lock_guard<std::mutex> lk(g_alloc_mu);
  return (int64_t)g_bytes;
}

int graphop_check_device_errors(void) { return check_async_error(true); }

int graphop_tune_reset(void) {
  tuning_mut() = Tuning();
  return GRAPHOP_OK;
}

int graphop_set_allocator(graphop_alloc_fn alloc_fn, graphop_free_fn free_fn) {
  GO_CHECK_ARG((alloc_fn == nullptr) == (free_fn == nullptr), "set_allocator: give both callbacks or neither");
  std::lock_guard<std::mutex> lk(g_alloc_mu);
  g_alloc = alloc_fn;
  g_free = free_fn;
  return GRAPHOP_OK;
}

int graphop_profile_enable(int on) {
  std::lock_guard<std::mutex> lk(g_prof_mu);
  g_prof_on = on != 0;
  return GRAPHOP_OK;
}

int graphop_profile_read(graphop_profile_rec_t* out, int cap) {
  std::lock_guard<std::mutex> lk(g_prof_mu);
  std::map<std::string, graphop_profile_rec_t> agg;
  std::vector<std::string> order;
  for (auto& r : g_prof) {
    float ms = 0.f;
    if (hipEventSynchronize(r.t1) != hipSuccess || hipEventElapsedTime(&ms, r.t0, r.t1) != hipSuccess) {
      set_error("profile_read: event query failed");
      return -1;
    }
    (void)hipEventDestroy(r.t0);
    (void)hipEventDestroy(r.t1);
    auto it = agg.find(r.name);
    if (it == agg.end()) {
      graphop_profile_rec_t rec;
      memset(&rec, 0, sizeof(rec));
      strncpy(rec.name, r.name, sizeof(rec.name) - 1);
      strncpy(rec.kernel, r.kernel ? r.kernel : "", sizeof(rec.kernel) - 1);
      rec.min_ms = ms;
      it = agg.emplace(r.name, rec).first;
      order.push_back(r.name);
    }
    it->second.calls += 1;
    it->second.total_ms += ms;
    if (ms < it->second.min_ms) it->second.min_ms = ms;
    if (ms > it->second.max_ms) it->second.max_ms = ms;
  }
  g_prof.clear();
  int n = 0;
  for (auto& k : order) {
    if (out && n < cap) out[n] = agg[k];
    ++n;
  }
  return n;
}

int graphop_partition_csr_count(const int64_t* indptr, int64_t n_rows, int64_t chunk_size,
                                int64_t* first_chunk, void* stream) {
  GO_CHECK_ARG(indptr && first_chunk, "partition_csr_count: NULL pointer");
  GO_CHECK_ARG(n_rows >= 0 && n_rows < 0x7ffffffeLL, "partition_csr_count: n_rows out of range");
  GO_CHECK_ARG(chunk_size >= 1, "partition_csr_count: chunk_size must be >= 1");
  return partition_count((const i64*)indptr, n_rows, chunk_size, (i64*)first_chunk,
                         (hipStream_t)stream);
}

int graphop_partition_csr_fill(const int64_t* indptr, const int64_t* first_chunk, int64_t n_rows,
                               int64_t chunk_size, int64_t n_chunks, int64_t* row,
                               int64_t* indptr_out, void* stream) {
  GO_CHECK_ARG(indptr && first_chunk && indptr_out && (row || n_chunks == 0),
               "partition_csr_fill: NULL pointer");
  GO_CHECK_ARG(n_rows >= 0 && n_chunks >= 0 && chunk_size >= 1, "partition_csr_fill: bad size");
  return partition_fill((const i64*)indptr, (const i64*)first_chunk, n_rows, chunk_size, n_chunks,
                        (i64*)row, (i64*)indptr_out, (hipStream_t)stream);
}

}
```

include/graphop_hip.h:

```cpp
#ifndef GRAPHOP_HIP_H_
#define GRAPHOP_HIP_H_

#include <stddef.h>
#include <stdint.h>

#ifdef __cplusplus
extern "C" {
#endif

#if defined(__GNUC__)
#define GRAPHOP_API __attribute__((visibility("default")))
#else
#define GRAPHOP_API
#endif

#define GRAPHOP_ABI_VERSION 8

#define GRAPHOP_F32 0
#define GRAPHOP_F64 1

#define GRAPHOP_OK 0
#define GRAPHOP_ERR_INVALID_ARGUMENT 1
#define GRAPHOP_ERR_HIP 2
#define GRAPHOP_ERR_BAD_GRAPH 3

typedef struct graphop_plan graphop_plan_t;

typedef struct graphop_plan_info {
  int64_t n_chunks;
  int64_t n_edges;
  int64_t n_segments;
  int64_t max_row;
  int64_t max_index;
  int64_t max_segment_len;
  int32_t rows_sorted;
  int32_t indptr_monotone;
  int32_t eid_identity;
  int32_t full_coverage;
  int32_t row_owned;
  int32_t has_idx32;
  int32_t dense_fill_pct;
  int32_t sorted_in_rows;
  int64_t n_dense_blocks;
  int64_t max_row_gap;
  int64_t n_geometry_fallbacks;
} graphop_plan_info_t;

GRAPHOP_API int graphop_abi_version(void);
GRAPHOP_API const char* graphop_last_error(void);
GRAPHOP_API int graphop_check_device_errors(void);

GRAPHOP_API int graphop_tune(const char* key, int value);
GRAPHOP_API int graphop_tune_reset(void);
GRAPHOP_API int graphop_tune_get(const char* key, int* value);
GRAPHOP_API const char* graphop_tune_key(int i);
GRAPHOP_API int64_t graphop_memory_bytes(void);

typedef void* (*graphop_alloc_fn)(size_t bytes, int device, void* stream);
typedef void (*graphop_free_fn)(void* ptr);
GRAPHOP_API int graphop_set_allocator(graphop_alloc_fn alloc_fn, graphop_free_fn free_fn);

typedef struct graphop_profile_rec {
  char name[48];
  char kernel[48];
  int64_t calls;
  double total_ms;
  double min_ms;
  double max_ms;
} graphop_profile_rec_t;
GRAPHOP_API int graphop_profile_enable(int on);
GRAPHOP_API int graphop_profile_read(graphop_profile_rec_t* out, int cap);

GRAPHOP_API int graphop_partition_csr_count(const int64_t* indptr, int64_t n_rows, int64_t chunk_size,
                                int64_t* first_chunk, void* stream);
GRAPHOP_API int graphop_partition_csr_fill(const int64_t* indptr, const int64_t* first_chunk, int64_t n_rows,
                               int64_t chunk_size, int64_t n_chunks, int64_t* row,
                               int64_t* indptr_out, void* stream);

GRAPHOP_API int graphop_plan_create(const int64_t* row, const int64_t* indptr, const int64_t* eid,
                        const int64_t* indices, int64_t n_chunks, int64_t n_edges,
                        int64_t n_index_bound, void* stream, graphop_plan_t** plan_out);
GRAPHOP_API int graphop_plan_info(const graphop_plan_t* plan, graphop_plan_info_t* info_out);
GRAPHOP_API void graphop_plan_destroy(graphop_plan_t* plan);

GRAPHOP_API int graphop_plan_prepare(graphop_plan_t* plan, int dtype, int64_t n_table_rows, int64_t h,
                         int64_t d, int fused, void* stream);

typedef struct graphop_sweep_info {
  int64_t win_cols;
  int32_t W;
  int32_t T;
  int32_t V;
  int32_t n_dealt;
} graphop_sweep_info_t;
GRAPHOP_API int graphop_plan_n_sweeps(const graphop_plan_t* plan);
GRAPHOP_API int graphop_plan_sweep_info(const graphop_plan_t* plan, int sweep, graphop_sweep_info_t* out);
GRAPHOP_API int graphop_plan_array(const graphop_plan_t* plan, const char* name, int sweep, const void** ptr,
                       int64_t* bytes);
GRAPHOP_API int graphop_plan_import(const int64_t* row, const int64_t* indptr, const int64_t* eid,
                        const int64_t* indices, const graphop_plan_info_t* info,
                        const int64_t* seg_chunk, const int32_t* idx32, const int32_t* eid32,
                        const int32_t* long_segs, int64_t n_long, const int32_t* blk_seg,
                        const int32_t* seg_e0, const int32_t* seg_row, void* stream,
                        graphop_plan_t** plan_out);
GRAPHOP_API int graphop_plan_import_sweep(graphop_plan_t* plan, const graphop_sweep_info_t* info,
                              const int32_t* vr_row, const int32_t* wp_lo, const int32_t* wp_hi,
                              void* stream);
GRAPHOP_API int graphop_plan_sweep_dealt(const graphop_plan_t* plan, int sweep, int i, int32_t* L, int32_t* K);
GRAPHOP_API int graphop_plan_sweep_build_dealt(graphop_plan_t* plan, const graphop_sweep_info_t* info, int32_t L,
                                   int32_t K, void* stream);

GRAPHOP_API int graphop_maskedmm_csr_forward(int dtype, const int64_t* row, const int64_t* indptr,
                                 const int64_t* eid, const int64_t* indices, const void* A,
                                 const void* B, void* y, int64_t n_chunks, int64_t n_edges,
                                 int64_t n_a, int64_t n_b, int64_t h, int64_t d,
                                 const graphop_plan_t* plan, void* stream);

GRAPHOP_API int graphop_maskedmm_csr_forward_partial(int dtype, const int64_t* row, const int64_t* indptr,
                                         const int64_t* eid, const int64_t* indices, const void* A,
                                         const void* B, void* y, int64_t n_chunks, int64_t n_slots,
                                         int64_t n_y, int64_t n_a, int64_t n_b, int64_t h, int64_t d,
                                         void* stream);

GRAPHOP_API int graphop_maskedmm_csr_backward(int dtype, const int64_t* row, const int64_t* indptr_r,
                                  const int64_t* eid_r, const int64_t* indices_r,
                                  const int64_t* col, const int64_t* indptr_c,
                                  const int64_t* eid_c, const int64_t* indices_c, const void* A,
                                  const void* B, const void* dy, void* dA, void* dB,
                                  int64_t n_row_chunks, int64_t n_col_chunks, int64_t n_edges,
                                  int64_t n_a, int64_t n_b, int64_t h, int64_t d,
                                  const graphop_plan_t* plan_r, const graphop_plan_t* plan_c,
                                  void* stream);

GRAPHOP_API int graphop_sparse_softmax_forward(int dtype, const int64_t* row, const int64_t* indptr,
                                   const int64_t* eid, const void* x, void* y, int64_t n_chunks,
                                   int64_t n_edges, int64_t h, void* workspace,
                                   int64_t workspace_rows, const graphop_plan_t* plan,
                                   void* stream);

GRAPHOP_API int graphop_sparse_softmax_backward(int dtype, const int64_t* row, const int64_t* indptr,
                                    const int64_t* eid, const void* y, const void* dy, void* dx,
                                    int64_t n_chunks, int64_t n_edges, int64_t h,
                                    void* workspace, int64_t workspace_rows,
                                    const graphop_plan_t* plan, void* stream);

GRAPHOP_API int graphop_vector_spmm_forward(int dtype, const int64_t* row, const int64_t* indptr,
                                const int64_t* eid, const int64_t* indices, const void* edata,
                                const void* x, void* y, int64_t n_chunks, int64_t n_edges,
                                int64_t n_x, int64_t n_y, int64_t h, int64_t d,
                                const graphop_plan_t* plan, void* stream);

GRAPHOP_API int graphop_vector_spmm_backward(int dtype, const int64_t* row, const int64_t* indptr,
                                 const int64_t* eid, const int64_t* indices, const int64_t* col,
                                 const int64_t* indptr_t, const int64_t* eid_t,
                                 const int64_t* indices_t, const void* edata, const void* dy,
                                 const void* x, void* dedata, void* dx, int64_t n_row_chunks,
                                 int64_t n_col_chunks, int64_t n_edges, int64_t n_x, int64_t n_dy,
                                 int64_t h, int64_t d, const graphop_plan_t* plan_r,
                                 const graphop_plan_t* plan_c, void* stream);

GRAPHOP_API int graphop_interleave_pairs(int dtype, const void* w0, const void* w1, void* out2, int64_t n, void* stream);
GRAPHOP_API int graphop_spmm_pair_supported(int dtype, int64_t n_chunks, int64_t n_edges, int64_t n_x, int64_t h,
                                int64_t d, const graphop_plan_t* plan);
GRAPHOP_API int graphop_spmm_pair(int dtype, const int64_t* row, const int64_t* indptr, const int64_t* eid,
                      const int64_t* indices, const void* w2, const void* X0, const void* X1, void* out0,
                      void* out1, int64_t n_chunks, int64_t n_edges, int64_t n_x, int64_t n_out, int64_t h,
                      int64_t d, const graphop_plan_t* plan, void* stream);
GRAPHOP_API int graphop_node_mul_edge_forward(int dtype, const int64_t* row, const int64_t* indptr,
                                  const int64_t* eid, const void* A, const void* B, void* y,
                                  int64_t n_chunks, int64_t n_edges, int64_t n_a, int64_t h,
                                  int64_t d, const graphop_plan_t* plan, void* stream);

GRAPHOP_API int graphop_node_mul_edge_backward(int dtype, const int64_t* row, const int64_t* indptr,
                                   const int64_t* eid, const void* A, const void* B,
                                   const void* dy, void* dA, void* dB, int64_t n_chunks,
                                   int64_t n_edges, int64_t n_a, int64_t h, int64_t d,
                                   const graphop_plan_t* plan, void* stream);

GRAPHOP_API int graphop_gat_scores_forward(int dtype, const int64_t* row, const int64_t* indptr, const int64_t* eid,
                               const int64_t* indices, const void* el, const void* er, void* y, int64_t n_chunks,
                               int64_t n_edges, int64_t n_l, int64_t n_r, int64_t h, double negative_slope,
                               const graphop_plan_t* plan, void* stream);
GRAPHOP_API int graphop_gat_scores_backward(int dtype, const int64_t* row, const int64_t* indptr_r,
                                const int64_t* eid_r, const int64_t* indices_r, const int64_t* col,
                                const int64_t* indptr_c, const int64_t* eid_c, const int64_t* indices_c,
                                const void* el, const void* er, const void* dy, void* del, void* der,
                                int64_t n_row_chunks, int64_t n_col_chunks, int64_t n_edges, int64_t n_l,
                                int64_t n_r, int64_t h, double negative_slope, const graphop_plan_t* plan_r,
                                const graphop_plan_t* plan_c, void* stream);

GRAPHOP_API int graphop_gatv2_scores_forward(int dtype, const int64_t* row, const int64_t* indptr, const int64_t* eid,
                                 const int64_t* indices, const void* xl, const void* xr, const void* att, void* y,
                                 int64_t n_chunks, int64_t n_edges, int64_t n_l, int64_t n_r, int64_t h, int64_t d,
                                 double negative_slope, const graphop_plan_t* plan, void* stream);
GRAPHOP_API int graphop_gatv2_scores_backward(int dtype, const int64_t* row, const int64_t* indptr_r,
                                  const int64_t* eid_r, const int64_t* indices_r, const int64_t* col,
                                  const int64_t* indptr_c, const int64_t* eid_c, const int64_t* indices_c,
                                  const void* xl, const void* xr, const void* att, const void* dy, void* dxl,
// ... 236 lines not shown
```

Baseline: 10.06 billion edges/s.

## Add LDS-tiled SDDMM kernel reusing staged A rows across column windows

Adds a new SDDMM path for f32, h=1, d=64. It stages a tile of R A-rows in LDS per (window, tile) task and groups edges by destination column into batched records, so each B row is loaded once and dotted against several staged A rows. A host-side layout builder precomputes parts, records, slot maps and row tables in parallel threads, and the kernel prefetches the next task's descriptors and touches its metadata. It is enabled by default with R=192. The cost is a large extra plan structure, preprocessing time, and a gate that falls back to the old sweep when the shape does not fit.

```diff
diff --git a/custom_op_benchmark_amd/_lib.py b/custom_op_benchmark_amd/_lib.py
--- a/custom_op_benchmark_amd/_lib.py
+++ b/custom_op_benchmark_amd/_lib.py
@@ -23,7 +23,8 @@
                 ("full_coverage", ctypes.c_int32), ("row_owned", ctypes.c_int32),
                 ("has_idx32", ctypes.c_int32), ("dense_fill_pct", ctypes.c_int32),
                 ("sorted_in_rows", ctypes.c_int32), ("n_dense_blocks", _c64), ("max_row_gap", _c64),
-                ("n_geometry_fallbacks", _c64)]
+                ("n_geometry_fallbacks", _c64),
+                ("sddmm_tile_rows", ctypes.c_int32), ("sddmm_tile_repeat_permille", ctypes.c_int32)]
 
 
 class SweepInfo(ctypes.Structure):
diff --git a/custom_op_benchmark_amd/csrc/common.h b/custom_op_benchmark_amd/csrc/common.h
--- a/custom_op_benchmark_amd/csrc/common.h
+++ b/custom_op_benchmark_amd/csrc/common.h
@@ -94,6 +94,23 @@
   static constexpr int kMaxDealt = 4;
   Dealt dealt[kMaxDealt];
   int n_dealt = 0;
+  struct Tile {
+    int R = 0, cap = 0;
+    int tiles = 0;
+    int fits = 0;
+    long long slots = 0, distinct = 0, records = 0, batches = 0, n_parts = 0;
+    long long bytes = 0;
+    int* part_ptr = nullptr;
+    int* parts = nullptr;
+    unsigned short* rec = nullptr;
+    int* bstart = nullptr;
+    int* slotw = nullptr;
+    int* rowtab = nullptr;
+    int* tdesc = nullptr;
+  };
+  static constexpr int kMaxTile = 4;
+  Tile tile[kMaxTile];
+  int n_tile = 0;
 };
 struct Walk {
   int W = 0;
diff --git a/custom_op_benchmark_amd/csrc/graphop_hip.hip b/custom_op_benchmark_amd/csrc/graphop_hip.hip
--- a/custom_op_benchmark_amd/csrc/graphop_hip.hip
+++ b/custom_op_benchmark_amd/csrc/graphop_hip.hip
@@ -11,6 +11,8 @@
 #include "host_attn_rows.h"
 #include "kernels_fast.h"
 #include "kernels_walk.h"
+#include "kernels_tile.h"
+#include "tile_layout.h"
 #include "kernels_attn_walk.h"
 #include "kernels_attn_bias_fwd.h"
 #include "kernels_block.h"
@@ -127,7 +129,8 @@
       staged_ok = pi.eid_identity || dl->eids != nullptr || opts->no_eids;
     }
   }
-  if (!staged_ok) {
+  out->sweep = sw;
+  if (!staged_ok && !(opts && opts->tile)) {
     const int rcp = plan_pin_sweep_tables(const_cast<graphop_plan*>(plan), sw, st);
     if (rcp != GRAPHOP_OK) return -rcp;
   }
@@ -458,10 +461,86 @@
 
 namespace {
 
+struct TileLaunch {
+  TileView view;
+  unsigned blocks;
+  size_t lds_bytes;
+  int nt;
+};
+template <int L, int NV>
+int choose_tile(const graphop_plan* plan, i64 n_table_rows, i64 h, int dtype, hipStream_t st, TileLaunch* out, bool dry_run) {
+  if constexpr (L != 16 || NV != 1) {
+    return 0;
+  } else {
+    const Tuning& t = tuning();
+    if (!t.sddmm_tile || !plan || dtype != GRAPHOP_F32 || h != 1) return 0;
+    if (!plan->info.eid_identity || !table_off32(n_table_rows, L, NV)) return 0;
+    const int R = t.sddmm_tile_rows;
+    if (R != 128 && R != 192 && R != 256 && R != 384) return 0;
+    SweepLaunch sl;
+    SweepOpts so;
+    so.dry_run = 1;
+    so.tile = 1;
+    so.bpc = sweep_bpc(NV, true);
+    const int use = choose_sweep(plan, n_table_rows, L, NV, st, &sl, false, &so);
+    if (use != 1) return use;
+    const int per_cu = R <= 192 ? 2 : 1;
+    if (t.sddmm_tile != 2 && (i64)sl.sweep->W * ceil_div((i64)sl.sweep->V, R) < 32LL * t.n_cu * per_cu) return 0;
+    const int lds_wg = (kTileLdsBytes / per_cu) & ~255;
+    int cap = (lds_wg - R * 16 * L * NV) / 4;
+    if (cap > kTileMaxCap) cap = kTileMaxCap;
+    const Sweep::Tile* tl = nullptr;
+    const int rc = plan_get_tile(const_cast<graphop_plan*>(plan), sl.sweep, R, cap, t.sddmm_tile == 2, t.sddmm_tile_min_repeat, st, &tl);
+    if (rc != GRAPHOP_OK) return -rc;
+    if (!tl) return 0;
+    plan_trim(const_cast<graphop_plan*>(plan));
+    TileView& v = out->view;
+    v = TileView{};
+    v.part_ptr = tl->part_ptr; v.parts = (const int4*)tl->parts; v.rec = tl->rec; v.bstart = tl->bstart; v.slotw = tl->slotw;
+    v.rowtab = (const int2*)tl->rowtab; v.tdesc = (const int4*)tl->tdesc; v.vr_row = sl.sweep->vr_row;
+    v.V = sl.sweep->V; v.W = sl.sweep->W; v.R = R; v.tiles = tl->tiles; v.win_cols = (int)sl.sweep->win_cols;
+    v.touch = t.sddmm_tile_touch ? 1 : 0;
+    v.sync = nullptr;
+    if (!dry_run) {
+      v.sync = plan_take_queue(const_cast<graphop_plan*>(plan), sl.sweep);
+      if (zero_async(v.sync, sizeof(int) * kQueueInts, st) != hipSuccess) return -GRAPHOP_ERR_HIP;
+    }
+    const i64 tasks = (i64)tl->tiles * v.W;
+    i64 nb = (i64)t.n_cu * per_cu;
+    if (nb > tasks) nb = tasks;
+    out->blocks = (unsigned)(nb < 1 ? 1 : nb);
+    out->lds_bytes = (size_t)R * 16 * L * NV + (size_t)cap * 4;
+    out->nt = per_cu == 2 ? 512 : 1024;
+    return 1;
+  }
+}
+template <int L, int NV>
+void launch_tile(const TileLaunch& tl, const float* a, const float* b, float* y, hipStream_t st) {
+  if constexpr (L == 16 && NV == 1) {
+    if (tl.nt == 512) {
+      allow_full_lds((const void*)k_sddmm_tile_f32<L, NV, 512>);
+      hipLaunchKernelGGL((k_sddmm_tile_f32<L, NV, 512>), dim3(tl.blocks), dim3(512), tl.lds_bytes, st, tl.view, a, b, y);
+    } else {
+      allow_full_lds((const void*)k_sddmm_tile_f32<L, NV, 1024>);
+      hipLaunchKernelGGL((k_sddmm_tile_f32<L, NV, 1024>), dim3(tl.blocks), dim3(1024), tl.lds_bytes, st, tl.view, a, b, y);
+    }
+  }
+}
+
 template <int L, int NV>
 int try_sddmm_sweep(const char* tag, int dtype, const graphop_plan* plan, i64 n_table_rows, const void* A,
                     const void* B, void* y, i64 h, int d4, hipStream_t st) {
   if (!plan) return 0;
+  {
+    TileLaunch tl;
+    const int ut = choose_tile<L, NV>(plan, n_table_rows, h, dtype, st, &tl, false);
+    if (ut < 0) return ut;
+    if (ut == 1) {
+      ProfScope prof(tag, st, "k_sddmm_tile_f32");
+      launch_tile<L, NV>(tl, (const float*)A, (const float*)B, (float*)y, st);
+      return 1;
+    }
+  }
   SweepLaunch sl;
   SweepOpts so;
   const bool f64 = dtype == GRAPHOP_F64;
@@ -1006,7 +1085,13 @@
     o.bpc = f64 ? 3 : sweep_bpc(NV, h == 1);
     o.staged = sddmm_staged(plan, L, NV, h, n_table_rows);
     o.stage_lds_per_group = StageCfg<L, 1>::kLdsIntsPerGroup * (int)sizeof(int) + (h > 1 ? 64 * (int)h : 0);
-    if (!f64 || (o.staged && NV == 1 && L >= 16))
+    int tiled = 0;
+    if (!f64) {
+      TileLaunch tl;
+      tiled = choose_tile<L, NV>(plan, n_table_rows, h, dtype, st, &tl, true);
+      if (tiled < 0) rc = tiled;
+    }
+    if (tiled == 0 && (!f64 || (o.staged && NV == 1 && L >= 16)))
       rc = choose_sweep(plan, n_table_rows, L, NV, st, &sl, false, &o);
     o.staged = spmm_staged(L, NV, h, n_table_rows);
     if (rc >= 0 && !f64) rc = choose_sweep(plan, n_table_rows, L, NV, st, &sl, true, &o);
diff --git a/custom_op_benchmark_amd/csrc/host.h b/custom_op_benchmark_amd/csrc/host.h
--- a/custom_op_benchmark_amd/csrc/host.h
+++ b/custom_op_benchmark_amd/csrc/host.h
@@ -55,6 +55,10 @@
   int walk_debug;
   int walk_fault;
   int walk_blocks;
+  int sddmm_tile;
+  int sddmm_tile_rows;
+  int sddmm_tile_min_repeat;
+  int sddmm_tile_touch;
   int plan_trim;
   int n_cu;
   Tuning() {
@@ -98,6 +102,10 @@
     walk_blocks = env_int("GRAPHOP_WALK_BLOCKS", 0);
     walk_debug = env_int("GRAPHOP_WALK_DEBUG", 0);
     walk_fault = 0;
+    sddmm_tile = env_int("GRAPHOP_SDDMM_TILE", 1);
+    sddmm_tile_rows = env_int("GRAPHOP_SDDMM_TILE_ROWS", 192);
+    sddmm_tile_min_repeat = env_int("GRAPHOP_SDDMM_TILE_MIN_REPEAT", 20);
+    sddmm_tile_touch = env_int("GRAPHOP_SDDMM_TILE_TOUCH", 1);
     plan_trim = env_int("GRAPHOP_PLAN_TRIM", 1);
     n_cu = 256;
     int dev = 0;
@@ -141,6 +149,7 @@
 }
 
 struct SweepLaunch {
+  const Sweep* sweep = nullptr;
   SweepView view;
   unsigned blocks;
   size_t lds_bytes;
@@ -155,6 +164,7 @@
   int touch = 0;
   int staged = 0;
   int stage_lds_per_group = 0;
+  int tile = 0;
   int no_eids = 0;
 };
 
@@ -167,6 +177,7 @@
 int plan_get_sweep(graphop_plan*, int, i64, int, hipStream_t, const Sweep**);
 int* plan_take_queue(graphop_plan*, const Sweep*);
 int plan_get_dealt(graphop_plan*, const Sweep*, int, int, hipStream_t, const Sweep::Dealt**, bool want_eids = true);
+int plan_get_tile(graphop_plan*, const Sweep*, int R, int cap, bool force, int min_repeat_pct, hipStream_t, const Sweep::Tile**);
 void plan_free_sweeps(graphop_plan*);
 int plan_get_walk(graphop_plan*, int, i64, int, int, int, int, hipStream_t, const Walk**, bool want_widx = true);
 int plan_build_seg_eptr(graphop_plan*, hipStream_t);
diff --git a/custom_op_benchmark_amd/csrc/kernels_tile.h b/custom_op_benchmark_amd/csrc/kernels_tile.h
--- /dev/null
+++ b/custom_op_benchmark_amd/csrc/kernels_tile.h
@@ -0,0 +1,193 @@
+#pragma once
+#include "kernels_wown.h"
+
+namespace graphop {
+
+struct TileView {
+  const int* part_ptr;
+  const int4* parts;
+  const unsigned short* rec;
+  const int* bstart;
+  const int* slotw;
+  const int2* rowtab;
+  const int4* tdesc;
+  const int* vr_row;
+  int* sync;
+  int V, W, R, tiles;
+  int win_cols;
+  int touch;
+};
+
+constexpr int kTileLdsBytes = 158 * 1024;
+
+__device__ __forceinline__ int row16_incl_scan(int v) {
+  v += __builtin_amdgcn_update_dpp(0, v, 0x111, 0xF, 0xF, true);
+  v += __builtin_amdgcn_update_dpp(0, v, 0x112, 0xF, 0xF, true);
+  v += __builtin_amdgcn_update_dpp(0, v, 0x114, 0xF, 0xF, true);
+  v += __builtin_amdgcn_update_dpp(0, v, 0x118, 0xF, 0xF, true);
+  return v;
+}
+__device__ __forceinline__ int row16_max(int v) {
+  v = max(v, __builtin_amdgcn_update_dpp(0, v, 0xB1, 0xF, 0xF, true));
+  v = max(v, __builtin_amdgcn_update_dpp(0, v, 0x4E, 0xF, 0xF, true));
+  v = max(v, __builtin_amdgcn_update_dpp(0, v, 0x141, 0xF, 0xF, true));
+  v = max(v, __builtin_amdgcn_update_dpp(0, v, 0x140, 0xF, 0xF, true));
+  return v;
+}
+
+constexpr int kTileDescParts = 4;
+
+template <int L = 16, int NV = 1, int NT = 1024>
+__global__ __launch_bounds__(NT, 4) void k_sddmm_tile_f32(TileView tv, const float* __restrict__ A,
+                                                          const float* __restrict__ B, float* __restrict__ y) {
+  static_assert(L == 16 && NV == 1, "256-B rows: one float4 per lane of a 16-lane group");
+  extern __shared__ float4 lds[];
+  __shared__ int task_sh[2][2];
+  __shared__ int desc_sh[2][2 + 4 * kTileDescParts];
+  __shared__ int ctr_sh;
+  constexpr int G = NT / L;
+  const int l = threadIdx.x % L, g = threadIdx.x / L;
+  float* res = reinterpret_cast<float*>(lds + (i64)tv.R * L);
+  const char* lds_l = reinterpret_cast<const char*>(lds) + l * 16;
+  SweepView qv{};
+  qv.sync = tv.sync;
+  qv.W = tv.W;
+  WownQueue queue(qv, tv.tiles);
+  auto fetch_desc = [&](int slot, int w, int t) {
+    const int lane = threadIdx.x & (kWave - 1);
+    const i64 task = (i64)w * tv.tiles + t;
+    const int p0 = tv.part_ptr[task], p1 = tv.part_ptr[task + 1];
+    if (lane < 4 * kTileDescParts && p0 * 4 + lane < p1 * 4)
+      desc_sh[slot][2 + lane] = reinterpret_cast<const int*>(tv.parts)[(i64)p0 * 4 + lane];
+    if (lane == 0) { desc_sh[slot][0] = p0; desc_sh[slot][1] = p1; }
+  };
+  int raw = -1;
+  if (threadIdx.x < kWave) {
+    int w = -1, t = 0;
+    const bool more = queue.pull(w, t);
+    raw = more ? queue.issue() : -1;
+    if (threadIdx.x == 0) { task_sh[0][0] = more ? w : -1; task_sh[0][1] = t; }
+    if (more) fetch_desc(0, w, t);
+  }
+  auto next_batch = [&]() {
+    int v = 0;
+    if (l == 0) v = atomicAdd(&ctr_sh, 1);
+    return group_bcast<L, 0>(v);
+  };
+  int par = 0;
+  for (;;) {
+    __syncthreads();
+    const int w = task_sh[par][0], t = task_sh[par][1];
+    if (w < 0) break;
+    if (threadIdx.x < kWave) {
+      int wn = -1, tn = 0;
+      const bool more = queue.resolve(raw, wn, tn);
+      raw = more ? queue.issue() : -1;
+      if (threadIdx.x == 0) { task_sh[par ^ 1][0] = more ? wn : -1; task_sh[par ^ 1][1] = tn; }
+    }
+    if (threadIdx.x == kWave) ctr_sh = 0;
+    const int v0 = t * tv.R;
+    const int nr = (tv.V - v0) < tv.R ? (tv.V - v0) : tv.R;
+    const int2* rows = tv.rowtab + ((i64)w * tv.V + v0);
+    for (int i = g; i < nr; i += G) {
+      const int2 r = rows[i];
+      const i64 arow = tv.vr_row[v0 + i];
+      if (((unsigned)r.y >> 16) != 0) lds[i * L + l] = ld4(A, arow * L + l);
+    }
+    __syncthreads();
+    if (threadIdx.x >= NT - kWave) {
+      const int wn = task_sh[par ^ 1][0], tn = task_sh[par ^ 1][1];
+      if (wn >= 0) {
+        fetch_desc(par ^ 1, wn, tn);
+        if (tv.touch) {
+          const int4 nd = tv.tdesc[(i64)wn * tv.tiles + tn];
+          const int lane = threadIdx.x & (kWave - 1);
+          int tch[11];
+#pragma unroll
+          for (int q = 0; q < 11; ++q) tch[q] = 0;
+          const int nrec = nd.y * 16;
+#pragma unroll
+          for (int q = 0; q < 3; ++q) {
+            const int at = (q * kWave + lane) * 64;
+            if (at < nrec) tch[q] = tv.rec[(i64)nd.x * 16 + at];
+          }
+#pragma unroll
+          for (int q = 0; q < 5; ++q) {
+            const int at = (q * kWave + lane) * 32;
+            if (at < nd.w) tch[3 + q] = tv.slotw[(i64)nd.z + at];
+          }
+          if (lane * 32 < nd.y) tch[8] = tv.bstart[nd.x + lane * 32];
+          const int vn = tn * tv.R;
+          const int nrn = (tv.V - vn) < tv.R ? (tv.V - vn) : tv.R;
+          if (lane * 16 < nrn) tch[9] = tv.rowtab[(i64)wn * tv.V + vn + lane * 16].x;
+          if (lane * 32 < nrn) tch[10] = tv.vr_row[vn + lane * 32];
+          asm volatile("; touched %0 %1 %2 %3 %4 %5 %6 %7 %8 %9 %10" ::"v"(tch[0]), "v"(tch[1]), "v"(tch[2]), "v"(tch[3]),
+                       "v"(tch[4]), "v"(tch[5]), "v"(tch[6]), "v"(tch[7]), "v"(tch[8]), "v"(tch[9]), "v"(tch[10]));
+        }
+      }
+    }
+    const unsigned win_id0 = (unsigned)w * (unsigned)tv.win_cols;
+    const int p0 = desc_sh[par][0], p1 = desc_sh[par][1];
+    for (int p = p0; p < p1; ++p) {
+      int4 pt;
+      if (p - p0 < kTileDescParts) {
+        const int* d = &desc_sh[par][2 + 4 * (p - p0)];
+        pt = make_int4(d[0], d[1], d[2], d[3]);
+      } else {
+        pt = tv.parts[p];
+      }
+      const int nb = (pt.y + 15) >> 4;
+      int b = next_batch();
+      int rw = 0, bs = 0;
+      if (b < nb) { rw = tv.rec[((i64)pt.x + b) * 16 + l]; bs = tv.bstart[(i64)pt.x + b]; }
+      while (b < nb) {
+        const bool valid = b * 16 + l < pt.y;
+        const int cnt = valid ? (rw & 3) + 1 : 0;
+        const unsigned my_off = valid ? (win_id0 + (unsigned)(rw >> 2)) * 256u : 0u;
+        const int first = bs + row16_incl_scan(cnt) - cnt;
+        const int gmax = row16_max(cnt);
+        int sw[4];
+#pragma unroll
+        for (int k = 0; k < 4; ++k) {
+          sw[k] = 0;
+          if (__builtin_amdgcn_ballot_w64(k < cnt) != 0 && k < cnt) sw[k] = tv.slotw[first + k];
+        }
+        float4 bb[16];
+        static_for<16>([&](auto uc) {
+          constexpr int u = decltype(uc)::value;
+          const unsigned o = group_bcast<L, u>(my_off);
+          bb[u] = ld16_off<float>(B, o + (unsigned)(l * 16));
+        });
+        const int bn = next_batch();
+        if (bn < nb) { rw = tv.rec[((i64)pt.x + bn) * 16 + l]; bs = tv.bstart[(i64)pt.x + bn]; }
+#pragma unroll
+        for (int k = 0; k < 4; ++k) {
+          if (k < gmax) {
+            const unsigned my_koff = ((unsigned)sw[k] >> 16) * 256u;
+            float part[16];
+            static_for<16>([&](auto uc) {
+              constexpr int u = decltype(uc)::value;
+              const unsigned ko = group_bcast<L, u>(my_koff);
+              const float4 av = *reinterpret_cast<const float4*>(lds_l + ko);
+              part[u] = dot4(av, bb[u]);
+            });
+            const float r = group_dots_to_owner<L, 16>(part, l);
+            if (k < cnt) res[sw[k] & 0xffff] = r;
+          }
+        }
+        b = bn;
+      }
+      __syncthreads();
+      if (threadIdx.x == kWave) ctr_sh = 0;
+      for (int i = pt.z + g; i < pt.z + pt.w; i += G) {
+        const int2 r = rows[i];
+        const int len = (int)((unsigned)r.y >> 16), off = r.y & 0xffff;
+        for (int x = l; x < len; x += L) __builtin_nontemporal_store(res[off + x], y + ((i64)r.x + x));
+      }
+      if (p + 1 < p1) __syncthreads();
+    }
+    par ^= 1;
+  }
+}
+
+}
diff --git a/custom_op_benchmark_amd/csrc/plan.hip b/custom_op_benchmark_amd/csrc/plan.hip
--- a/custom_op_benchmark_amd/csrc/plan.hip
+++ b/custom_op_benchmark_amd/csrc/plan.hip
@@ -4,6 +4,7 @@
 #include <vector>
 
 #include "common.h"
+#include "tile_layout.h"
 
 namespace graphop {
 
@@ -786,11 +787,14 @@
     if (p->idx32 && p->indices) { go_free(p->idx32); p->idx32 = nullptr; }
     if (p->eid32 && p->eid) { go_free(p->eid32); p->eid32 = nullptr; }
   }
-  for (auto& s : *(std::vector<Sweep>*)p->sweeps)
-    if (!s.runtime_wp && s.n_dealt > 0) {
+  for (auto& s : *(std::vector<Sweep>*)p->sweeps) {
+    bool tiled = false;
+    for (int i = 0; i < s.n_tile; ++i) tiled = tiled || s.tile[i].slotw != nullptr;
+    if (!s.runtime_wp && (s.n_dealt > 0 || tiled)) {
       go_free(s.wp_lo); go_free(s.wp_hi);
       s.wp_lo = s.wp_hi = nullptr;
     }
+  }
 }
 
 int plan_get_sweep(graphop_plan* p, int W, i64 win_cols, int T, hipStream_t st, const Sweep** out) {
@@ -894,6 +898,92 @@
   if (hipGetLastError() != hipSuccess || hipStreamSynchronize(st) != hipSuccess) return fail(GRAPHOP_ERR_HIP);
   s->dealt[s->n_dealt] = d;
   *out = &s->dealt[s->n_dealt++];
+  return GRAPHOP_OK;
+}
+
+static void tile_free_arrays(Sweep::Tile& t) {
+  go_free(t.part_ptr); go_free(t.parts); go_free(t.rec); go_free(t.bstart); go_free(t.slotw); go_free(t.rowtab); go_free(t.tdesc);
+  t.part_ptr = t.parts = t.bstart = t.slotw = t.rowtab = t.tdesc = nullptr;
+  t.rec = nullptr;
+  t.bytes = 0;
+}
+template <typename T>
+static int tile_upload(T** dst, const std::vector<T>& src, Sweep::Tile& t, hipStream_t st) {
+  const size_t bytes = sizeof(T) * (src.size() ? src.size() : 8);
+  GO_HIP(go_malloc((void**)dst, bytes, st));
+  if (!src.empty()) GO_HIP(hipMemcpyAsync(*dst, src.data(), sizeof(T) * src.size(), hipMemcpyHostToDevice, st));
+  t.bytes += (long long)bytes;
+  return GRAPHOP_OK;
+}
+
+int plan_get_tile(graphop_plan* p, const Sweep* sw, int R, int cap, bool force, int min_repeat_pct, hipStream_t st,
+                  const Sweep::Tile** out) {
+  std::lock_guard<std::mutex> lk(*(std::mutex*)p->sweep_mu);
+  Sweep* s = const_cast<Sweep*>(sw);
+  *out = nullptr;
+  Sweep::Tile* t = nullptr;
+  for (int i = 0; i < s->n_tile; ++i)
+    if (s->tile[i].R == R && s->tile[i].cap == cap) t = &s->tile[i];
+  auto wanted = [&](const Sweep::Tile& x) {
+    return x.fits && x.slots > 0 && (force || (x.slots - x.distinct) * 100 >= (long long)min_repeat_pct * x.slots);
+  };
+  if (t && (!wanted(*t) || t->slotw)) {
+    if (wanted(*t)) *out = t;
+    return GRAPHOP_OK;
+  }
+  if (!t && s->n_tile >= Sweep::kMaxTile) return GRAPHOP_OK;
+  {
+    const int rc_cap = check_not_capturing(st, "building the tile layout of a plan");
+    if (rc_cap != GRAPHOP_OK) return rc_cap;
+  }
+  const i64 E = p->info.n_edges;
+  if (R < 1 || R > kTileMaxRows || cap < 1 || cap > kTileMaxCap || E <= 0 || E + kTileSlotPad >= 0x7fffffffLL ||
+      s->win_cols > kTileMaxWinCols)
+    return GRAPHOP_OK;
+  {
+    int rc_in = plan_ensure_mirrors(p, st);
+    if (rc_in == GRAPHOP_OK && (!s->wp_lo || !s->wp_hi || !s->vr_row)) rc_in = sweep_fill_arrays(p, *s, st);
+    if (rc_in != GRAPHOP_OK) return rc_in;
+  }
+  if (!p->idx32) return GRAPHOP_OK;
+  const size_t nwp = (size_t)s->V * (size_t)s->W;
+  std::vector<int> h_lo(nwp), h_hi(nwp), h_idx((size_t)E);
+  GO_HIP(hipMemcpyAsync(h_lo.data(), s->wp_lo, sizeof(int) * nwp, hipMemcpyDeviceToHost, st));
+  GO_HIP(hipMemcpyAsync(h_hi.data(), s->wp_hi, sizeof(int) * nwp, hipMemcpyDeviceToHost, st));
+  GO_HIP(hipMemcpyAsync(h_idx.data(), p->idx32, sizeof(int) * (size_t)E, hipMemcpyDeviceToHost, st));
+  GO_HIP(hipStreamSynchronize(st));
+  TileLayoutHost host;
+  std::vector<tile_detail::TaskCount> counts;
+  TileTotals tot = build_tile_layout(s->V, s->W, R, cap, s->win_cols, h_lo.data(), h_hi.data(), h_idx.data(),
+                                     force ? &host : nullptr, 0, &counts);
+  if (!t) {
+    t = &s->tile[s->n_tile++];
+    *t = Sweep::Tile();
+    t->R = R; t->cap = cap; t->tiles = (int)ceil_div((i64)s->V, R);
+  }
+  t->fits = tot.fits ? 1 : 0;
+  t->slots = tot.slots; t->distinct = tot.distinct; t->records = tot.records; t->batches = tot.batches; t->n_parts = tot.parts;
+  p->info.sddmm_tile_rows = R;
+  p->info.sddmm_tile_repeat_permille = tot.slots > 0 ? (int32_t)((tot.slots - tot.distinct) * 1000 / tot.slots) : 0;
+  if (!wanted(*t)) return GRAPHOP_OK;
+  if (!force) {
+    tot = build_tile_layout(s->V, s->W, R, cap, s->win_cols, h_lo.data(), h_hi.data(), h_idx.data(), &host, 0, &counts);
+    if (!tot.fits) { t->fits = 0; return GRAPHOP_OK; }
+  }
+  int rc = tile_upload(&t->part_ptr, host.part_ptr, *t, st);
+  if (rc == GRAPHOP_OK) rc = tile_upload(&t->parts, host.parts, *t, st);
+  if (rc == GRAPHOP_OK) rc = tile_upload(&t->rec, host.rec, *t, st);
+  if (rc == GRAPHOP_OK) rc = tile_upload(&t->bstart, host.bstart, *t, st);
+  if (rc == GRAPHOP_OK) rc = tile_upload(&t->slotw, host.slotw, *t, st);
+  if (rc == GRAPHOP_OK) rc = tile_upload(&t->rowtab, host.rowtab, *t, st);
+  if (rc == GRAPHOP_OK) rc = tile_upload(&t->tdesc, host.tdesc, *t, st);
+  if (rc == GRAPHOP_OK && hipStreamSynchronize(st) != hipSuccess) rc = GRAPHOP_ERR_HIP;
+  if (rc != GRAPHOP_OK) {
+    (void)hipStreamSynchronize(st);
+    tile_free_arrays(*t);
+    return rc;
+  }
+  *out = t;
   return GRAPHOP_OK;
 }
 
@@ -1043,6 +1133,7 @@
       go_free(s.vr_row); go_free(s.wp_lo); go_free(s.wp_hi);
       go_free(s.queues);
       for (int i = 0; i < s.n_dealt; ++i) { go_free(s.dealt[i].rec); go_free(s.dealt[i].ids); go_free(s.dealt[i].eids); }
+      for (int i = 0; i < s.n_tile; ++i) tile_free_arrays(s.tile[i]);
     }
     delete vec;
   }
diff --git a/custom_op_benchmark_amd/csrc/plan_api.hip b/custom_op_benchmark_amd/csrc/plan_api.hip
--- a/custom_op_benchmark_amd/csrc/plan_api.hip
+++ b/custom_op_benchmark_amd/csrc/plan_api.hip
@@ -99,6 +99,8 @@
   p->row = row; p->indptr = indptr; p->eid = eid; p->indices = indices;
   p->info = *info;
   p->info.n_geometry_fallbacks = 0;
+  p->info.sddmm_tile_rows = 0;
+  p->info.sddmm_tile_repeat_permille = 0;
   (void)hipGetDevice(&p->device);
   plan_init_sweeps(p);
   int rc = plan_import_arrays(p, (const i64*)seg_chunk, idx32, eid32, long_segs, n_long, blk_seg, seg_e0,
diff --git a/custom_op_benchmark_amd/csrc/runtime.hip b/custom_op_benchmark_amd/csrc/runtime.hip
--- a/custom_op_benchmark_amd/csrc/runtime.hip
+++ b/custom_op_benchmark_amd/csrc/runtime.hip
@@ -226,6 +226,8 @@
       {"spmm_flat_min_chunks", &t.spmm_flat_min_chunks}, {"staged_ids", &t.staged_ids}, {"attn_max_d", &t.attn_max_d},
       {"touch_sddmm", &t.touch_sddmm}, {"walk", &t.walk}, {"walk_window_kb", &t.walk_window_kb}, {"walk_window_kb_col", &t.walk_window_kb_col},
       {"walk_drift", &t.walk_drift}, {"walk_min_bin", &t.walk_min_bin}, {"walk_blocks", &t.walk_blocks}, {"walk_debug", &t.walk_debug}, {"walk_fault", &t.walk_fault}, {"walk_steps", &t.walk_steps},
+      {"sddmm_tile", &t.sddmm_tile}, {"sddmm_tile_rows", &t.sddmm_tile_rows}, {"sddmm_tile_min_repeat", &t.sddmm_tile_min_repeat},
+      {"sddmm_tile_touch", &t.sddmm_tile_touch},
       {"plan_trim", &t.plan_trim}};
 }
 }
diff --git a/custom_op_benchmark_amd/csrc/tile_layout.h b/custom_op_benchmark_amd/csrc/tile_layout.h
--- /dev/null
+++ b/custom_op_benchmark_amd/csrc/tile_layout.h
@@ -0,0 +1,217 @@
+#pragma once
+#include <algorithm>
+#include <cstdint>
+#include <thread>
+#include <vector>
+
+namespace graphop {
+
+constexpr int kTileMaxRows = 384;
+constexpr int kTileMaxCap = 65535;
+constexpr int kTileMaxRowSlots = 65535;
+constexpr int kTileRecSlots = 4;
+constexpr int kTileBatch = 16;
+constexpr int kTileMaxWinCols = 1 << 14;
+constexpr int kTileSlotPad = 64;
+
+struct TileTotals {
+  long long slots = 0, distinct = 0, records = 0, batches = 0, parts = 0;
+  int max_part_slots = 0;
+  bool fits = true;
+  double repeat_fraction() const { return slots > 0 ? 1.0 - (double)distinct / (double)slots : 0.0; }
+};
+
+struct TileLayoutHost {
+  std::vector<int> part_ptr;
+  std::vector<int> parts;
+  std::vector<uint16_t> rec;
+  std::vector<int> bstart;
+  std::vector<int> slotw;
+  std::vector<int> rowtab;
+  std::vector<int> tdesc;
+  std::vector<long long> task_slots, task_distinct;
+};
+
+namespace tile_detail {
+
+struct Scratch {
+  std::vector<int> cnt, pos4, posr, seen, touched;
+  explicit Scratch(long long win_cols) : cnt((size_t)win_cols, 0), pos4((size_t)win_cols, 0), posr((size_t)win_cols, 0), seen((size_t)win_cols, 0) {}
+};
+
+struct TaskCount {
+  int parts = 0;
+  long long batches = 0, slots = 0, distinct = 0, records = 0;
+  int max_part_slots = 0;
+  bool fits = true;
+};
+
+struct Geometry {
+  int V, W, R, cap, tiles;
+  long long win_cols;
+  const int *wp_lo, *wp_hi, *idx32;
+};
+
+inline TaskCount do_task(const Geometry& g, int w, int t, Scratch& sc, TileLayoutHost* out, int p0, long long b0, long long s0) {
+  TaskCount tc;
+  const int v0 = t * g.R, nr = std::min(g.R, g.V - v0);
+  const long long base = (long long)w * g.V + v0, col0 = (long long)w * g.win_cols;
+  int i = 0;
+  while (i < nr) {
+    int i1 = i, part_slots = 0;
+    while (i1 < nr) {
+      const int len = g.wp_hi[base + i1] - g.wp_lo[base + i1];
+      if (len > g.cap || len > kTileMaxRowSlots) { tc.fits = false; return tc; }
+      if (part_slots + len > g.cap) break;
+      part_slots += len;
+      ++i1;
+    }
+    if (part_slots == 0) break;
+    sc.touched.clear();
+    for (int r = i; r < i1; ++r)
+      for (int e = g.wp_lo[base + r]; e < g.wp_hi[base + r]; ++e) {
+        const int c = (int)(g.idx32[e] - col0);
+        if (sc.cnt[(size_t)c]++ == 0) sc.touched.push_back(c);
+      }
+    std::sort(sc.touched.begin(), sc.touched.end());
+    long long ncls[kTileRecSlots + 1] = {0, 0, 0, 0, 0};
+    for (const int c : sc.touched) {
+      const int n = sc.cnt[(size_t)c];
+      ncls[kTileRecSlots] += n / kTileRecSlots;
+      if (n % kTileRecSlots) ++ncls[n % kTileRecSlots];
+    }
+    const long long nrec = ncls[1] + ncls[2] + ncls[3] + ncls[4];
+    const long long nbatch = (nrec + kTileBatch - 1) / kTileBatch;
+    if (out) {
+      long long rfirst[kTileRecSlots + 1], sfirst[kTileRecSlots + 1], rcur[kTileRecSlots + 1];
+      long long racc = 0, sacc = 0;
+      for (int k = kTileRecSlots; k >= 1; --k) { rfirst[k] = racc; sfirst[k] = sacc; racc += ncls[k]; sacc += ncls[k] * k; rcur[k] = 0; }
+      uint16_t* rec = out->rec.data() + (b0 + tc.batches) * kTileBatch;
+      for (long long q = 0; q < nbatch * kTileBatch; ++q) rec[q] = 0;
+      for (const int c : sc.touched) {
+        const int n = sc.cnt[(size_t)c], full = n / kTileRecSlots, rem = n % kTileRecSlots;
+        sc.pos4[(size_t)c] = (int)(sfirst[kTileRecSlots] + rcur[kTileRecSlots] * kTileRecSlots);
+        for (int q = 0; q < full; ++q) rec[rfirst[kTileRecSlots] + rcur[kTileRecSlots]++] = (uint16_t)((c << 2) | (kTileRecSlots - 1));
+        if (rem) {
+          sc.posr[(size_t)c] = (int)(sfirst[rem] + rcur[rem] * rem);
+          rec[rfirst[rem] + rcur[rem]++] = (uint16_t)((c << 2) | (rem - 1));
+        }
+      }
+      int* bstart = out->bstart.data() + (b0 + tc.batches);
+      const long long sbase = s0 + tc.slots;
+      for (long long b = 0; b < nbatch; ++b) {
+        const long long q = b * kTileBatch;
+        long long s = 0;
+        for (int k = kTileRecSlots; k >= 1; --k) {
+          const long long in_front = std::min(std::max(q - rfirst[k], 0LL), ncls[k]);
+          s += in_front * k;
+        }
+        bstart[b] = (int)(sbase + s);
+      }
+      int off = 0;
+      for (int r = i; r < i1; ++r) {
+        const int lo = g.wp_lo[base + r], hi = g.wp_hi[base + r];
+        out->rowtab[2 * (size_t)(base + r)] = lo;
+        out->rowtab[2 * (size_t)(base + r) + 1] = (int)((unsigned)off | ((unsigned)(hi - lo) << 16));
+        for (int e = lo; e < hi; ++e) {
+          const int c = (int)(g.idx32[e] - col0);
+          const int k = sc.seen[(size_t)c]++;
+          const int n4 = (sc.cnt[(size_t)c] / kTileRecSlots) * kTileRecSlots;
+          const int pos = k < n4 ? sc.pos4[(size_t)c] + k : sc.posr[(size_t)c] + (k - n4);
+          out->slotw[(size_t)(sbase + pos)] = (r << 16) | (off + (e - lo));
+        }
+        off += hi - lo;
+      }
+      int* pt = out->parts.data() + 4 * (size_t)(p0 + tc.parts);
+      pt[0] = (int)(b0 + tc.batches); pt[1] = (int)nrec; pt[2] = i; pt[3] = i1 - i;
+    }
+    for (const int c : sc.touched) { sc.cnt[(size_t)c] = 0; sc.seen[(size_t)c] = 0; }
+    tc.parts += 1;
+    tc.batches += nbatch;
+    tc.slots += part_slots;
+    tc.distinct += (long long)sc.touched.size();
+    tc.records += nrec;
+    tc.max_part_slots = std::max(tc.max_part_slots, part_slots);
+    i = i1;
+  }
+  if (out) {
+    const int done = tc.parts > 0 ? out->parts[4 * (size_t)(p0 + tc.parts - 1) + 2] + out->parts[4 * (size_t)(p0 + tc.parts - 1) + 3] : 0;
+    for (int r = done; r < nr; ++r) {
+      out->rowtab[2 * (size_t)(base + r)] = g.wp_lo[base + r];
+      out->rowtab[2 * (size_t)(base + r) + 1] = 0;
+    }
+  }
+  return tc;
+}
+
+template <typename F>
+inline void parallel_tasks(long long n, int threads, F&& f) {
+  if (threads < 1) threads = 1;
+  if (threads > n) threads = (int)(n > 0 ? n : 1);
+  if (threads == 1) { f(0, 0LL, n); return; }
+  std::vector<std::thread> pool;
+  for (int k = 0; k < threads; ++k) pool.emplace_back([&f, k, n, threads]() { f(k, n * k / threads, n * (k + 1) / threads); });
+  for (auto& th : pool) th.join();
+}
+
+}
+
+inline TileTotals build_tile_layout(int V, int W, int R, int cap, long long win_cols, const int* wp_lo, const int* wp_hi,
+                                    const int* idx32, TileLayoutHost* out, int threads = 0,
+                                    std::vector<tile_detail::TaskCount>* reuse = nullptr) {
+  using namespace tile_detail;
+  TileTotals tot;
+  if (V < 1 || W < 1 || R < 1 || R > kTileMaxRows || cap < 1 || cap > kTileMaxCap || win_cols < 1 || win_cols > kTileMaxWinCols) { tot.fits = false; return tot; }
+  const int tiles = (V + R - 1) / R;
+  const long long ntask = (long long)W * tiles;
+  const Geometry g{V, W, R, cap, tiles, win_cols, wp_lo, wp_hi, idx32};
+  if (threads <= 0) {
+    const unsigned hw = std::thread::hardware_concurrency();
+    threads = (int)std::min<unsigned>(hw ? hw : 1, 16);
+  }
+  std::vector<TaskCount> local;
+  std::vector<TaskCount>& counts = reuse ? *reuse : local;
+  if ((long long)counts.size() != ntask) {
+    counts.assign((size_t)ntask, TaskCount());
+    parallel_tasks(ntask, threads, [&](int, long long a, long long b) {
+      Scratch sc(win_cols);
+      for (long long k = a; k < b; ++k) counts[(size_t)k] = do_task(g, (int)(k / tiles), (int)(k % tiles), sc, nullptr, 0, 0, 0);
+    });
+  }
+  std::vector<long long> b0((size_t)ntask + 1, 0), s0((size_t)ntask + 1, 0);
+  std::vector<int> p0((size_t)ntask + 1, 0);
+  for (long long k = 0; k < ntask; ++k) {
+    const TaskCount& c = counts[(size_t)k];
+    tot.fits = tot.fits && c.fits;
+    tot.slots += c.slots; tot.distinct += c.distinct; tot.records += c.records; tot.batches += c.batches; tot.parts += c.parts;
+    tot.max_part_slots = std::max(tot.max_part_slots, c.max_part_slots);
+    p0[(size_t)k + 1] = p0[(size_t)k] + c.parts;
+    b0[(size_t)k + 1] = b0[(size_t)k] + c.batches;
+    s0[(size_t)k + 1] = s0[(size_t)k] + c.slots;
+  }
+  if (!tot.fits || !out) return tot;
+  if (tot.slots + kTileSlotPad >= 0x7fffffffLL || tot.batches * kTileBatch >= 0x7fffffffLL) { tot.fits = false; return tot; }
+  out->part_ptr.assign(p0.begin(), p0.end());
+  out->parts.assign(4 * (size_t)tot.parts, 0);
+  out->rec.assign((size_t)(tot.batches * kTileBatch), 0);
+  out->bstart.assign((size_t)tot.batches, 0);
+  out->slotw.assign((size_t)(tot.slots + kTileSlotPad), 0);
+  out->rowtab.assign(2 * (size_t)W * V, 0);
+  out->tdesc.assign(4 * (size_t)ntask, 0);
+  out->task_slots.resize((size_t)ntask);
+  out->task_distinct.resize((size_t)ntask);
+  for (long long k = 0; k < ntask; ++k) {
+    out->task_slots[(size_t)k] = counts[(size_t)k].slots;
+    out->task_distinct[(size_t)k] = counts[(size_t)k].distinct;
+    int* td = out->tdesc.data() + 4 * (size_t)k;
+    td[0] = (int)b0[(size_t)k]; td[1] = (int)counts[(size_t)k].batches; td[2] = (int)s0[(size_t)k]; td[3] = (int)counts[(size_t)k].slots;
+  }
+  parallel_tasks(ntask, threads, [&](int, long long a, long long b) {
+    Scratch sc(win_cols);
+    for (long long k = a; k < b; ++k)
+      (void)do_task(g, (int)(k / tiles), (int)(k % tiles), sc, out, p0[(size_t)k], b0[(size_t)k], s0[(size_t)k]);
+  });
+  return tot;
+}
+
+}
diff --git a/include/graphop_hip.h b/include/graphop_hip.h
--- a/include/graphop_hip.h
+++ b/include/graphop_hip.h
@@ -44,6 +44,8 @@
   int64_t n_dense_blocks;
   int64_t max_row_gap;
   int64_t n_geometry_fallbacks;
+  int32_t sddmm_tile_rows;
+  int32_t sddmm_tile_repeat_permille;
 } graphop_plan_info_t;
 
 GRAPHOP_API int graphop_abi_version(void);
```

Result: faster. 10.24 billion edges/s, median of 6 (+1.7%).
